# WCC-Analytics/sidecar

Hardware: AMD Instinct MI355X
Metric: record-merges/sec (whole node) + rounds-to-converge wall time, H=32768 S=16 (higher is better)
Workload: dtype int64

## Files before the change

sidecar_amd/csrc/gx_device.hpp:

```cpp
#pragma once
#include <hip/hip_runtime.h>
#include <stdint.h>

#include "../../include/gx.h"

#define GXD __device__ __forceinline__
#define GXHD __host__ __device__ __forceinline__

#define GX_GLOBAL __attribute__((address_space(1)))
typedef unsigned int gx_u32x4 __attribute__((ext_vector_type(4)));
template <class T>
GXD T gld(const T *p) {
  return *(const GX_GLOBAL T *)p;
}
typedef unsigned int gx_u32x3 __attribute__((ext_vector_type(3)));
template <class T>
GXD void gst(T *p, T v) {
  *(GX_GLOBAL T *)p = v;
}
GXD gx_u32x4 gld4(const void *p) { return *(const GX_GLOBAL gx_u32x4 *)p; }
GXD gx_u32x3 gld3(const void *p) { return *(const GX_GLOBAL gx_u32x3 *)p; }
GXD void gst4(void *p, gx_u32x4 v) { *(GX_GLOBAL gx_u32x4 *)p = v; }

struct grec {
  uint64_t w;
  uint32_t r;
  uint32_t pad;
};
GXD grec gld_rec(const grec *p) {
  const gx_u32x4 x = gld4(p);
  grec g;
  g.w = (uint64_t)x.x | ((uint64_t)x.y << 32);
  g.r = x.z;
  g.pad = x.w;
  return g;
}
GXD void gst_rec(grec *p, const grec &g) {
  gx_u32x4 x;
  x.x = (uint32_t)g.w;
  x.y = (uint32_t)(g.w >> 32);
  x.z = g.r;
  x.w = g.pad;
  gst4(p, x);
}

enum {
  C_GOSSIP_MERGES, C_AE_MERGES, C_LOCAL_MERGES, C_GOSSIP_ACC, C_AE_ACC, C_LOCAL_ACC, C_STALE,
  C_RETX, C_QDROP, C_LDROP, C_SDROP, C_PDROP, C_DEQ, C_NIL, C_PACKETS, C_RECSENT, C_EXPIRED,
  C_GC, C_OWNTOMB, C_EXPSRV, C_SENDJOBS, C_AEX, C_CHURN, C_SCANSLOTS, C_AESLOTS, C_BYTESENT,
  C_CAPCUT, C_CHG, C_QDEFER,
  C_LOCKED_MERGES, C_LOCK_BUF, C_LOCK_DROP, C_LOCK_DRAIN, C_AE_LOCKED, C_NCTR
};
enum {
  C_LOST = C_NCTR, C_FD_PROBES, C_FD_PROBE_FAIL, C_FD_SUSPECT, C_FD_CONFIRM, C_FD_DEATH, C_FD_REFUTE,
  C_FD_ALIVE, C_FD_SENT, C_FD_RECV, C_FD_STATE_MERGE, C_EXP_DEFER, C_FEXP, C_AE_DEFER, C_AE_DEFER_LOST, C_FD_HQ, C_FD_HQ_DROP, C_NCTR_ALL
};
#define GX_NCTR_SLOTS 56
static_assert(C_NCTR_ALL <= GX_NCTR_SLOTS, "counter slots");

#define GX_SHARDS 64
#define GX_DI_MAX 256
struct DevCtr {
  unsigned long long c[GX_SHARDS][GX_NCTR_SLOTS];
  unsigned long long last_change_p1[GX_SHARDS][8];
  unsigned long long bytes[GX_SHARDS][16];
  unsigned long long units[GX_SHARDS][16];
  unsigned long long first_drop[GX_SHARDS][8];
};

enum { SRC_GOSSIP = 0, SRC_AE = 1, SRC_LOCAL = 2 };
enum { ST_PEER = 1, ST_PHASE_BS = 2, ST_PHASE_BT = 3, ST_CHURN = 4, ST_INIT_TS = 5, ST_INIT_AGE = 6,
       ST_AE = 7, ST_FD_PHASE = 8, ST_FD_PERM = 9, ST_FD_RELAY = 10, ST_DEPART = 11, ST_PROBE = 12, ST_PP_PHASE = 13 };

#define XPLAN_BATCH 64
#define XPLAN_GMAX 64

struct Dev {
  gx_params p;
  int64_t epoch;
  uint32_t H, S, R, Q, A, L, SQ, DQ, K;
  uint32_t NG, KE;
  uint32_t KG;
  uint32_t lo, Hl, G, gid;
  uint32_t n_remote;
  uint32_t *msg_key;
  uint32_t *in_stamp;
  int64_t round, now;
  int partitioned;
  uint64_t *view;
  unsigned long long *minexp;
  uint8_t *own_status;
  gx_host_state *hs;
  gx_job *fifo;
  gx_sleeper *sleep;
  grec *dq;
  grec *arena;
  uint32_t *arena_len;
  uint32_t AW;
  uint32_t *arena_bits;
  grec *msg;
  uint64_t *msg_w0;
  uint32_t *msg_len;
  uint32_t *msg_dst;
  uint32_t DI;
  uint32_t DR;
  uint32_t *in_cnt;
  uint32_t *in_cnt_nx;
  uint4 *in_hdr;
  uint4 *in_ovf;
  grec *in_rec;
  uint32_t *work_cnt;
  uint32_t *wl_cnt, *wl_cnt_nx;
  uint32_t *ovf_cnt, *ovf_cnt_nx;
  uint32_t *work;
  uint32_t *mrec;
  grec *scan_list;
  uint32_t *scan_cnt;
  uint8_t *tick;
  uint16_t *sbytes;
  gx_server_times *srvt;
  int64_t *vlc;
  int32_t *ev_slot;
  gx_change_event *ev_log;
  uint32_t *ev_cnt;
  uint32_t ev_cap;
  DevCtr *ctr;
  gx_member *mem;
  int32_t *fd_dl;
  gx_fd_host *fdh;
  gx_fd_msg *fdm;
  uint32_t *fd_len;
  uint32_t *fd_peers;
  uint32_t *fd_np;
  uint64_t *fd_snap;
  int pair_split;
  uint64_t divS;
  uint32_t logS;
  int departures;
  uint32_t nblk_ae;
  uint64_t *snap;
  uint32_t snap_tag, snap_word;
  uint32_t *quiet_w;
  uint32_t QW;
  uint32_t sfilt;
  uint32_t C;
  grec *lkb;
  uint32_t PW;
  uint32_t *pexp;
  int in_round;
  uint32_t P;
  uint64_t *dpool;
  uint32_t *dpool_host, *dpool_res;
  uint8_t *ro_flag;
  uint32_t *ro_list;
  uint32_t *dslot;
  uint32_t *claim_bits;
  uint32_t *ro_n;
  uint32_t HQ;
  gx_fd_msg *fdq;
  uint8_t *ob_buf;
  const uint32_t *ob_cnt;
  uint32_t *ob_claim;
  unsigned long long *probe_x;
  unsigned long long *kprof;
};

GXHD uint64_t mix64(uint64_t z) {
  z += 0x9E3779B97F4A7C15ull;
  z = (z ^ (z >> 30)) * 0xBF58476D1CE4E5B9ull;
  z = (z ^ (z >> 27)) * 0x94D049BB133111EBull;
  return z ^ (z >> 31);
}
GXHD uint64_t rng4(uint64_t seed, uint64_t stream, uint64_t a, uint64_t b, uint64_t c) {
  uint64_t h = mix64(seed ^ (stream * 0xD1B54A32D192ED03ull));
  h = mix64(h ^ a);
  h = mix64(h ^ b);
  return mix64(h ^ c);
}
GXHD uint32_t unif(uint64_t x, uint32_t m) { return (uint32_t)(((x >> 32) * (uint64_t)m) >> 32); }
GXHD int st_of(uint64_t w) { return (int)(w & 7u); }
GXHD int64_t ts_of(uint64_t w) { return (int64_t)(w >> GX_TS_SHIFT); }
GXHD uint64_t pack(int64_t ts, int st) { return ((uint64_t)ts << GX_TS_SHIFT) | (uint64_t)st; }

GXHD uint32_t feistel_perm(uint64_t key, uint32_t q, uint32_t m) {
  uint32_t b = 0;
  while ((1u << b) < m) b++;
  uint32_t hb = (b + 1) / 2;
  if (hb == 0) hb = 1;
  uint32_t hmask = (1u << hb) - 1;
  uint32_t x = q;
  do {
    uint32_t L = x >> hb, Rr = x & hmask;
    for (uint32_t i = 0; i < 4; i++) {
      uint32_t F = (uint32_t)(mix64(key ^ ((uint64_t)i << 32) ^ Rr)) & hmask;
      uint32_t t = Rr;
      Rr = L ^ F;
      L = t;
    }
    x = (L << hb) | Rr;
  } while (x >= m);
  return x;
}
GXHD uint32_t feistel_inv(uint64_t key, uint32_t q, uint32_t m) {
  uint32_t b = 0;
  while ((1u << b) < m) b++;
  uint32_t hb = (b + 1) / 2;
  if (hb == 0) hb = 1;
  uint32_t hmask = (1u << hb) - 1;
  uint32_t x = q;
  do {
    uint32_t L = x >> hb, Rr = x & hmask;
    for (int i = 3; i >= 0; i--) {
      const uint32_t pr = L;
      L = Rr ^ ((uint32_t)(mix64(key ^ ((uint64_t)i << 32) ^ pr)) & hmask);
      Rr = pr;
    }
    x = (L << hb) | Rr;
  } while (x >= m);
  return x;
}

GXHD unsigned long long exp_time(const gx_params &p, uint64_t w) {
  int st = st_of(w);
  if (st == GX_ABSENT) return ~0ull;
  int64_t life = st == GX_TOMBSTONE ? p.tombstone_lifespan_ns
                                    : (st == GX_DRAINING ? p.draining_lifespan_ns : p.alive_lifespan_ns);
  return (unsigned long long)(ts_of(w) + life);
}

GXHD bool departed_at(const gx_params &p, int64_t round, uint32_t u) {
  if (p.depart_round < 0 || round < p.depart_round || !p.depart_ppm) return false;
  return (uint32_t)(rng4(p.seed, ST_DEPART, u, 0, 0) % 1000000ull) < p.depart_ppm;
}

GXD uint32_t shard_id() { return blockIdx.x & (GX_SHARDS - 1); }

GXD unsigned long long wave_sum(unsigned long long x) {
  for (int o = 32; o > 0; o >>= 1) x += __shfl_xor(x, o, 64);
  return x;
}
GXD unsigned long long wave_min(unsigned long long x) {
  for (int o = 32; o > 0; o >>= 1) {
    unsigned long long y = __shfl_xor(x, o, 64);
    x = y < x ? y : x;
  }
  return x;
}

GXD uint32_t wave_min32(uint32_t x) {
  for (int o = 32; o > 0; o >>= 1) {
    const uint32_t y = (uint32_t)__shfl_xor((int)x, o, 64);
    x = y < x ? y : x;
  }
  return x;
}

struct Acc {
  unsigned c[C_NCTR];
  bool changed;
  bool locked;
  GXD Acc() : changed(false), locked(false) {
#pragma unroll
    for (int i = 0; i < C_NCTR; i++) c[i] = 0;
  }
};

GXD void ctr_atomic(const Dev &d, int i, unsigned long long v) {
  if (v) atomicAdd(&d.ctr->c[shard_id()][i], v);
}
GXD void mark_change(const Dev &d) {
  atomicMax(&d.ctr->last_change_p1[shard_id()][0], (unsigned long long)(d.round + 1));
}
GXD void kbytes(const Dev &d, int k, unsigned long long b, unsigned long long u) {
  if (b) atomicAdd(&d.ctr->bytes[shard_id()][k], b);
  if (u) atomicAdd(&d.ctr->units[shard_id()][k], u);
}
GXD void acc_flush(const Dev &d, const Acc &a) {
#pragma unroll
  for (int i = 0; i < C_NCTR; i++) {
    if (__ballot(a.c[i] != 0) == 0) continue;
    unsigned long long x = wave_sum((unsigned long long)a.c[i]);
    if ((threadIdx.x & 63) == 0) ctr_atomic(d, i, x);
  }
  bool any = __ballot(a.changed) != 0;
  if ((threadIdx.x & 63) == 0 && any) mark_change(d);
  if (__ballot(a.locked) != 0 && (threadIdx.x & 63) == 0)
    atomicMin(&d.ctr->first_drop[shard_id()][1], (unsigned long long)d.round);
}

GXD uint32_t li(const Dev &d, uint32_t v) { return v - d.lo; }
GXD uint32_t owner_of(const Dev &d, uint32_t r) { return d.S == 1 ? r : (uint32_t)__umul64hi(d.divS, (uint64_t)r); }
GXD bool owned_by(const Dev &d, uint32_t r, uint32_t o) { return r - o * d.S < d.S; }
GXD bool departed(const Dev &d, uint32_t u) { return d.departures && departed_at(d.p, d.round, u); }

GXD void wave_sync() {
  __builtin_amdgcn_fence(__ATOMIC_SEQ_CST, "wavefront");
  __builtin_amdgcn_wave_barrier();
}

#define GX_ERR_INBOX 1u
#define GX_WC_ERR 4
#define GX_WC_SCANS 5
#define GX_WC_N 8
#define GX_SNAP_QUIET 0xffffffffu
GXD uint32_t inbox_claim(const Dev &d, uint32_t vi) { return atomicAdd(&d.in_cnt[vi], 1u); }
GXD void inbox_header(const Dev &d, uint32_t vi, uint32_t pos, uint32_t key, uint32_t entry, uint32_t len,
                      uint32_t slot) {
  if (pos < d.DI) d.in_hdr[(size_t)vi * d.DI + pos] = make_uint4(key, entry, len, slot);
  else d.in_ovf[atomicAdd(d.ovf_cnt, 1u)] = make_uint4(key, entry, len, vi);
}
GXD void inbox_header(const Dev &d, uint32_t vi, uint32_t pos, uint32_t key, uint32_t entry, uint32_t len) {
  inbox_header(d, vi, pos, key, entry, len, pos);
}
GXD void inbox_put(const Dev &d, uint32_t vi, uint32_t key, uint32_t entry, uint32_t len) {
  inbox_header(d, vi, inbox_claim(d, vi), key, entry, len);
}
GXD grec *packet_recs(const Dev &d, uint32_t vi, uint32_t slot, uint32_t entry) {
  return slot < d.DR ? &d.in_rec[((size_t)vi * d.DR + slot) * d.p.packet_cap] : &d.msg[(size_t)entry * d.p.packet_cap];
}
GXD uint4 inbox_next(const Dev &d, uint32_t vi, int64_t after) {
  uint4 best = make_uint4(0xffffffffu, 0u, 0u, 0u);
  bool found = false;
  const uint32_t cnt = d.in_cnt[vi], n = cnt < d.DI ? cnt : d.DI;
  for (uint32_t i = 0; i < n; i++) {
    const uint4 h = d.in_hdr[(size_t)vi * d.DI + i];
    if ((int64_t)h.x > after && (!found || h.x < best.x)) {
      best = h;
      found = true;
    }
  }
  const uint32_t no = *d.ovf_cnt;
  for (uint32_t i = 0; i < no; i++) {
    const uint4 h = d.in_ovf[i];
    if (h.w == vi && (int64_t)h.x > after && (!found || h.x < best.x)) {
      best = make_uint4(h.x, h.y, h.z, 0xffffffffu);
      found = true;
    }
  }
  return best;
}
GXD void flag_live(const Dev &d, uint32_t vi, uint32_t n) { atomicAdd(&d.mrec[vi], n); }
GXD gx_member *memp(const Dev &d, uint32_t v, uint32_t m) { return &d.mem[(size_t)li(d, v) * d.H + m]; }
GXD int32_t *dlp(const Dev &d, uint32_t v, uint32_t m) { return &d.fd_dl[(size_t)li(d, v) * d.H + m]; }
GXD gx_fd_host *fdhp(const Dev &d, uint32_t v) { return &d.fdh[li(d, v)]; }
GXD bool reach(const Dev &d, uint32_t a, uint32_t b) {
  if (departed(d, a) || departed(d, b)) return false;
  return !(d.partitioned && ((a < d.H / 2) != (b < d.H / 2)));
}
GXD uint64_t *vrow(const Dev &d, uint32_t v) { return &d.view[(size_t)li(d, v) * d.R]; }
GXD gx_host_state *hst(const Dev &d, uint32_t v) { return &d.hs[li(d, v)]; }

GXD void set_slot(const Dev &d, Acc &a, uint32_t v, uint64_t *slot, uint64_t nw) {
  if (*slot != nw) {
    *slot = nw;
    a.changed = true;
    atomicMin(&d.minexp[li(d, v)], exp_time(d.p, nw));
  }
}

GXD bool locked_in(const Dev &d, uint32_t lockw) { return GX_LOCK_AT(lockw, d.round) != 0u; }
GXD bool host_locked(const Dev &d, uint32_t v) { return locked_in(d, gld(&hst(d, v)->lock)); }
GXD uint32_t lock_snap(uint32_t lockw, uint32_t flags, int64_t round, bool rw) {
  const uint32_t b = 1u << (round & 1), w = 16u << (round & 1);
  lockw = (lockw & ~b) | ((flags & 3u) ? b : 0u);
  return rw ? (lockw & ~w) | ((flags & 2u) ? w : 0u) : lockw;
}
#define GX_NOHOST 0xffffffffu
#define GX_LOCK_READERS_CLAIMED 2u
GXD bool ro_side(const Dev &d, uint32_t v) {
  const gx_host_state *h = hst(d, v);
  const uint32_t lw = gld(&h->lock);
  return d.p.lock_readers && locked_in(d, lw) && !GX_LOCK_W_AT(lw, d.round) && GX_LOCK_BUF(lw) == 0u &&
         !(lw & (GX_LOCK_PENDING_EXPIRE | GX_LOCK_DEFER_MERGE)) && h->bt_next > d.round;
}
GXD bool ro_pair(const Dev &d, uint32_t a, uint32_t b) {
  return d.p.lock_readers && (!host_locked(d, a) || ro_side(d, a)) && (!host_locked(d, b) || ro_side(d, b));
}
GXD uint32_t pipe_cap(const Dev &d, uint32_t vi, uint32_t lw) {
  if (!(lw & GX_LOCK_DEFER_MERGE)) return d.C;
  uint32_t slot = (d.lo + vi) % d.P;
  if (d.p.lock_readers == GX_LOCK_READERS_CLAIMED) slot = d.dslot[d.lo + vi];
  if (slot >= d.P) return d.C;
  const uint32_t res = d.dpool_res[slot];
  return d.C > res ? d.C - res : 0u;
}
GXD uint32_t quiet_term(const Dev &d, uint32_t vi, const gx_host_state &hs) {
  const uint32_t lw = hs.lock;
  if (!(hs.flags & 3u) || !locked_in(d, lw) || !GX_LOCK_AT(lw, d.round + 1)) return 0u;
  if (GX_LOCK_BUF(lw) < pipe_cap(d, vi, lw)) return 0u;
  uint32_t dist = 0;
  if (hs.flags & 1u) dist = hs.nil_pos_bs - hs.fifo_head;
  if ((hs.flags & 2u) && hs.nil_pos_bt - hs.fifo_head > dist) dist = hs.nil_pos_bt - hs.fifo_head;
  if (dist >= hs.fifo_tail - hs.fifo_head) return 0u;
  const uint32_t kg = d.KG ? d.KG : 1u;
  const uint64_t b = (uint64_t)d.round + 1u + (dist + kg) / kg;
  return b < 0xfffffffeull ? (uint32_t)b : 0xfffffffeu;
}
GXD void next_round_fields(Dev &d) {
  d.round++;
  d.now = d.p.t0_ns + d.round * d.p.round_ns;
  d.partitioned = d.round >= d.p.partition_start && d.round < d.p.partition_end;
  uint32_t *const ic = d.in_cnt, *const wl = d.wl_cnt, *const ov = d.ovf_cnt;
  d.in_cnt = d.in_cnt_nx;
  d.in_cnt_nx = ic;
  d.wl_cnt = d.wl_cnt_nx;
  d.wl_cnt_nx = wl;
  d.ovf_cnt = d.ovf_cnt_nx;
  d.ovf_cnt_nx = ov;
}
GXD void note_locked(const Dev &d) { atomicMin(&d.ctr->first_drop[shard_id()][1], (unsigned long long)d.round); }

GXD gx_server_times *srv_times(const Dev &d, uint32_t v, uint32_t o) {
  return &d.srvt[(size_t)li(d, v) * d.H + o];
}
GXD void ev_put(const Dev &d, int32_t k, uint32_t pos, uint32_t r, uint64_t nw, int prev) {
  if (pos >= d.ev_cap) return;
  gx_change_event ev;
  ev.service.updated_ns = ts_of(nw);
  ev.service.host = r / d.S;
  ev.service.svc = (uint16_t)(r % d.S);
  ev.service.status = (uint8_t)st_of(nw);
  ev.service.flags = 0;
  ev.time_ns = ts_of(nw);
  ev.previous_status = (uint32_t)prev;
  ev.pad = 0;
  d.ev_log[(size_t)k * d.ev_cap + pos] = ev;
}
GXD void svc_changed(const Dev &d, Acc &a, uint32_t v, uint32_t r, uint64_t nw, int prev) {
  int64_t ts = ts_of(nw);
  gx_server_times *t = srv_times(d, v, owner_of(d, r));
  t->last_updated_ns = ts;
  t->last_changed_ns = ts;
  d.vlc[li(d, v)] = ts;
  a.c[C_CHG]++;
  int32_t k = d.ev_slot[li(d, v)];
  if (k >= 0) ev_put(d, k, d.ev_cnt[k]++, r, nw, prev);
}

GXD gx_job make_job(uint64_t a, uint32_t c, uint32_t meta) {
  gx_job j;
  j.a = a;
  j.c = c;
  j.meta = meta;
  return j;
}
GXHD uint32_t meta_of(int kind, uint32_t pass, uint32_t np) { return GX_JOB_META((uint32_t)kind, pass, np, 0); }
GXD uint32_t fifo_room(const Dev &d, uint32_t head, uint32_t tail, uint32_t stored) {
  return stored == tail ? d.Q - (stored - head) : 0u;
}

GXD uint32_t *list_bits(const Dev &d, uint32_t vi, uint32_t w) { return &d.arena_bits[(size_t)vi * d.AW + w]; }
GXD void list_release(const Dev &d, uint32_t vi, uint32_t &arena_used, uint32_t slot, bool lane0) {
  if (slot >= d.A) return;
  if (lane0) atomicAnd(list_bits(d, vi, slot >> 5), ~(1u << (slot & 31)));
  arena_used &= ~(1u << (slot >> 5));
}
template <int T = 1>
GXD int list_alloc(const Dev &d, uint32_t vi, uint32_t &arena_used, bool lane0) {
  const uint32_t wfree = ~arena_used & (d.AW >= 32 ? 0xffffffffu : ((1u << d.AW) - 1u));
  if (!wfree) return -1;
  const uint32_t w = (uint32_t)__builtin_ctz(wfree);
  uint32_t *p = list_bits(d, vi, w);
  uint32_t word = lane0 ? __hip_atomic_load(p, __ATOMIC_RELAXED, __HIP_MEMORY_SCOPE_AGENT) : 0u;
  if (T > 1) word = (uint32_t)__shfl((int)word, 0, T);
  const uint32_t b = (uint32_t)__builtin_ctz(~word), nw = word | (1u << b);
  if (lane0) __hip_atomic_store(p, nw, __ATOMIC_RELAXED, __HIP_MEMORY_SCOPE_AGENT);
  if (nw == 0xffffffffu) arena_used |= 1u << w;
  return (int)(w * 32 + b);
}
GXD void free_list_r(const Dev &d, uint32_t vi, gx_host_state &hs, const gx_job &j, bool lane0) {
  if (GX_JOB_KIND(j.meta) == GX_JOB_SEND) list_release(d, vi, hs.arena_used, j.c & 0xffff, lane0);
}

GXD void push_job_r(const Dev &d, Acc &a, uint32_t v, gx_host_state &hs, const gx_job &j, bool lane0) {
  const uint32_t kind = GX_JOB_KIND(j.meta);
  if (kind == GX_JOB_NIL_BS) hs.nil_pos_bs = hs.fifo_tail;
  else if (kind == GX_JOB_NIL_BT) hs.nil_pos_bt = hs.fifo_tail;
  if (fifo_room(d, hs.fifo_head, hs.fifo_tail, hs.fifo_stored)) {
    if (lane0) d.fifo[(size_t)li(d, v) * d.Q + (hs.fifo_tail % d.Q)] = j;
    hs.fifo_stored++;
  } else {
    if (lane0) a.c[C_QDEFER]++;
    free_list_r(d, li(d, v), hs, j, lane0);
  }
  hs.fifo_tail++;
}
GXD void push_sleep_r(const Dev &d, Acc &a, uint32_t v, gx_host_state &hs, const gx_job &j, uint32_t wake,
                      bool lane0) {
  if (hs.sleep_tail - hs.sleep_head >= d.SQ) {
    if (lane0) a.c[C_SDROP]++;
    free_list_r(d, li(d, v), hs, j, lane0);
    return;
  }
  if (lane0) {
    gx_sleeper *z = &d.sleep[(size_t)li(d, v) * d.SQ + (hs.sleep_tail & (d.SQ - 1u))];
    gx_u32x4 x0, x1;
    x0.x = (uint32_t)j.a;
    x0.y = (uint32_t)(j.a >> 32);
    x0.z = j.c;
    x0.w = j.meta;
    x1.x = wake;
    x1.y = x1.z = x1.w = 0u;
    gst4(&z->job, x0);
    gst4(&z->wake, x1);
  }
  hs.sleep_tail++;
}
GXD void push_job(const Dev &d, Acc &a, uint32_t v, const gx_job &j) {
  gx_host_state *h = hst(d, v);
  const uint32_t kind = GX_JOB_KIND(j.meta), tail = h->fifo_tail, stored = h->fifo_stored;
  if (kind == GX_JOB_NIL_BS) h->nil_pos_bs = tail;
  else if (kind == GX_JOB_NIL_BT) h->nil_pos_bt = tail;
  if (fifo_room(d, h->fifo_head, tail, stored)) {
    d.fifo[(size_t)li(d, v) * d.Q + (tail % d.Q)] = j;
    h->fifo_stored = stored + 1;
  } else {
    a.c[C_QDEFER]++;
    if (kind == GX_JOB_SEND) {
      uint32_t au = h->arena_used;
      list_release(d, li(d, v), au, j.c & 0xffff, true);
      h->arena_used = au;
    }
  }
  h->fifo_tail = tail + 1;
}
GXD void free_list(const Dev &d, uint32_t v, const gx_job &j) {
  gx_host_state *h = hst(d, v);
  uint32_t au = h->arena_used;
  if (GX_JOB_KIND(j.meta) == GX_JOB_SEND) list_release(d, li(d, v), au, j.c & 0xffff, true);
  h->arena_used = au;
}

GXD void wake_host(const Dev &d, Acc &a, uint32_t v) {
  gx_host_state *h = hst(d, v);
  while (h->sleep_head != h->sleep_tail) {
    const gx_sleeper &z = d.sleep[(size_t)li(d, v) * d.SQ + (h->sleep_head & (d.SQ - 1u))];
    if ((int64_t)z.wake > d.round) break;
    const gx_job j = z.job;
    h->sleep_head++;
    push_job(d, a, v, j);
  }
}

GXD gx_job pop_job_r(const Dev &d, uint32_t vi, gx_host_state &hs, const gx_job *pj) {
  const uint32_t p = hs.fifo_head++;
  if (p != hs.fifo_stored) return pj ? *pj : d.fifo[(size_t)vi * d.Q + (p % d.Q)];
  hs.fifo_stored = hs.fifo_head;
  uint32_t kind = GX_JOB_LOST;
  if ((hs.flags & 1u) && p == hs.nil_pos_bs) kind = GX_JOB_NIL_BS;
  else if ((hs.flags & 2u) && p == hs.nil_pos_bt) kind = GX_JOB_NIL_BT;
  return make_job(0, 0, meta_of((int)kind, 0, 1));
}
GXD void count_lost(const Dev &d, Acc &a, bool lane0) {
  if (!lane0) return;
  a.c[C_QDROP]++;
  atomicMin(&d.ctr->first_drop[shard_id()][0], (unsigned long long)d.round);
}

GXD uint32_t ring_add(uint32_t base, uint32_t k, uint32_t q) {
  const uint32_t x = base + k;
  return x >= q ? x - q : x;
// ... 418 lines not shown
```

sidecar_amd/csrc/gx_engine.hip:

```cpp
#include <hip/hip_runtime.h>

#include <math.h>
#include <stdio.h>
#include <stdlib.h>
#include <string.h>

#include <algorithm>
#include <chrono>
#include <deque>
#include <numeric>
#include <string>
#include <thread>
#include <type_traits>
#include <vector>


#define HIPCHK(x)                                                                          \
  do {                                                                                     \
    hipError_t _e = (x);                                                                   \
    if (_e != hipSuccess) {                                                                \
      fprintf(stderr, "gx: HIP error %s at %s:%d\n", hipGetErrorString(_e), __FILE__, __LINE__); \
      return GX_EIO;                                                                       \
    }                                                                                      \
  } while (0)
#define GXTRY(x)         \
  do {                   \
    int rc_ = (x);       \
    if (rc_) return rc_; \
  } while (0)

static uint32_t pow2_at_least(uint32_t x) {
  uint32_t v = 1;
  while (v < x) v <<= 1;
  return v;
}

#include "../../include/gx_watch.h"
#include "../../include/gx_ckpt.h"
#include "gx_kernels.hpp"
#include "gx_fd.hpp"
#include "gx_codec.hpp"

struct TimedLaunch {
  int cls;
  hipEvent_t a, b;
};

struct DevMem {
  struct Buf {
    void *p;
    size_t bytes;
    uint32_t id;
  };
  std::vector<Buf> bufs;
  DevMem() = default;
  DevMem(const DevMem &) = delete;
  DevMem &operator=(const DevMem &) = delete;
  ~DevMem() { release(); }
  template <class T>
  int take(uint32_t id, T *&p, size_t bytes) {
    void *q = nullptr;
    if (hipMalloc(&q, bytes) != hipSuccess) {
      (void)hipGetLastError();
      return GX_ENOMEM;
    }
    bufs.push_back({q, bytes, id});
    p = (T *)q;
    return GX_OK;
  }
  template <class T>
  int take(uint32_t id, T *&p, size_t bytes, int fill, hipStream_t s) {
    GXTRY(take(id, p, bytes));
    if (bytes) HIPCHK(hipMemsetAsync(p, fill, bytes, s));
    return GX_OK;
  }
  template <class T>
  int take(T *&p, size_t bytes) {
    return take(0u, p, bytes);
  }
  template <class T>
  int take(T *&p, size_t bytes, int fill, hipStream_t s) {
    return take(0u, p, bytes, fill, s);
  }
  template <class T>
  void drop(T *&p) {
    bufs.erase(std::remove_if(bufs.begin(), bufs.end(), [&](const Buf &b) { return b.p == (void *)p; }), bufs.end());
    (void)hipFree(p);
    p = nullptr;
  }
  const Buf *find(uint32_t id) const {
    for (const Buf &b : bufs)
      if (b.id == id) return &b;
    return nullptr;
  }
  void release() {
    for (const Buf &b : bufs) (void)hipFree(b.p);
    bufs.clear();
  }
};

struct DevBuf {
  void *p = nullptr;
  size_t cap = 0;
  DevBuf() = default;
  DevBuf(const DevBuf &) = delete;
  DevBuf &operator=(const DevBuf &) = delete;
  ~DevBuf() { (void)hipFree(p); }
};
static int dbuf(DevBuf &b, size_t bytes, void **out, size_t min_cap = 1 << 16) {
  if (bytes > b.cap) {
    (void)hipFree(b.p);
    b.p = nullptr;
    b.cap = 0;
    size_t c = min_cap;
    while (c < bytes) c <<= 1;
    if (hipMalloc(&b.p, c) != hipSuccess) {
      (void)hipGetLastError();
      return GX_ENOMEM;
    }
    b.cap = c;
  }
  *out = b.p;
  return GX_OK;
}

#define GX_QUIET_SLOTS 4

enum AeCall : uint32_t { AE_PLANNED = 1, AE_LOCAL = 2, AE_DELTA = 4, AE_RET = 8, AE_CLAIM = 16 };

struct gx_engine {
  Dev d{};
  DevMem mem;
  hipStream_t stream;
  hipStream_t own_stream;
  hipStream_t side_stream;
  hipEvent_t side_start, side_done;
  bool side_pending;
  bool round_open;
  bool scan_heavy = true;
  uint64_t *scan_snap;
  uint64_t *scan_snap_dev;
  uint32_t scan_tag[2] = {~0u, ~0u};
  uint32_t scan_k, scan_last;
  uint32_t quiet_tag[GX_QUIET_SLOTS], quiet_seq;
  bool quiet_nowait;
  int64_t quiet_until, quiet_from;
  bool quiet_now;
  bool quiet_send = true;
  uint32_t quiet_batch;
  uint32_t *in_cnt_buf;
  int async_phases;
  int device;
  int timing;
  std::vector<TimedLaunch> pending_ev;
  std::vector<uint32_t> pp_host, pp_idx, pp_off;
  int64_t pp_round = -1;
  uint32_t pp_cursor;
  uint32_t *pp_dev;
  int32_t *pp_prow;
  uint32_t *name_rank;
  double ms[GX_K_COUNT];
  uint64_t launches[GX_K_COUNT];
  uint64_t host_bytes[GX_K_COUNT], host_units[GX_K_COUNT];
  struct CodecState *codec;
  uint32_t *ob_entries;
  uint32_t *ob_counts;
  uint32_t n_ob;
  bool ob_async;
  uint32_t *ob_total;
  uint32_t *ae_pa, *ae_pb, *ae_pack_host, *ae_pack_t, *ae_pack_other;
  uint8_t *ae_pack_first, *ae_skip;
  uint64_t *fd_rsnap;
  int32_t *ae_prow;
  uint8_t *ae_pcount;
  uint32_t nblk, nmw;
  ulonglong2 *ae_dig;
  uint32_t *ae_mask;
  uint32_t *ae_fmask;
  uint16_t *ae_lt;
  uint16_t *ae_retL;
  uint32_t *ae_bcnt;
  uint32_t *ae_cnt;
  uint32_t *ae_nfol;
  uint64_t *ae_sz;
  uint64_t *ae_off;
  uint64_t *ae_rioff;
  uint32_t *ae_err;
  uint8_t *ae_rov;
  unsigned long long *ro_xc;
  struct AeChain {
    int64_t step = -1;
    uint32_t done;
    uint32_t n_plan, n_pack;
    std::vector<uint32_t> gstart;
    std::vector<uint64_t> lead_off;
    uint64_t lead_total, lead_in_total, ret_total;
  } chain;
  struct Listener {
    uint32_t view, id, cap;
    std::deque<gx_change_event> ring;
  };
  std::vector<Listener> listeners;
  std::vector<uint32_t> log_views;
  uint64_t listener_drops;
  DevBuf api;
  unsigned long long *conv_bad;
  uint64_t *digest_buf;
  size_t kprof_n;
  hipStream_t xplan_stream;
  uint32_t *xplan_dev;
  uint32_t *xplan_host;
  int64_t xplan_start[2] = {-1, -1};
  uint64_t xplan_waits[2];
  hipEvent_t xplan_ev[2];
  hipEvent_t xplan_join;
  int64_t xbound_round = -1;
  XBound xbound;
  const uint32_t *xbound_dev;
  uint32_t *ob_claim;
  uint32_t scan_nch;
  grec *scan_tmp;
  ScanChunk *scan_chunk;
  struct Watch {
    uint32_t n, log_rounds;
    int64_t first_round;
    uint64_t missed;
    uint32_t *keys;
    uint64_t *thr;
    uint32_t *log;
    std::vector<uint32_t> keys_host;
    std::vector<uint64_t> thr_host;
  } watch;
};

static void codec_free(gx_engine *e);

static int ensure_api(gx_engine *e, size_t bytes) {
  void *p;
  return dbuf(e->api, bytes, &p, 1 << 20);
}

static bool own(const gx_engine *e, uint32_t v) { return v >= e->d.lo && v < e->d.lo + e->d.Hl; }
static bool vec_of(const gx_engine *e) { return e->d.R % 2 == 0; }
static bool ev_of(const gx_engine *e) { return !e->log_views.empty(); }
static bool pp_state(const Dev &d) { return d.p.fd_enable && d.p.fd_push_pull_state; }
static int64_t now_of(const gx_engine *e) { return e->d.p.t0_ns + e->d.round * e->d.p.round_ns; }
static int64_t abs_tm(const gx_engine *e, int64_t t) { return t ? t + e->d.epoch : 0; }
static void set_round_fields(gx_engine *e) {
  Dev &d = e->d;
  const uint32_t par = (uint32_t)(d.round & 1);
  d.in_cnt = e->in_cnt_buf + (size_t)par * d.Hl;
  d.in_cnt_nx = e->in_cnt_buf + (size_t)(par ^ 1u) * d.Hl;
  d.wl_cnt = d.work_cnt + par;
  d.wl_cnt_nx = d.work_cnt + (par ^ 1u);
  d.ovf_cnt = d.work_cnt + 2 + par;
  d.ovf_cnt_nx = d.work_cnt + 2 + (par ^ 1u);
  e->d.now = now_of(e);
  e->d.partitioned = e->d.round >= e->d.p.partition_start && e->d.round < e->d.p.partition_end;
  e->d.pair_split = e->d.partitioned && !e->d.p.fd_enable;
}

struct LaunchTimer {
  gx_engine *e;
  int cls;
  hipEvent_t a, b;
  hipStream_t st;
  LaunchTimer(gx_engine *e_, int cls_, hipStream_t s_ = nullptr) : e(e_), cls(cls_), a(nullptr), b(nullptr), st(s_ ? s_ : e_->stream) {
    e->launches[cls]++;
    if (e->timing) {
      (void)hipEventCreate(&a);
      (void)hipEventCreate(&b);
      (void)hipEventRecord(a, st);
    }
  }
  ~LaunchTimer() {
    if (e->timing) {
      (void)hipEventRecord(b, st);
      e->pending_ev.push_back({cls, a, b});
    }
  }
};

static int drain_timing(gx_engine *e) {
  if (e->pending_ev.empty()) return GX_OK;
  HIPCHK(hipStreamSynchronize(e->stream));
  for (auto &t : e->pending_ev) {
    float ms = 0;
    (void)hipEventElapsedTime(&ms, t.a, t.b);
    e->ms[t.cls] += ms;
    (void)hipEventDestroy(t.a);
    (void)hipEventDestroy(t.b);
  }
  e->pending_ev.clear();
  return GX_OK;
}

static int deliver_events(gx_engine *e) {
  size_t nlog = e->log_views.size();
  if (!nlog) return GX_OK;
  std::vector<uint32_t> cnt(nlog);
  HIPCHK(hipMemcpy(cnt.data(), e->d.ev_cnt, sizeof(uint32_t) * nlog, hipMemcpyDeviceToHost));
  bool any = false;
  for (uint32_t c : cnt) any |= c != 0;
  if (!any) return GX_OK;
  for (size_t k = 0; k < nlog; k++) {
    if (!cnt[k]) continue;
    uint32_t n = cnt[k] < e->d.ev_cap ? cnt[k] : e->d.ev_cap;
    std::vector<gx_change_event> ev(n);
    HIPCHK(hipMemcpy(ev.data(), &e->d.ev_log[k * e->d.ev_cap], sizeof(gx_change_event) * n, hipMemcpyDeviceToHost));
    for (auto &x : ev) {
      x.service.updated_ns += e->d.epoch;
      x.time_ns = abs_tm(e, x.time_ns);
    }
    for (auto &l : e->listeners) {
      if (l.view != e->log_views[k]) continue;
      uint32_t room = l.cap - (uint32_t)l.ring.size();
      uint32_t take = cnt[k] < room ? cnt[k] : room;
      for (uint32_t i = 0; i < take; i++) l.ring.push_back(ev[i]);
      e->listener_drops += cnt[k] - take;
    }
  }
  HIPCHK(hipMemset(e->d.ev_cnt, 0, sizeof(uint32_t) * nlog));
  return GX_OK;
}

static int take_device_error(gx_engine *e) {
  if (e->d.G < 2) return GX_OK;
  uint32_t err = 0;
  HIPCHK(hipMemcpy(&err, &e->d.work_cnt[GX_WC_ERR], sizeof(err), hipMemcpyDeviceToHost));
  if (!err) return GX_OK;
  HIPCHK(hipMemset(&e->d.work_cnt[GX_WC_ERR], 0, sizeof(err)));
  return GX_EINVAL;
}

static int join_side(gx_engine *e) {
  if (!e->side_pending) return GX_OK;
  HIPCHK(hipStreamWaitEvent(e->stream, e->side_done, 0));
  e->side_pending = false;
  return GX_OK;
}

static int sync_main(gx_engine *e) {
  HIPCHK(hipStreamSynchronize(e->stream));
  HIPCHK(hipGetLastError());
  return take_device_error(e);
}

static int sync_check(gx_engine *e) {
  int jr = join_side(e);
  if (jr) return jr;
  HIPCHK(hipStreamSynchronize(e->stream));
  HIPCHK(hipGetLastError());
  int rc = take_device_error(e);
  if (rc) return rc;
  return ev_of(e) ? deliver_events(e) : GX_OK;
}

template <class T>
static int read_back(gx_engine *e, const void *dev, T *host) {
  HIPCHK(hipMemcpyAsync(host, dev, sizeof(T), hipMemcpyDeviceToHost, e->stream));
  return sync_check(e);
}

static int phase_done(gx_engine *e) {
  if (e->async_phases && !ev_of(e)) {
    HIPCHK(hipGetLastError());
    return GX_OK;
  }
  return sync_check(e);
}

static inline unsigned nblk(size_t n, unsigned t) { return (unsigned)((n + t - 1) / t); }

template <class F>
static void with_flag(bool a, F &&f) {
  if (a) f(std::true_type{});
  else f(std::false_type{});
}
template <class F>
static void with_flags(bool a, bool b, F &&f) {
  with_flag(a, [&](auto A) { with_flag(b, [&](auto B) { f(A, B); }); });
}
static int own_class(uint32_t S) { return S <= 4 ? 1 : S <= 8 ? 2 : 4; }
template <class F>
static void with_own(int own, F &&f) {
  if (own == 0) f(std::integral_constant<int, 0>{});
  else if (own == 1) f(std::integral_constant<int, 1>{});
  else if (own == 2) f(std::integral_constant<int, 2>{});
  else f(std::integral_constant<int, 4>{});
}

struct InRound {
  Dev &d;
  explicit InRound(Dev &d_) : d(d_) { d.in_round = 1; }
  ~InRound() { d.in_round = 0; }
};

template <int T>
static void launch_owner(const Dev &d, hipStream_t s) {
  k_owner<T><<<nblk(d.Hl, 256 / T), 256, 0, s>>>(d);
}
static void owner_launch(const Dev &d, hipStream_t s) {
  if (d.S <= 1) launch_owner<1>(d, s);
  else if (d.S <= 2) launch_owner<2>(d, s);
  else if (d.S <= 4) launch_owner<4>(d, s);
  else if (d.S <= 8) launch_owner<8>(d, s);
  else if (d.S <= 16) launch_owner<16>(d, s);
  else if (d.S <= 32) launch_owner<32>(d, s);
  else launch_owner<64>(d, s);
}
#define SCAN_GRID 2048

static int scan_probe_begin(gx_engine *e) {
  e->d.snap = nullptr;
  if (e->d.round % 2) return GX_OK;
  e->d.snap_tag = (uint32_t)e->d.round;
  e->d.snap_word = GX_WC_SCANS;
  const uint32_t i = e->scan_k & 1u;
  if (e->scan_k >= 2) {
    const uint64_t v = __atomic_load_n(&e->scan_snap[i], __ATOMIC_ACQUIRE);
    if ((uint32_t)(v >> 32) == e->scan_tag[i]) {
      e->scan_heavy = (uint32_t)v != e->scan_last;
      e->scan_last = (uint32_t)v;
    }
  }
  e->scan_tag[i] = (uint32_t)e->d.round;
  e->d.snap = &e->scan_snap_dev[i];
  return GX_OK;
}
static int scan_probe_end(gx_engine *e) {
  if (!e->d.snap) return GX_OK;
  if (e->d.snap < &e->scan_snap_dev[2]) e->scan_k++;
  e->d.snap = nullptr;
  return GX_OK;
}

static bool quiet_params(const Dev &d) {
  return d.G == 1 && d.K && d.p.lock_model == 1 && !d.p.lock_readers && !d.p.fd_enable && !d.departures &&
         !d.p.fd_handoff_shared && d.NG == 1 && !d.p.probe_piggyback && !d.p.limit_bytes && d.p.retransmit_rounds > 0;
}
static int quiet_take(gx_engine *e) {
  int free_slot = -1;
  for (int i = GX_QUIET_SLOTS - 1; i >= 0; i--) {
    if (e->quiet_tag[i]) {
      const uint64_t v = __atomic_load_n(&e->scan_snap[2 + i], __ATOMIC_ACQUIRE);
      if ((uint32_t)(v >> 32) != e->quiet_tag[i]) continue;
      e->quiet_tag[i] = 0;
      if ((int64_t)(uint32_t)v > e->quiet_until) e->quiet_until = (int64_t)(uint32_t)v;
    }
    free_slot = i;
  }
  return free_slot;
}
#define GX_QUIET_WAIT_MS 1000
static void quiet_probe(gx_engine *e) {
  Dev &d = e->d;
  int free_slot = quiet_take(e);
  if (d.snap || d.round <= e->quiet_from) return;
  if (free_slot < 0 && !e->quiet_nowait) {
    const auto deadline = std::chrono::steady_clock::now() + std::chrono::milliseconds(GX_QUIET_WAIT_MS);
    while ((free_slot = quiet_take(e)) < 0) {
      if (std::chrono::steady_clock::now() > deadline) {
        e->quiet_nowait = true;
        break;
      }
      std::this_thread::yield();
    }
  }
  if (free_slot < 0) return;
  if (!++e->quiet_seq) ++e->quiet_seq;
  e->quiet_tag[free_slot] = e->quiet_seq;
  d.snap = &e->scan_snap_dev[2 + free_slot];
  d.snap_tag = e->quiet_seq;
  d.snap_word = GX_SNAP_QUIET;
}
static void quiet_invalidate(gx_engine *e) {
  memset(e->quiet_tag, 0, sizeof(e->quiet_tag));
  e->quiet_until = 0;
  e->quiet_from = e->d.round;
}

enum Entry {
  ENTRY_READ,
  ENTRY_MUTATE,
  ENTRY_PHASE,
  ENTRY_ROUNDS,
};
static int enter(gx_engine *e, Entry what) {
  HIPCHK(hipSetDevice(e->device));
  if (what == ENTRY_MUTATE || what == ENTRY_PHASE) quiet_invalidate(e);
  set_round_fields(e);
  return GX_OK;
}
static bool quiet_round(const gx_engine *e, bool storm) {
  return quiet_params(e->d) && !storm && e->log_views.empty() && e->d.round < e->quiet_until;
}

struct SendSel {
  bool x, scan, plan;
  int own;
  bool quiet;
};
static void launch_send(gx_engine *e, SendSel sel, int do_bt, int nr) {
  const Dev &d = e->d;
  const unsigned g = nblk(d.Hl, 64);
  hipStream_t s = e->stream;
  if (sel.quiet && sel.plan && !ev_of(e)) {
    if (!sel.scan) {
      k_send<4, false, false, false, false, 0, true, true><<<g, 256, 0, s>>>(d, do_bt, nr);
      return;
    }
    with_flag(vec_of(e), [&](auto V) {
      with_own(sel.own, [&](auto O) { k_send<4, false, true, V(), false, O(), true, true><<<g, 256, 0, s>>>(d, do_bt, nr); });
    });
    return;
  }
  auto rest = [&](auto X, auto P) {
    if (!sel.scan) {
      k_send<4, X(), false, false, false, 0, P()><<<g, 256, 0, s>>>(d, do_bt, 1);
      return;
    }
    with_flags(vec_of(e), ev_of(e), [&](auto V, auto E) {
      with_own(sel.own, [&](auto O) { k_send<4, X(), true, V(), E(), O(), P()><<<g, 256, 0, s>>>(d, do_bt, 1); });
    });
  };
  if (sel.plan) rest(std::false_type{}, std::true_type{});
  else with_flag(sel.x, [&](auto X) { rest(X, std::false_type{}); });
}

static int round_send_impl(gx_engine *e, int nr = 1) {
  Dev &d = e->d;
  set_round_fields(e);
  InRound in_round_guard(d);
  if (nr > 1) {
    d.snap = nullptr;
    quiet_take(e);
  } else {
    int rc = scan_probe_begin(e);
    if (rc) return rc;
    if (quiet_params(d)) quiet_probe(e);
  }
  d.n_remote = 0;
  hipStream_t s = e->stream;
  if (d.p.probe_piggyback) {
    LaunchTimer t(e, GX_K_SEND);
    k_wake<<<nblk(d.Hl, 64), 64, 0, s>>>(d);
    k_probe<4><<<nblk(d.Hl, 64), 256, 0, s>>>(d);
  }
  const bool vec = vec_of(e), ev = ev_of(e);
  const bool storm = d.p.storm_round >= 0 && d.round == d.p.storm_round && d.H >= 2;
  const bool bt_apart = d.p.fd_enable || storm;
  const bool scan_in_send = !bt_apart && d.K && !e->scan_heavy;
  const bool fused = scan_in_send && d.S <= 16;
  const bool plan = !d.p.limit_bytes && d.p.retransmit_rounds > 0 && !d.departures && !d.p.fd_enable;
  e->quiet_now = quiet_round(e, storm);
  const SendSel sel{d.p.fd_enable || d.departures, scan_in_send, plan, fused ? own_class(d.S) : 0,
                    e->quiet_now && e->quiet_send};
  if (!fused) {
    LaunchTimer t(e, GX_K_OWNER);
    owner_launch(d, s);
  }
  if (!scan_in_send) {
    LaunchTimer t(e, GX_K_SCAN);
    const unsigned grid = d.Hl < SCAN_GRID ? d.Hl : SCAN_GRID;
    if (vec && !ev && e->scan_nch > 1) {
      k_scan_split<true><<<SCAN_GRID, 256, GX_SCAN_WAVE ? 4 * sizeof(grec) * d.L : 0, s>>>(d, e->scan_tmp, e->scan_chunk,
                                                                                         e->scan_nch);
      k_scan_join<<<grid, 256, 0, s>>>(d, e->scan_tmp, e->scan_chunk, e->scan_nch);
    } else {
      with_flags(vec, ev, [&](auto V, auto E) {
        k_scan<V(), E()><<<grid, 256, 0, s>>>(d, d.scan_list, d.L, d.L, d.scan_cnt, -1);
      });
    }
    if (bt_apart) k_bt_finish<<<nblk(d.Hl, 256), 256, 0, s>>>(d);
  }
  if (d.p.fd_enable) {
    LaunchTimer t(e, GX_K_FD);
    k_fd_tick<<<d.Hl, 64, 0, s>>>(d);
  }
  if (storm) {
    LaunchTimer t(e, GX_K_STORM);
    with_flag(ev, [&](auto E) {
      if (d.S >= 2 && 64 % d.S == 0) k_storm_p2<E(), true><<<d.Hl, 256, 0, s>>>(d);
      else k_storm<E()><<<d.Hl, 256, 0, s>>>(d);
    });
  }
  {
    LaunchTimer t(e, GX_K_SEND);
    if (d.p.fd_enable) k_fd_send<<<nblk(d.Hl, 64), 64, 0, s>>>(d);
    launch_send(e, sel, bt_apart ? 0 : 1, sel.quiet ? nr : 1);
  }
  HIPCHK(hipGetLastError());
  return scan_probe_end(e);
}

#ifndef GX_LOCK_APPEND
#define GX_LOCK_APPEND 1
#endif
#ifndef GX_MERGE_LAPP_NR64
#define GX_MERGE_LAPP_NR64 1
#endif
#ifndef GX_LOCK_APPEND_HL
#define GX_LOCK_APPEND_HL 32768
#endif
#ifndef GX_MERGE_SMALL_HL
#define GX_MERGE_SMALL_HL 16384
#endif
static void launch_merge(gx_engine *e, bool small) {
  const Dev &d = e->d;
  const unsigned g = nblk(d.Hl, small ? 16u : (unsigned)MERGE_NR);
  with_flags(d.R < (1u << 26), ev_of(e), [&](auto K32, auto E) {
    if (small) k_merge_seg<K32(), E(), 16, MERGE_WPE_GM><<<g, 64 * MERGE_WAVES, 0, e->stream>>>(d);
    else k_merge_seg<K32(), E()><<<g, 64 * MERGE_WAVES, 0, e->stream>>>(d);
  });
}

static int round_merge_impl(gx_engine *e) {
  Dev &d = e->d;
  set_round_fields(e);
  InRound in_round_guard(d);
  hipStream_t s = e->stream;
  if (d.p.lock_readers) {
    LaunchTimer t(e, GX_K_AE);
    with_flags(vec_of(e), ev_of(e), [&](auto V, auto E) { k_defer_drain<V(), E()><<<d.P, 256, 0, s>>>(d); });
  }
  if (d.KE) {
    LaunchTimer t(e, GX_K_MERGE);
    const bool lapp = GX_LOCK_APPEND && d.p.lock_model && !d.p.fd_handoff_shared && d.NG == 1 && d.Hl >= GX_LOCK_APPEND_HL;
    if (lapp) k_lock_append<<<nblk(d.Hl, 16), 256, 0, s>>>(d);
    const bool small = d.NG > 1 || d.Hl < GX_MERGE_SMALL_HL || (d.p.lock_model && !(GX_MERGE_LAPP_NR64 && lapp));
    launch_merge(e, small);
  }
  if (d.p.fd_enable && d.K) {
    LaunchTimer t(e, GX_K_FD);
    k_fd_recv<<<nblk(d.Hl, 64), 64, 0, s>>>(d);
  }
  HIPCHK(hipGetLastError());
  return GX_OK;
}

#ifndef GX_AE_PF_OFF
#define GX_AE_PF_OFF 1
#endif
#ifndef GX_AE_NT_OFF
#define GX_AE_NT_OFF true
#endif
#ifndef GX_AE_PF_LOCK
#define GX_AE_PF_LOCK 1
#endif
static bool ae_round(const gx_engine *e) {
  const Dev &d = e->d;
  if (d.p.ae_period_rounds && d.p.push_pull_stagger) return true;
  return d.p.ae_period_rounds && (uint64_t)d.round % d.p.ae_period_rounds == d.p.ae_phase;
}
static bool pp_initiates(const Dev &d, uint32_t i) {
  if (!d.p.push_pull_stagger) return true;
  return (uint64_t)d.round % d.p.ae_period_rounds == rng4(d.p.seed, ST_PP_PHASE, i, 0, 0) % d.p.ae_period_rounds;
}
struct AeMatching {
  uint32_t base[2], len[2];
  uint64_t key0, key1;
  uint32_t n0, np;
};
static AeMatching ae_matching(const Dev &d) {
  AeMatching m;
  m.base[0] = 0;
  m.base[1] = d.H / 2;
  m.len[0] = d.pair_split ? d.H / 2 : d.H;
  m.len[1] = d.pair_split ? d.H - d.H / 2 : 0;
  m.key0 = rng4(d.p.seed, ST_AE, (uint64_t)d.round, m.base[0], 0);
  m.key1 = m.len[1] ? rng4(d.p.seed, ST_AE, (uint64_t)d.round, m.base[1], 0) : 0;
  m.n0 = m.len[0] / 2;
  m.np = m.n0 + m.len[1] / 2;
  return m;
}

static bool ae_partner(const Dev &d, uint32_t i, uint32_t *out) {
  uint32_t base = 0, m = d.H;
  if (d.partitioned && !d.p.fd_enable) {
    const uint32_t half = d.H / 2;
    base = i < half ? 0 : half;
    m = i < half ? half : d.H - half;
  }
  if (m < 2) return false;
  const uint64_t x = rng4(d.p.seed, ST_AE, (uint64_t)d.round, i, 1);
  const uint32_t idx = unif(x, m - 1), self = i - base;
  *out = base + (idx >= self ? idx + 1 : idx);
  return true;
}
static void ae_ro_launch(gx_engine *e, const uint32_t *pa, const uint32_t *pb, uint64_t key0, uint64_t key1, uint32_t np) {
  const Dev &d = e->d;
  k_ae_claim<<<1, 256, 0, e->stream>>>(d, pa, pb, key0, key1, np);
  with_flags(vec_of(e), ev_of(e), [&](auto V, auto E) {
    k_ae_rox<V(), E()><<<ae_grid(np, 1), 256, 0, e->stream>>>(d, pa, pb, key0, key1);
  });
}
static void launch_ae_plan(gx_engine *e, bool pf2, unsigned np, hipStream_t st, const uint32_t *pa, const uint32_t *pb,
                           const int32_t *prow, const uint8_t *pcount, const AeIn &in, const uint8_t *skip) {
  const bool ev = ev_of(e);
  with_flag(vec_of(e), [&](auto V) {
    (ev ? k_ae_plan_ev<V()> : pf2 ? k_ae_plan_pf2<V()> : k_ae_plan<V()>)<<<np, 256, 0, st>>>(e->d, pa, pb, prow, pcount, in, skip);
  });
}
static uint32_t pp_schedule(gx_engine *e) {
  Dev &d = e->d;
  if (e->pp_round == d.round) return (uint32_t)e->pp_off.size() - 1;
  set_round_fields(e);
  const bool dep = d.departures;
  std::vector<uint32_t> last(d.H, 0), bat, ia, ib;
  uint32_t nb = 0;
  for (uint32_t i = 0; i < d.H; i++) {
    uint32_t b;
    if (!pp_initiates(d, i) || (dep && departed_at(d.p, d.round, i)) || !ae_partner(d, i, &b) ||
        (dep && departed_at(d.p, d.round, b)))
      continue;
    const uint32_t k = 1 + std::max(last[i], last[b]);
    last[i] = last[b] = k;
    ia.push_back(i);
    ib.push_back(b);
    bat.push_back(k - 1);
    nb = std::max(nb, k);
  }
  const size_t n = ia.size();
  e->pp_off.assign(nb + 1, 0);
  for (uint32_t x : bat) e->pp_off[x + 1]++;
  for (uint32_t q = 0; q < nb; q++) e->pp_off[q + 1] += e->pp_off[q];
  std::vector<uint32_t> cur(e->pp_off.begin(), e->pp_off.end() - 1);
  e->pp_host.assign(2 * n, 0);
  e->pp_idx.assign(n, 0);
  for (size_t t = 0; t < n; t++) {
    const uint32_t at = cur[bat[t]]++;
    e->pp_host[at] = ia[t];
    e->pp_host[n + at] = ib[t];
    e->pp_idx[at] = (uint32_t)t;
  }
  e->pp_round = d.round;
  e->pp_cursor = 0;
  return nb;
}
static bool ae_step_due(gx_engine *e) {
  if (e->d.G < 2 || !ae_round(e)) return false;
  if (e->d.p.push_pull_mode != GX_PP_INITIATE) return true;
  const uint32_t nb = pp_schedule(e);
  return e->pp_cursor < nb;
}
static int64_t ae_step(const gx_engine *e) {
  return e->d.round * (2 * (int64_t)GX_MAX_HOSTS) + (e->d.p.push_pull_mode == GX_PP_INITIATE ? e->pp_cursor : 0);
}
static int ae_initiate(gx_engine *e) {
  Dev &d = e->d;
  const uint32_t nb = pp_schedule(e);
  const size_t n = e->pp_idx.size();
  if (!n) return GX_OK;
  const std::vector<uint32_t> &off = e->pp_off;
  HIPCHK(hipMemcpyAsync(e->pp_dev, e->pp_host.data(), sizeof(uint32_t) * 2 * n, hipMemcpyHostToDevice, e->stream));
  AeIn none;
  memset(&none, 0, sizeof(none));
  LaunchTimer t(e, GX_K_AE);
  for (uint32_t q = 0; q < nb; q++) {
    const uint32_t *pa = e->pp_dev + off[q], *pb = e->pp_dev + n + off[q];
    const unsigned np = off[q + 1] - off[q];
    launch_ae_plan(e, false, np, e->stream, pa, pb, e->pp_prow, nullptr, none, nullptr);
    if (d.p.lock_readers) ae_ro_launch(e, pa, pb, 0, 0, np);
  }
  return GX_OK;
}

static int ae_whole_impl(gx_engine *e, bool quiet) {
  Dev &d = e->d;
  set_round_fields(e);
  hipStream_t s = e->stream;
  if (ae_round(e) && d.p.push_pull_mode == GX_PP_INITIATE) {
    int rc = ae_initiate(e);
    if (rc) return rc;
  } else if (ae_round(e)) {
    const AeMatching m = ae_matching(d);
    const uint32_t np = m.np;
    const uint64_t key0 = m.key0, key1 = m.key1;
    if (np && quiet) {
      LaunchTimer t(e, GX_K_AE);
      k_ae_locked_note<<<1, 64, 0, s>>>(d, np, 1u);
    } else if (np) {
      LaunchTimer t(e, GX_K_AE);
      const bool vec = vec_of(e), ev = ev_of(e);
      if (vec && !ev && d.p.lock_model)
        k_ae_chunk<true, GX_AE_PF_LOCK, true, true><<<ae_grid(np, 1), 256, 0, s>>>(d, key0, key1, np);
      else if (vec && !ev) k_ae<true, GX_AE_PF_OFF, GX_AE_NT_OFF, GX_AE_NT_OFF><<<np, 256, 0, s>>>(d, key0, key1);
      else if (vec) k_ae_ev<true><<<np, 256, 0, s>>>(d, key0, key1);
      else if (!ev) k_ae<false><<<np, 256, 0, s>>>(d, key0, key1);
      else k_ae_ev<false><<<np, 256, 0, s>>>(d, key0, key1);
    }
    if (np && pp_state(d)) {
      LaunchTimer t(e, GX_K_FD);
      k_fd_pushpull_pair<<<np, 128, 0, s>>>(d, key0, key1);
    }
    if (np && d.p.lock_readers) {
      LaunchTimer t(e, GX_K_AE);
      ae_ro_launch(e, nullptr, nullptr, key0, key1, np);
    }
  }
  HIPCHK(hipGetLastError());
  return GX_OK;
}

#define WATCH_GRID 512
static int watch_round_end(gx_engine *e) {
  gx_engine::Watch &w = e->watch;
  Dev &d = e->d;
  if (w.n) {
    const int64_t k = d.round - w.first_round;
    if (k >= (int64_t)w.log_rounds) {
      w.missed++;
    } else if (d.Hl) {
      LaunchTimer t(e, GX_K_CONVERGE);
      const unsigned gx = std::min(nblk(d.Hl, WATCH_VIEWS), (unsigned)WATCH_GRID);
      k_watch<<<dim3(gx, nblk(w.n, 64)), 256, 0, e->stream>>>(d, w.keys, w.thr, w.n, w.log + 2 * ((size_t)w.n + 1) * (size_t)k);
      HIPCHK(hipGetLastError());
    }
  }
  d.round++;
  return GX_OK;
}

static int run_one_round(gx_engine *e) {
  int rc = round_send_impl(e);
  const bool quiet = e->quiet_now;
  e->quiet_now = false;
  if (!rc && !quiet) rc = round_merge_impl(e);
  if (!rc) rc = ae_whole_impl(e, quiet);
  if (!rc) rc = watch_round_end(e);
  return rc;
}

#ifndef GX_QUIET_BATCH
#define GX_QUIET_BATCH 32
#endif
static uint32_t quiet_batch_len(gx_engine *e, uint32_t left) {
  Dev &d = e->d;
  if (e->quiet_batch < 2 || left < 2 || !e->quiet_send || !quiet_params(d) || !e->log_views.empty() || e->watch.n) return 1;
  quiet_take(e);
  const int64_t r0 = d.round;
  if (r0 >= e->quiet_until) return 1;
  uint32_t n = (uint32_t)std::min<int64_t>({(int64_t)left, (int64_t)e->quiet_batch, e->quiet_until - r0});
  for (uint32_t j = 0; j < n; j++) {
    d.round = r0 + j;
    const bool storm = d.p.storm_round >= 0 && d.round == d.p.storm_round;
    if (storm || (d.p.push_pull_mode == GX_PP_INITIATE && ae_round(e))) n = j;
  }
  d.round = r0;
  return n < 2 ? 1 : n;
}
static int run_quiet_batch(gx_engine *e, uint32_t n) {
  Dev &d = e->d;
  int rc = round_send_impl(e, (int)n);
  e->quiet_now = false;
  if (rc) return rc;
  const int64_t r0 = d.round;
  int64_t first = -1;
  uint32_t pairs = 0;
  for (uint32_t j = 0; j < n; j++) {
    d.round = r0 + j;
    if (!ae_round(e)) continue;
    set_round_fields(e);
    const uint32_t np = ae_matching(d).np;
    if (np && first < 0) first = d.round;
    pairs += np;
  }
  if (pairs) {
    d.round = first;
    set_round_fields(e);
    LaunchTimer t(e, GX_K_AE);
    k_ae_locked_note<<<1, 64, 0, e->stream>>>(d, pairs, 1u);
  }
  d.round = r0 + n;
  HIPCHK(hipGetLastError());
  return GX_OK;
}

static int wake_all(gx_engine *e) {
  set_round_fields(e);
  k_wake<<<nblk(e->d.Hl, 64), 64, 0, e->stream>>>(e->d);
  HIPCHK(hipGetLastError());
  return GX_OK;
}

extern "C" {

int gx_abi_version(void) { return GX_ABI_VERSION; }

int gx_set_stream(gx_engine *e, void *stream, int mode) {
  if (!e || (mode & ~(GX_STREAM_CALLER | GX_STREAM_ASYNC))) return GX_EINVAL;
  GXTRY(enter(e, ENTRY_MUTATE));
  if (e->side_pending) HIPCHK(hipStreamSynchronize(e->side_stream));
  e->side_pending = false;
  HIPCHK(hipStreamSynchronize(e->stream));
  e->stream = (mode & GX_STREAM_CALLER) ? (hipStream_t)stream : e->own_stream;
  e->async_phases = (mode & GX_STREAM_ASYNC) ? 1 : 0;
  return GX_OK;
}
const char *gx_backend(void) { return "hip-gfx950"; }

void gx_params_default(gx_params *p) {
  memset(p, 0, sizeof(*p));
  p->n_hosts = 64;
  p->n_services = 8;
  p->fanout = 3;
  p->packet_cap = 32;
  p->pending_cap = 100;
  p->queue_cap = 1024;
  p->list_slots = 16;
  p->gossip_stop_on_empty = 1;
  p->alive_interval_rounds = 5;
  p->tombstone_interval_rounds = 10;
  p->retransmit_rounds = 5;
  p->alive_count = 5;
  p->tombstone_count = 10;
  p->init_mode = GX_INIT_EMPTY;
  p->t0_ns = 1700000000000000000ll;
  p->round_ns = 200000000ll;
  p->alive_lifespan_ns = 80000000000ll;
  p->draining_lifespan_ns = 600000000000ll;
  p->tombstone_lifespan_ns = 10800000000000ll;
  p->stale_fudge_ns = 60000000000ll;
  p->alive_broadcast_interval_ns = 60000000000ll;
  p->pass_increment_ns = 50;
  p->tombstone_bump_ns = 1000000000ll;
  p->seed = 0x5EEDull;
  p->aged_max_ns = 100000000000ll;
  p->storm_round = -1;
  p->overhead_bytes = 3;
  p->fd_probe_rounds = 5;
  p->fd_indirect_checks = 3;
  p->fd_msg_cap = 16;
  p->fd_msg_bytes = 64;
  p->fd_gossip_dead_rounds = 150;
  p->depart_round = -1;
  p->fd_push_pull_state = 1;
  p->lock_model = 1;
  p->lock_buffer = 1024 + 1 + 25 + 1 + 25 + 1;
  gx_fd_defaults(p);
}

int gx_fd_defaults(gx_params *p) {
  if (!p || p->n_hosts < 1 || p->fd_probe_rounds < 1 || p->round_ns <= 0) return GX_EINVAL;
  const int suspicion_mult = 4, max_mult = 6, retransmit_mult = 4;
  const double n = (double)p->n_hosts;
  uint32_t limit = (uint32_t)(retransmit_mult * (int)ceil(log10(n + 1.0)));
  p->fd_retransmit_limit = limit > GX_FD_MAX_TX ? GX_FD_MAX_TX : limit;
  const double node_scale = fmax(1.0, log10(fmax(1.0, n)));
  const int64_t interval = (int64_t)p->fd_probe_rounds * p->round_ns;
  const int64_t tmin = (int64_t)suspicion_mult * (int64_t)(node_scale * 1000.0) * interval / 1000;
  const int64_t tmax = (int64_t)max_mult * tmin;
  int k = suspicion_mult - 2;
  if ((int)p->n_hosts - 2 < k) k = 0;
  p->fd_suspicion_k = (uint32_t)k;
  for (int c = 0; c < 8; c++) {
    int64_t t = tmin;
    if (c == 0) {
      t = k < 1 ? tmin : tmax;
    } else if (c <= k) {
      const double frac = log((double)c + 1.0) / log((double)k + 1.0);
      const double raw = (double)tmax / 1e9 - frac * ((double)tmax / 1e9 - (double)tmin / 1e9);
      t = (int64_t)floor(1000.0 * raw) * 1000000ll;
      if (t < tmin) t = tmin;
    }
    p->fd_suspicion_rounds[c] = (uint32_t)((t + p->round_ns - 1) / p->round_ns);
  }
  return GX_OK;
}

static int check_params(const gx_params *p) {
  if (!p || p->n_hosts < 1 || p->n_services < 1 || p->n_services > 64) return GX_EINVAL;
  if (p->fanout > 16 || p->packet_cap < 1 || p->packet_cap > 256 || p->pending_cap > 256) return GX_EINVAL;
  if (p->queue_cap < 1 || p->list_slots < 1 || p->list_slots > GX_MAX_LIST_SLOTS) return GX_EINVAL;
  if (p->n_hosts > GX_MAX_HOSTS) return GX_EINVAL;
  if (p->alive_interval_rounds < 1 || p->tombstone_interval_rounds < 1) return GX_EINVAL;
  if (p->retransmit_rounds > 1000) return GX_EINVAL;
  if (p->alive_count < 1 || p->alive_count > GX_JOB_MAX_PASSES || p->tombstone_count < 1 ||
      p->tombstone_count > GX_JOB_MAX_PASSES)
    return GX_EINVAL;
  if (p->init_mode > GX_INIT_WARM) return GX_EINVAL;
  if (p->t0_ns < 0 || p->t0_ns > ((int64_t)1 << 62) || p->round_ns <= 0) return GX_EINVAL;
  {
    const int64_t lim = (int64_t)1 << 58;
    for (int64_t x : {p->alive_lifespan_ns, p->draining_lifespan_ns, p->tombstone_lifespan_ns, p->stale_fudge_ns,
                      p->aged_max_ns})
      if (x < 0 || x > lim) return GX_EINVAL;
  }
  if ((uint64_t)p->n_hosts * p->n_services > 0xffffffffull) return GX_EINVAL;
  if (p->ae_period_rounds && p->ae_phase >= p->ae_period_rounds) return GX_EINVAL;
  if (p->limit_bytes > (1u << 24) || p->overhead_bytes > (1u << 16)) return GX_EINVAL;
  if (p->n_shards > 1 && (p->shard_id >= p->n_shards || p->n_shards > p->n_hosts || p->n_shards > 64)) return GX_EINVAL;
  if (p->depart_ppm > 1000000u) return GX_EINVAL;
  if (p->gossip_messages > 16) return GX_EINVAL;
  if (p->push_pull_mode > GX_PP_INITIATE || (p->push_pull_mode == GX_PP_INITIATE && p->fd_enable)) return GX_EINVAL;
  if (p->inbox_slots > GX_DI_MAX) return GX_EINVAL;
  if (p->lock_model > 1 || p->lock_buffer < 1 || p->lock_buffer > 65535) return GX_EINVAL;
  if (p->lock_model && (((uint64_t)p->n_hosts + (p->n_shards > 1 ? p->n_shards : 1) - 1) / (p->n_shards > 1 ? p->n_shards : 1)) *
                               p->lock_buffer * 16ull > GX_LOCK_BUF_MAX_BYTES)
    return GX_EINVAL;
  if (p->probe_piggyback > 1 || (p->probe_piggyback && (p->fd_enable || p->fd_probe_rounds < 1)))
    return GX_EINVAL;
  if (p->push_pull_stagger > 1 || (p->push_pull_stagger && (p->push_pull_mode != GX_PP_INITIATE || !p->ae_period_rounds)))
    return GX_EINVAL;
  if (p->lock_readers > GX_LOCK_READERS_CLAIMED || (p->lock_readers && !p->lock_model) || p->lock_defer_slots > GX_POOL_MAX)
    return GX_EINVAL;
  if (p->lock_readers && p->n_shards > 1 && (p->lock_readers == GX_LOCK_READERS_CLAIMED || p->fd_enable))
    return GX_EINVAL;
  if (p->fd_handoff_shared > 1 || (p->fd_handoff_shared && (!p->fd_enable || !p->lock_model || p->n_shards > 1)))
    return GX_EINVAL;
  if (p->fd_enable) {
    if (p->n_hosts > 65534 || p->fanout > 16) return GX_EINVAL;
    if (p->fd_probe_rounds < 1 || p->fd_indirect_checks > 16 || p->fd_msg_cap < 1 || p->fd_msg_cap > 64) return GX_EINVAL;
    if (p->fd_retransmit_limit < 1 || p->fd_retransmit_limit > GX_FD_MAX_TX || p->fd_suspicion_k > 2) return GX_EINVAL;
    for (uint32_t c = 0; c <= p->fd_suspicion_k; c++)
      if (p->fd_suspicion_rounds[c] > (1u << 30)) return GX_EINVAL;
  }
  return GX_OK;
}

int gx_destroy(gx_engine *e) {
  if (!e) return GX_EINVAL;
  (void)hipSetDevice(e->device);
  if (e->stream) (void)hipStreamSynchronize(e->stream);
  if (e->side_stream) (void)hipStreamSynchronize(e->side_stream);
  if (e->xplan_stream) (void)hipStreamSynchronize(e->xplan_stream);
  for (auto &t : e->pending_ev) {
    (void)hipEventDestroy(t.a);
    (void)hipEventDestroy(t.b);
  }
  e->mem.release();
  codec_free(e);
  if (e->own_stream) (void)hipStreamDestroy(e->own_stream);
  if (e->side_stream) (void)hipStreamDestroy(e->side_stream);
  if (e->xplan_stream) (void)hipStreamDestroy(e->xplan_stream);
  for (hipEvent_t ev : {e->side_start, e->side_done, e->xplan_ev[0], e->xplan_ev[1], e->xplan_join})
    if (ev) (void)hipEventDestroy(ev);
  if (e->scan_snap) (void)hipHostFree(e->scan_snap);
  if (e->xplan_host) (void)hipHostFree(e->xplan_host);
  delete e;
  return GX_OK;
}

static void create_dims(gx_engine *e, const gx_params *p) {
  Dev &d = e->d;
  d.p = *p;
  d.epoch = gx_epoch_of(p->t0_ns);
  d.p.t0_ns -= d.epoch;
  d.H = p->n_hosts;
  d.S = p->n_services;
  d.R = p->n_hosts * p->n_services;
  d.Q = p->queue_cap;
  d.A = p->list_slots;
  d.AW = (d.A + 31) / 32;
  d.L = p->packet_cap + p->pending_cap;
  d.K = p->fanout;
  d.NG = p->gossip_messages > 1 ? p->gossip_messages : 1;
  d.KG = d.K * d.NG;
  d.KE = d.KG + (p->probe_piggyback ? 2u : 0u);
  d.divS = d.S > 1 ? ~0ull / d.S + 1 : 0;
  while ((1u << d.logS) < d.S) d.logS++;
  d.G = p->n_shards > 1 ? p->n_shards : 1;
  d.gid = d.G > 1 ? p->shard_id : 0;
  d.lo = (uint32_t)(((uint64_t)d.gid * d.H) / d.G);
  d.Hl = (uint32_t)(((uint64_t)(d.gid + 1) * d.H) / d.G) - d.lo;
  d.SQ = pow2_at_least(64 > d.KE * (p->retransmit_rounds + 1) ? 64 : d.KE * (p->retransmit_rounds + 1));
  d.DQ = pow2_at_least(d.L + p->pending_cap + 64);
  d.nblk_ae = (d.R + GX_DIGEST_SLOTS - 1) / GX_DIGEST_SLOTS;
  d.DI = p->inbox_slots ? p->inbox_slots : (d.NG > 1 ? GX_DI_MAX : 64);
  d.DR = d.DI < 8 ? d.DI : 8;
  d.sfilt = 1u;
  d.QW = 4 * nblk(d.Hl ? d.Hl : 1, 64);
  d.departures = p->depart_round >= 0 && p->depart_ppm;
  if (p->lock_model) {
    d.C = p->lock_buffer;
    d.PW = (d.H + 31) / 32;
    if (p->lock_readers) d.P = p->lock_defer_slots ? p->lock_defer_slots : 64;
    if (p->fd_handoff_shared) d.HQ = d.C > GX_LOCK_HANDLER_AT ? d.C - GX_LOCK_HANDLER_AT : 0;
  }
  e->scan_nch = 1;
  if (d.R >= 65536 && d.S >= 2 && 128 % d.S == 0)
    e->scan_nch = d.R / 32768 < 16 ? d.R / 32768 : 16;
  if (getenv("GX_KPROF"))
    e->kprof_n = (size_t)nblk(d.Hl, 64) * 4 * 8 + GX_KPROF_MERGE_N + 3ull * d.H;
  if (const char *qs = getenv("GX_QUIET_SEND")) e->quiet_send = strcmp(qs, "0") != 0;
  e->quiet_batch = GX_QUIET_BATCH;
  if (const char *qb = getenv("GX_QUIET_BATCH")) e->quiet_batch = (uint32_t)std::min(std::max(atol(qb), 1l), 1024l);
  if (d.G > 1) {
    e->nblk = d.nblk_ae;
    e->nmw = (e->nblk + 31) / 32;
  }
}

static int create_streams(gx_engine *e) {
  HIPCHK(hipStreamCreateWithFlags(&e->own_stream, hipStreamNonBlocking));
  e->stream = e->own_stream;
  HIPCHK(hipStreamCreateWithFlags(&e->side_stream, hipStreamNonBlocking));
  HIPCHK(hipEventCreateWithFlags(&e->side_start, hipEventDisableTiming));
  HIPCHK(hipEventCreateWithFlags(&e->side_done, hipEventDisableTiming));
  HIPCHK(hipHostMalloc((void **)&e->scan_snap, (2 + GX_QUIET_SLOTS) * sizeof(uint64_t), hipHostMallocMapped));
  HIPCHK(hipHostGetDevicePointer((void **)&e->scan_snap_dev, e->scan_snap, 0));
  e->scan_snap[0] = e->scan_snap[1] = ~0ull;
  for (int i = 0; i < GX_QUIET_SLOTS; i++) e->scan_snap[2 + i] = 0;
  return GX_OK;
}

#define DERIVED 0u
#define TAKE(...) GXTRY(e->mem.take(__VA_ARGS__))

static int create_buffers(gx_engine *e) {
  Dev &d = e->d;
  const gx_params *p = &d.p;
  hipStream_t s = e->stream;
  const size_t Hg = d.H, H = d.Hl, K = d.KE ? d.KE : 1;
  TAKE(GX_CK_VIEW, d.view, sizeof(uint64_t) * H * d.R);
  TAKE(GX_CK_OWN_STATUS, d.own_status, H * d.S);
  TAKE(GX_CK_HS, d.hs, sizeof(gx_host_state) * H);
  TAKE(GX_CK_FIFO, d.fifo, sizeof(gx_job) * H * d.Q);
  TAKE(GX_CK_SLEEP, d.sleep, sizeof(gx_sleeper) * H * d.SQ);
  TAKE(GX_CK_DQ, d.dq, sizeof(grec) * H * d.DQ);
  TAKE(GX_CK_ARENA, d.arena, sizeof(grec) * H * d.A * d.L);
  TAKE(GX_CK_ARENA_LEN, d.arena_len, sizeof(uint32_t) * H * d.A, 0, s);
  TAKE(GX_CK_ARENA_BITS, d.arena_bits, sizeof(uint32_t) * H * d.AW);
  TAKE(GX_CK_MSG, d.msg, sizeof(grec) * Hg * K * p->packet_cap);
  TAKE(GX_CK_MSG_W0, d.msg_w0, sizeof(uint64_t) * Hg * K * p->packet_cap);
  TAKE(GX_CK_MSG_LEN, d.msg_len, sizeof(uint32_t) * Hg * K, 0, s);
  TAKE(GX_CK_MSG_DST, d.msg_dst, sizeof(uint32_t) * Hg * K);
  TAKE(GX_CK_MSG_KEY, d.msg_key, sizeof(uint32_t) * Hg * K);
  TAKE(GX_CK_IN_CNT, e->in_cnt_buf, sizeof(uint32_t) * 2 * H, 0, s);
  TAKE(GX_CK_IN_HDR, d.in_hdr, sizeof(uint4) * H * d.DI);
  TAKE(GX_CK_IN_OVF, d.in_ovf, sizeof(uint4) * Hg * K);
  TAKE(GX_CK_IN_REC, d.in_rec, sizeof(grec) * H * d.DR * p->packet_cap);
  TAKE(GX_CK_WORK_CNT, d.work_cnt, sizeof(uint32_t) * GX_WC_N, 0, s);
  TAKE(DERIVED, d.quiet_w, sizeof(uint32_t) * 2 * d.QW, 0, s);
  TAKE(GX_CK_WORK, d.work, sizeof(uint32_t) * H);
  if (p->push_pull_mode == GX_PP_INITIATE && d.G < 2) {
    TAKE(DERIVED, e->pp_dev, sizeof(uint32_t) * 2 * Hg);
    TAKE(DERIVED, e->pp_prow, sizeof(int32_t) * Hg, 0xff, s);
  }
  TAKE(GX_CK_MREC, d.mrec, sizeof(uint32_t) * H, 0, s);
  TAKE(GX_CK_MINEXP, d.minexp, sizeof(unsigned long long) * H);
  TAKE(GX_CK_SCAN_LIST, d.scan_list, sizeof(grec) * H * d.L);
  TAKE(GX_CK_SCAN_CNT, d.scan_cnt, sizeof(uint32_t) * H);
  if (e->scan_nch > 1) {
    TAKE(DERIVED, e->scan_tmp, sizeof(grec) * H * e->scan_nch * d.L);
    TAKE(DERIVED, e->scan_chunk, sizeof(ScanChunk) * H * e->scan_nch);
  }
  TAKE(GX_CK_TICK, d.tick, H, 0, s);
  TAKE(GX_CK_SBYTES, d.sbytes, sizeof(uint16_t) * d.R);
  TAKE(GX_CK_SRVT, d.srvt, sizeof(gx_server_times) * H * Hg);
  TAKE(GX_CK_VLC, d.vlc, sizeof(int64_t) * H);
  TAKE(DERIVED, d.ev_slot, sizeof(int32_t) * H, 0xff, s);
  TAKE(GX_CK_CTR, d.ctr, sizeof(DevCtr), 0, s);
  if (p->fd_enable) {
    TAKE(GX_CK_MEM, d.mem, sizeof(gx_member) * H * Hg);
    TAKE(GX_CK_FD_DL, d.fd_dl, sizeof(int32_t) * H * Hg);
    TAKE(GX_CK_FDH, d.fdh, sizeof(gx_fd_host) * H);
    TAKE(GX_CK_FDM, d.fdm, sizeof(gx_fd_msg) * Hg * K * p->fd_msg_cap);
    TAKE(GX_CK_FD_LEN, d.fd_len, sizeof(uint32_t) * Hg * K, 0, s);
    TAKE(GX_CK_FD_PEERS, d.fd_peers, sizeof(uint32_t) * H * K);
    TAKE(GX_CK_FD_NP, d.fd_np, sizeof(uint32_t) * H);
    if (p->fd_push_pull_state) TAKE(GX_CK_FD_SNAP, d.fd_snap, sizeof(uint64_t) * H * Hg);
  }
  if (p->lock_model) {
    TAKE(GX_CK_LKB, d.lkb, sizeof(grec) * H * d.C);
    if (p->storm_round >= 0 || p->fd_enable) TAKE(GX_CK_PEXP, d.pexp, sizeof(uint32_t) * H * d.PW, 0, s);
    if (p->lock_readers) {
      TAKE(GX_CK_DPOOL, d.dpool, sizeof(uint64_t) * d.P * d.R);
      TAKE(GX_CK_DPOOL_HOST, d.dpool_host, sizeof(uint32_t) * d.P, 0xff, s);
      TAKE(GX_CK_DPOOL_RES, d.dpool_res, sizeof(uint32_t) * d.P, 0, s);
      TAKE(DERIVED, d.ro_flag, H, 0, s);
      TAKE(DERIVED, d.ro_list, sizeof(uint32_t) * H);
      TAKE(DERIVED, d.ro_n, sizeof(uint32_t), 0, s);
      TAKE(GX_CK_DSLOT, d.dslot, sizeof(uint32_t) * Hg, 0xff, s);
      TAKE(DERIVED, d.claim_bits, sizeof(uint32_t) * ((Hg + 31) / 32), 0, s);
    }
    if (p->fd_handoff_shared) TAKE(GX_CK_FDQ, d.fdq, sizeof(gx_fd_msg) * H * (d.HQ ? d.HQ : 1));
  }
  TAKE(DERIVED, e->conv_bad, sizeof(unsigned long long));
  if (e->kprof_n) TAKE(DERIVED, d.kprof, sizeof(unsigned long long) * e->kprof_n, 0, s);
  TAKE(DERIVED, e->digest_buf, sizeof(uint64_t) * H);
  if (d.G > 1) {
    TAKE(DERIVED, e->ob_entries, sizeof(uint32_t) * H * K);
    TAKE(GX_CK_IN_STAMP, d.in_stamp, sizeof(uint32_t) * Hg * K, 0, s);
    TAKE(DERIVED, e->ob_total, sizeof(uint32_t));
    TAKE(DERIVED, e->ob_claim, sizeof(uint32_t) * (XPLAN_GMAX + 1), 0, s);
    if (p->probe_piggyback) TAKE(GX_CK_PROBE_X, d.probe_x, sizeof(unsigned long long) * 2, 0, s);
    TAKE(DERIVED, e->ob_counts, sizeof(uint32_t) * d.G * (1 + 2 * ((H * K + 255) / 256)));
    const size_t np = Hg / 2 + 1;
    TAKE(DERIVED, e->ae_pa, sizeof(uint32_t) * np);
    TAKE(DERIVED, e->ae_pb, sizeof(uint32_t) * np);
    TAKE(DERIVED, e->ae_prow, sizeof(int32_t) * np);
    TAKE(DERIVED, e->ae_pcount, np);
    TAKE(DERIVED, e->ae_pack_host, sizeof(uint32_t) * np);
    TAKE(DERIVED, e->ae_pack_t, sizeof(uint32_t) * np);
    TAKE(DERIVED, e->ae_pack_other, sizeof(uint32_t) * np);
    TAKE(DERIVED, e->ae_pack_first, np);
    TAKE(DERIVED, e->ae_skip, np);
    if (pp_state(d)) TAKE(DERIVED, e->fd_rsnap, sizeof(uint64_t) * np * Hg);
    TAKE(DERIVED, e->ae_dig, sizeof(ulonglong2) * H * e->nblk);
    TAKE(DERIVED, e->ae_mask, sizeof(uint32_t) * H * e->nmw);
    TAKE(DERIVED, e->ae_fmask, sizeof(uint32_t) * H * e->nmw);
    TAKE(DERIVED, e->ae_lt, sizeof(uint16_t) * H * e->nblk);
    TAKE(DERIVED, e->ae_retL, sizeof(uint16_t) * H * e->nblk);
    TAKE(DERIVED, e->ae_bcnt, sizeof(uint32_t) * H * e->nblk);
    TAKE(DERIVED, e->ae_cnt, sizeof(uint32_t) * H);
    TAKE(DERIVED, e->ae_nfol, sizeof(uint32_t) * H);
    TAKE(DERIVED, e->ae_sz, sizeof(uint64_t) * 4 * H);
    TAKE(DERIVED, e->ae_off, sizeof(uint64_t) * 4 * H);
    TAKE(DERIVED, e->ae_rioff, sizeof(uint64_t) * H);
    TAKE(DERIVED, e->ae_err, sizeof(uint32_t));
    if (p->lock_readers) {
      TAKE(DERIVED, e->ae_rov, np, 0, s);
      TAKE(GX_CK_RO_XC, e->ro_xc, sizeof(unsigned long long) * 3, 0, s);
    }
  }
  return GX_OK;
}
#undef TAKE
#undef DERIVED

static int create_init(gx_engine *e) {
  Dev &d = e->d;
  hipStream_t s = e->stream;
  DevMem tmp;
  uint64_t *rec_word;
  GXTRY(tmp.take(rec_word, sizeof(uint64_t) * d.R));
  HIPCHK(hipMemsetAsync(d.ctr->first_drop, 0xff, sizeof(d.ctr->first_drop), s));
  k_fill_u16<<<256, 256, 0, s>>>(d.sbytes, d.R, (uint16_t)GX_STATIC_BYTES_DEFAULT);
  set_round_fields(e);
  k_init_rec<<<nblk(d.R, 256), 256, 0, s>>>(d, rec_word);
  k_init_views<<<2048, 256, 0, s>>>(d, rec_word);
  k_init_times<<<2048, 256, 0, s>>>(d, rec_word);
  k_init_hosts<<<nblk(d.Hl, 256), 256, 0, s>>>(d);
  if (d.p.fd_enable) k_fd_init<<<2048, 256, 0, s>>>(d);
  k_minexp_recompute<<<d.Hl, 256, 0, s>>>(d, 0);
  return sync_check(e);
}

int gx_create(const gx_params *p, gx_engine **out) {
  if (!out) return GX_EINVAL;
  int rc = check_params(p);
  if (rc) return rc;
  int ndev = 0;
  if (hipGetDeviceCount(&ndev) != hipSuccess || ndev <= 0 || p->device < 0 || p->device >= ndev) return GX_EIO;
  HIPCHK(hipSetDevice(p->device));
  gx_engine *e = new gx_engine();
  e->device = p->device;
  create_dims(e, p);
  if ((rc = create_streams(e)) || (rc = create_buffers(e)) || (rc = create_init(e))) {
    (void)hipGetLastError();
    gx_destroy(e);
    return rc;
  }
  *out = e;
  return GX_OK;
}

int gx_set_round(gx_engine *e, int64_t round) {
  if (!e || round < e->d.round || round >= GX_MAX_ROUND) return GX_EINVAL;
  const bool jump = round != e->d.round;
  e->d.round = round;
  e->pp_cursor = 0;
  GXTRY(enter(e, ENTRY_MUTATE));
  if (jump) {
    HIPCHK(hipMemsetAsync(e->in_cnt_buf, 0, sizeof(uint32_t) * 2 * e->d.Hl, e->stream));
    HIPCHK(hipMemsetAsync(e->d.work_cnt, 0, sizeof(uint32_t) * GX_WC_ERR, e->stream));
  }
  int rc = wake_all(e);
  return rc ? rc : sync_check(e);
}

int gx_get_round(gx_engine *e, int64_t *round) {
  if (!e || !round) return GX_EINVAL;
  *round = e->d.round;
  return GX_OK;
}

int gx_enable_timing(gx_engine *e, int on) {
  if (!e) return GX_EINVAL;
  e->timing = on ? 1 : 0;
  return GX_OK;
}

int gx_run_rounds(gx_engine *e, uint32_t n_rounds) {
  if (!e || e->d.G > 1 || e->d.round + n_rounds >= GX_MAX_ROUND) return GX_EINVAL;
  GXTRY(enter(e, ENTRY_ROUNDS));
  e->quiet_nowait = false;
  for (uint32_t i = 0; i < n_rounds;) {
    const uint32_t nb = quiet_batch_len(e, n_rounds - i);
    int rc = nb > 1 ? run_quiet_batch(e, nb) : run_one_round(e);
    if (rc) return rc;
    i += nb;
    if (e->pending_ev.size() > 4096) {
      rc = drain_timing(e);
      if (rc) return rc;
    }
  }
  int rc = wake_all(e);
  if (rc) return rc;
  return sync_check(e);
}

static uint32_t shard_of(const Dev &d, uint32_t v) {
  uint32_t g = (uint32_t)(((uint64_t)v * d.G) / d.H);
  while (g > 0 && (uint32_t)(((uint64_t)g * d.H) / d.G) > v) g--;
  while (g + 1 < d.G && (uint32_t)(((uint64_t)(g + 1) * d.H) / d.G) <= v) g++;
  return g;
}
static size_t slot_bytes(const Dev &d) {
  return 16 + 16ull * d.p.packet_cap + (d.p.fd_enable ? 16ull * d.p.fd_msg_cap : 0);
}

int gx_round_send(gx_engine *e) {
  if (!e) return GX_EINVAL;
  GXTRY(enter(e, ENTRY_PHASE));
  e->round_open = true;
  int rc = round_send_impl(e);
  return rc ? rc : phase_done(e);
}

static void outbox_plan(gx_engine *e) {
  const Dev &d = e->d;
  const size_t ne = (size_t)d.Hl * d.KE;
  const uint32_t nchunk = (uint32_t)((ne + 255) / 256);
  uint32_t *ccnt = e->ob_counts + d.G, *off = ccnt + (size_t)nchunk * d.G;
  const size_t lds = sizeof(uint32_t) * 4 * d.G;
  k_ob_count<<<nchunk, 256, lds, e->stream>>>(d, ccnt);
  k_ob_scan<<<1, 256, 0, e->stream>>>(d, ccnt, nchunk, off, e->ob_counts);
  k_ob_fill<<<nchunk, 256, lds, e->stream>>>(d, off, e->ob_entries);
}

int gx_outbox_bytes(gx_engine *e, uint64_t *bytes) {
  if (!e || !bytes) return GX_EINVAL;
  GXTRY(enter(e, ENTRY_PHASE));
  Dev &d = e->d;
  for (uint32_t g = 0; g < d.G; g++) bytes[g] = 0;
  e->n_ob = 0;
  e->ob_async = false;
  if (d.G < 2 || !d.KE) return GX_OK;
  outbox_plan(e);
  std::vector<uint32_t> cnt(d.G);
  HIPCHK(hipMemcpyAsync(cnt.data(), e->ob_counts, sizeof(uint32_t) * d.G, hipMemcpyDeviceToHost, e->stream));
  int rc = sync_check(e);
  if (rc) return rc;
  uint64_t n = 0;
  for (uint32_t g = 0; g < d.G; g++) {
    bytes[g] = cnt[g] * slot_bytes(d);
    n += cnt[g];
  }
  e->n_ob = (uint32_t)n;
  return GX_OK;
}

int gx_outbox_sizes_async(gx_engine *e, uint64_t *bytes) {
  if (!e || !bytes) return GX_EINVAL;
  GXTRY(enter(e, ENTRY_PHASE));
  Dev &d = e->d;
  e->n_ob = 0;
  e->ob_async = false;
  if (d.G < 2 || !d.KE) {
    HIPCHK(hipMemsetAsync(bytes, 0, sizeof(uint64_t) * d.G, e->stream));
    return phase_done(e);
  }
  outbox_plan(e);
  k_ob_bytes<<<1, 64, 0, e->stream>>>(d, e->ob_counts, (unsigned long long *)bytes, e->ob_total);
  e->ob_async = true;
  return phase_done(e);
}

int gx_outbox_pack(gx_engine *e, void *buf, uint64_t cap) {
  if (!e || (cap && !buf)) return GX_EINVAL;
  if (!e->ob_async && !e->n_ob) return GX_OK;
  if (!e->ob_async && cap < e->n_ob * slot_bytes(e->d)) return GX_EINVAL;
  GXTRY(enter(e, ENTRY_PHASE));
  if (e->ob_async) {
    e->ob_async = false;
    const uint32_t cap_slots = (uint32_t)(cap / slot_bytes(e->d));
    const uint32_t nmax = e->d.Hl * e->d.KE;
    if (nmax) k_outbox_pack<<<nmax, 64, 0, e->stream>>>(e->d, e->ob_entries, 0, (uint8_t *)buf, e->ob_total, cap_slots);
    return phase_done(e);
  }
  k_outbox_pack<<<e->n_ob, 64, 0, e->stream>>>(e->d, e->ob_entries, e->n_ob, (uint8_t *)buf);
  return phase_done(e);
}

static bool send_packs(const Dev &d);
static int xplan_launch(gx_engine *e, int k, int64_t start) {
  Dev &d = e->d;
  const size_t n = (size_t)XPLAN_BATCH * d.G * d.G;
  uint32_t *dev = e->xplan_dev + (size_t)k * n;
  if (send_packs(d)) {
    HIPCHK(hipEventRecord(e->xplan_join, e->stream));
    HIPCHK(hipStreamWaitEvent(e->xplan_stream, e->xplan_join, 0));
  }
  HIPCHK(hipMemsetAsync(dev, 0, sizeof(uint32_t) * n, e->xplan_stream));
  k_xplan<<<dim3(nblk(d.H, 256), XPLAN_BATCH), 256, 0, e->xplan_stream>>>(d, start, dev);
  HIPCHK(hipGetLastError());
  HIPCHK(hipMemcpyAsync(e->xplan_host + (size_t)k * n, dev, sizeof(uint32_t) * n, hipMemcpyDeviceToHost,
                        e->xplan_stream));
  HIPCHK(hipEventRecord(e->xplan_ev[k], e->xplan_stream));
  e->xplan_start[k] = start;
  return GX_OK;
}
static int xplan_counts(gx_engine *e, const uint32_t **out) {
  Dev &d = e->d;
  if (!e->xplan_dev) {
    if (hipStreamCreateWithFlags(&e->xplan_stream, hipStreamNonBlocking) != hipSuccess ||
        hipEventCreateWithFlags(&e->xplan_ev[0], hipEventDisableTiming) != hipSuccess ||
        hipEventCreateWithFlags(&e->xplan_ev[1], hipEventDisableTiming) != hipSuccess ||
        hipEventCreateWithFlags(&e->xplan_join, hipEventDisableTiming) != hipSuccess ||
        hipHostMalloc((void **)&e->xplan_host, sizeof(uint32_t) * 2 * XPLAN_BATCH * d.G * d.G) != hipSuccess ||
        e->mem.take(e->xplan_dev, sizeof(uint32_t) * 2 * XPLAN_BATCH * d.G * d.G)) {
      (void)hipGetLastError();
      return GX_ENOMEM;
    }
  }
  const int64_t start = d.round - d.round % XPLAN_BATCH;
  const int k = (int)((start / XPLAN_BATCH) & 1);
  int rc = GX_OK;
  if (e->xplan_start[k] != start) rc = xplan_launch(e, k, start);
  if (!rc && e->xplan_start[k ^ 1] != start + XPLAN_BATCH) rc = xplan_launch(e, k ^ 1, start + XPLAN_BATCH);
  if (rc) return rc;
  e->xplan_waits[1]++;
  const hipError_t q = hipEventQuery(e->xplan_ev[k]);
  if (q == hipErrorNotReady) {
    e->xplan_waits[0]++;
    HIPCHK(hipEventSynchronize(e->xplan_ev[k]));
  } else {
    HIPCHK(q);
  }
  const size_t row = ((size_t)k * XPLAN_BATCH + (size_t)(d.round - start)) * d.G * d.G;
  *out = e->xplan_host + row;
  e->xbound_dev = e->xplan_dev + row + (size_t)d.gid * d.G;
  return GX_OK;
}

int gx_exchange_plan(gx_engine *e, uint64_t *sizes) {
  if (!e || !sizes) return GX_EINVAL;
  Dev &d = e->d;
  if (d.p.fd_enable) return GX_ENOSYS;
  if (d.G > XPLAN_GMAX) return GX_EINVAL;
  for (uint32_t i = 0; i < d.G * d.G; i++) sizes[i] = 0;
  if (d.G < 2 || !d.KE) return GX_OK;
  GXTRY(enter(e, ENTRY_PHASE));
// ... 112 lines not shown
```

sidecar_amd/csrc/gx_kernels.hpp:

```cpp
#pragma once
#include "gx_device.hpp"

GXD unsigned long long block_excl_scan64(unsigned long long x, unsigned long long *s_wave,
                                         unsigned long long &total) {
  uint32_t lane = threadIdx.x & 63, w = threadIdx.x >> 6, nw = (blockDim.x + 63) >> 6;
  unsigned long long incl = x;
  for (int o = 1; o < 64; o <<= 1) {
    unsigned long long y = __shfl_up(incl, o, 64);
    if ((int)lane >= o) incl += y;
  }
  if (lane == 63) s_wave[w] = incl;
  __syncthreads();
  unsigned long long off = 0, tot = 0;
  for (uint32_t i = 0; i < nw; i++) {
    unsigned long long c = s_wave[i];
    if (i < w) off += c;
    tot += c;
  }
  __syncthreads();
  total = tot;
  return off + incl - x;
}
GXD uint32_t fld(unsigned long long x, int i) { return (uint32_t)((x >> (16 * i)) & 0xffffu); }

// ... 1176 lines not shown
    h->fifo_tail = tail0 + jobs;
    h->fifo_stored = st0 + ok;
    if (jobs) d.vlc[vi] = d.now;
    if (evk >= 0) d.ev_cnt[evk] = ev0 + n_ev;
    kbytes(d, GX_K_STORM, 8ull * (hi - lo) * d.S + 16ull * ok + 16ull * jobs, (unsigned long long)(hi - lo) * d.S);
    ctr_atomic(d, C_EXPSRV, jobs);
    ctr_atomic(d, C_QDEFER, jobs - ok);
  }
}

GXD uint64_t peer_seed(const Dev &d) {
  return mix64(mix64(d.p.seed ^ ((uint64_t)ST_PEER * 0xD1B54A32D192ED03ull)) ^ (uint64_t)d.round);
}
GXD uint32_t sample_peers_h(const Dev &d, uint64_t h2, uint32_t u, uint32_t *peers) {
  uint32_t base = 0, m = d.H;
  if (d.partitioned) {
    uint32_t half = d.H / 2;
    if (u < half) {
      base = 0;
      m = half;
    } else {
      base = half;
      m = d.H - half;
    }
  }
  if (m < 2) return 0;
  const uint64_t h3 = mix64(h2 ^ u);
  uint32_t want = d.K < m - 1 ? d.K : m - 1, cnt = 0;
  for (uint32_t a = 0; cnt < want && a < 64u * d.K; a++) {
    uint64_t x = mix64(h3 ^ a);
    uint32_t idx = unif(x, m - 1), self = u - base;
    uint32_t p = base + (idx >= self ? idx + 1 : idx);
    bool dup = false;
    for (uint32_t i = 0; i < cnt; i++) dup |= peers[i] == p;
    if (!dup) peers[cnt++] = p;
  }
  return cnt;
}
GXD uint32_t sample_peers(const Dev &d, uint32_t u, uint32_t *peers) {
  uint32_t base = 0, m = d.H;
  if (d.partitioned) {
    uint32_t half = d.H / 2;
    if (u < half) {
      base = 0;
      m = half;
    } else {
      base = half;
      m = d.H - half;
    }
  }
  if (m < 2) return 0;
  uint32_t want = d.K < m - 1 ? d.K : m - 1, cnt = 0;
  for (uint32_t a = 0; cnt < want && a < 64u * d.K; a++) {
    uint64_t x = rng4(d.p.seed, ST_PEER, (uint64_t)d.round, u, a);
    uint32_t idx = unif(x, m - 1), self = u - base;
    uint32_t p = base + (idx >= self ? idx + 1 : idx);
    bool dup = false;
    for (uint32_t i = 0; i < cnt; i++) dup |= peers[i] == p;
    if (!dup) peers[cnt++] = p;
  }
  return cnt;
}

#define GX_KP(k)                                                                                   \
  do {                                                                                             \
    if (d.kprof && (threadIdx.x & 63) == 0)                                                        \
      d.kprof[((size_t)blockIdx.x * (blockDim.x >> 6) + (threadIdx.x >> 6)) * 8 + (k)] = wall_clock64(); \
  } while (0)

#ifndef PLAN_CH
#define PLAN_CH 4
#endif
#ifdef GX_SEND_SPLIT
#define GX_SPLIT_DECL unsigned long long sp_t = wall_clock64(), sp_acc[4] = {0, 0, 0, 0}, sp_n = 0, sp_rf = 0;
#define GX_SPLIT(k)                              \
  do {                                           \
    const unsigned long long t_ = wall_clock64(); \
    sp_acc[k] += t_ - sp_t;                      \
    sp_t = t_;                                   \
  } while (0)
#define GX_SPLIT_FLUSH()                                                                                 \
  do {                                                                                                   \
    if (d.kprof && (threadIdx.x & 63) == 0) {                                                           \
      unsigned long long *k_ = &d.kprof[((size_t)blockIdx.x * (blockDim.x >> 6) + (threadIdx.x >> 6)) * 8]; \
      k_[1] = sp_acc[0];                                                                                 \
      k_[2] = sp_acc[1];                                                                                 \
      k_[3] = sp_acc[2];                                                                                 \
      k_[4] = sp_acc[3];                                                                                 \
      k_[5] = sp_n;                                                                                      \
      k_[6] = sp_rf;                                                                                     \
    }                                                                                                    \
  } while (0)
#else
#define GX_SPLIT_DECL
#define GX_SPLIT(k) \
  do {              \
  } while (0)
#define GX_SPLIT_FLUSH() \
  do {                   \
  } while (0)
#endif
#ifndef GX_PLAN_RECS
#define GX_PLAN_RECS 32
#endif
#define PLAN_RECS GX_PLAN_RECS
struct PlanCall {
  uint64_t bw;
  uint64_t emask;
  const grec *list;
  const uint64_t *row;
  uint32_t kind, rb;
  uint32_t m, l;
  uint32_t head, nh;
  uint32_t push;
  uint32_t x, key;
  uint32_t peer;
  uint32_t lpre;
  uint32_t lk;
  uint32_t oslot;
};
GXD uint32_t shard_of_d(const Dev &d, uint32_t v) {
  uint32_t g = (uint32_t)(((uint64_t)v * d.G) / d.H);
  while (g > 0 && (uint32_t)(((uint64_t)g * d.H) / d.G) > v) g--;
  while (g + 1 < d.G && (uint32_t)(((uint64_t)(g + 1) * d.H) / d.G) <= v) g++;
  return g;
}
GXD uint32_t *ob_slot_hdr(const Dev &d, uint32_t slot) {
  return reinterpret_cast<uint32_t *>(d.ob_buf + (size_t)slot * (16u + 16u * d.p.packet_cap));
}
static_assert(sizeof(PlanCall) >= 17 * sizeof(uint32_t), "a PlanCall slot holds a team's 16 peers and their count");
#define GX_NOSLOT 0xffffffffu
#define GX_NOSLOT_W0 0xfffffffeu
GXD bool w0_fwd(const Dev &d, uint32_t slot, uint32_t tick, uint32_t key, uint32_t v) {
  return slot == GX_NOSLOT_W0 && tick != 2 && !owned_by(d, key, v);
}

GXD grec plan_item(const Dev &d, const PlanCall &c, uint32_t i) {
  grec g;
  g.pad = 0;
  if (c.kind == GX_JOB_SEND) {
    const grec s = c.list[i];
    g.w = s.w + c.bw;
    g.r = s.r;
  } else if (c.kind == GX_JOB_EXPIRE) {
    g.w = c.bw;
    g.r = c.rb + (c.emask ? nth_set_bit(c.emask, i) : i);
  } else {
    g.w = c.bw;
    g.r = c.rb;
  }
  return g;
}

template <int T, bool QUIET = false>
GXD void send_planned(const Dev &d, Acc &a, uint32_t idx, gx_host_state &hs, gx_job *pjs, PlanCall *pl,
                      const uint32_t *peers, uint32_t np, unsigned long long &kb, unsigned long long &kl,
                      uint32_t npf0 = 0) {
  constexpr int PLAN_Q = PLAN_RECS / T;
  const uint32_t lane = threadIdx.x & 63, tl = lane & (T - 1), tw = lane / T;
  const bool lead = tl == 0;
  const uint64_t tmask = T == 64 ? ~0ull : ((1ull << T) - 1ull);
  const uint32_t u = d.lo + idx, cap = d.p.packet_cap, mask = d.DQ - 1;
  grec *dq = &d.dq[(size_t)idx * d.DQ];
  grec *const arena_t = &d.arena[(size_t)idx * d.A * d.L];
  grec *const msg_t = &d.msg[(size_t)idx * d.KE * cap];
  uint64_t *const w0_t = &d.msg_w0[(size_t)idx * d.KE * cap];
  const int64_t t_stale = d.now - d.p.tombstone_lifespan_ns - d.p.stale_fudge_ns;
  const int64_t t_gc = d.now - d.p.tombstone_lifespan_ns;
  uint32_t pf0 = hs.fifo_head, npf = npf0;
  uint32_t j = 0, n = 0;
  bool stop = np == 0;
  unsigned fm = 0, fs = 0, nlines = 0;
  GX_SPLIT_DECL
  const bool lmod = QUIET || d.p.lock_model != 0;
  constexpr int NR = (16 + T - 1) / T;
  const bool direct = !QUIET && d.ob_buf != nullptr;
  uint32_t osl[NR];
  uint32_t emit = 0;
#pragma unroll
  for (int r = 0; r < NR; r++) osl[r] = GX_NOSLOT;
  uint32_t og[NR], rk[NR], ksrc[NR], krun[NR], lc[NR], lb[NR], le[NR];
  if (direct) {
    unsigned long long pend[NR];
#pragma unroll
    for (int r = 0; r < NR; r++) {
      const uint32_t jj = (uint32_t)r * T + tl;
      og[r] = jj < np && peers[jj] - d.lo >= d.Hl ? shard_of_d(d, peers[jj]) : d.G;
      pend[r] = __ballot(og[r] < d.G);
      rk[r] = ksrc[r] = krun[r] = lc[r] = 0;
    }
    for (;;) {
      int r0 = -1;
#pragma unroll
      for (int r = NR - 1; r >= 0; r--) r0 = pend[r] ? r : r0;
      if (r0 < 0) break;
      unsigned long long p0 = pend[0];
      uint32_t g0 = og[0];
#pragma unroll
      for (int r = 1; r < NR; r++) {
        p0 = r == r0 ? pend[r] : p0;
        g0 = r == r0 ? og[r] : g0;
      }
      const uint32_t src = (uint32_t)__builtin_ctzll(p0);
      const uint32_t gs = (uint32_t)__shfl((int)g0, (int)src, 64);
      uint32_t acc = 0;
#pragma unroll
      for (int r = 0; r < NR; r++) {
        const unsigned long long m = __ballot(og[r] == gs);
        if (og[r] == gs) {
          rk[r] = acc + (uint32_t)__popcll(m & ((1ull << lane) - 1ull));
          ksrc[r] = src;
          krun[r] = (uint32_t)r0;
        }
        acc += (uint32_t)__popcll(m);
        pend[r] &= ~m;
      }
#pragma unroll
      for (int r = 0; r < NR; r++)
        if (r == r0 && lane == src) lc[r] = acc;
    }
#pragma unroll
    for (int r = 0; r < NR; r++) {
      lb[r] = le[r] = 0;
      if (lc[r]) {
        lb[r] = atomicAdd(&d.ob_claim[og[r]], lc[r]);
        le[r] = d.ob_cnt[og[r]];
      }
    }
  }
  uint32_t lkm = QUIET ? ~0u : 0u, fullm = lkm;
  for (uint32_t j0 = 0; !QUIET && j0 < np; j0 += T) {
    const uint32_t jj = j0 + tl;
    const uint32_t lw = jj < np && peers[jj] - d.lo < d.Hl ? gld(&hst(d, peers[jj])->lock) : 0u;
    const bool lk = locked_in(d, lw);
    lkm |= (uint32_t)((__ballot(lk) >> (tw * T)) & tmask) << j0;
    const bool full = lk && GX_LOCK_BUF(lw) >= pipe_cap(d, jj < np ? peers[jj] - d.lo : 0u, lw);
    fullm |= (uint32_t)((__ballot(full) >> (tw * T)) & tmask) << j0;
  }
  if (direct) {
#pragma unroll
    for (int r = 0; r < NR; r++) {
      if (lc[r]) {
        uint32_t st = 0;
        for (uint32_t x = 0; x < og[r]; x++) st += d.ob_cnt[x];
        if (lb[r] + lc[r] > le[r]) atomicOr(&d.work_cnt[GX_WC_ERR], GX_ERR_INBOX);
        lb[r] += st;
        le[r] += st;
      }
    }
#pragma unroll
    for (int r = 0; r < NR; r++) {
      uint32_t b = 0, e = 0;
#pragma unroll
      for (int r2 = 0; r2 < NR; r2++) {
        const uint32_t x = (uint32_t)__shfl((int)lb[r2], (int)ksrc[r], 64), y = (uint32_t)__shfl((int)le[r2], (int)ksrc[r], 64);
        if (krun[r] == (uint32_t)r2) {
          b = x;
          e = y;
        }
      }
      if (og[r] < d.G && b + rk[r] < e) osl[r] = b + rk[r];
    }
  }
  while (!stop) {
#ifdef GX_SEND_SPLIT
    sp_n++;
    sp_t = wall_clock64();
#endif
    uint32_t nc = 0, tot = 0;
    bool any_push = false;
    PlanCall cp;
    cp.push = 0;
    while (nc < PLAN_CH && !stop) {
      PlanCall c;
      c.kind = 0xffu;
      c.bw = c.emask = 0;
      c.rb = 0;
      c.list = nullptr;
      c.m = 0;
      c.push = 0;
      c.peer = peers[j];
      c.row = !QUIET && c.peer - d.lo < d.Hl ? &d.view[(size_t)(c.peer - d.lo) * d.R] : nullptr;
      c.lk = ((lkm >> j) & 1u) | (lmod ? ((fullm >> j) & 1u) << 1 : 0u);
      c.x = idx * d.KE + j * d.NG + n;
      c.key = u * d.KE + j * d.NG + n;
      c.oslot = GX_NOSLOT;
      if (direct && !c.row) {
        uint32_t v = osl[0];
#pragma unroll
        for (int r = 1; r < NR; r++) v = j / T == (uint32_t)r ? osl[r] : v;
        c.oslot = (uint32_t)__shfl((int)v, (int)(j % T), T);
      }
      bool empty = false;
      if (hs.fifo_head != hs.fifo_tail) {
        gx_job jb = make_job(0, 0, 0);
        if (hs.fifo_head != hs.fifo_stored) {
          uint32_t q = hs.fifo_head - pf0;
          if (q >= npf) {
            const uint32_t left = hs.fifo_stored - hs.fifo_head, win = pj_window<T>(d);
            const uint32_t nl = left < win ? left : win;
            wave_sync();
            for (uint32_t x = tl; x < nl; x += T) pjs[x] = d.fifo[(size_t)idx * d.Q + ((hs.fifo_head + x) % d.Q)];
            wave_sync();
#ifdef GX_SEND_SPLIT
            sp_rf++;
#endif
            pf0 = hs.fifo_head;
            npf = nl;
            q = 0;
            if (lead) kb += 16ull * npf;
          }
          jb = pjs[q];
          hs.fifo_head++;
        } else {
          jb = pop_job_r(d, idx, hs, nullptr);
        }
        if (lead) a.c[C_DEQ]++;
        const uint32_t kind = GX_JOB_KIND(jb.meta), pass = GX_JOB_PASS(jb.meta), npass = GX_JOB_NPASSES(jb.meta);
        if (kind == GX_JOB_LOST) {
          count_lost(d, a, lead);
        } else if (kind == GX_JOB_NIL_BS) {
          if (lead) a.c[C_NIL]++;
          hs.flags &= ~1u;
          hs.bs_next = d.round + d.p.alive_interval_rounds;
        } else if (kind == GX_JOB_NIL_BT) {
          if (lead) a.c[C_NIL]++;
          hs.flags &= ~2u;
          hs.bt_next = d.round + d.p.tombstone_interval_rounds;
        } else if (kind == GX_JOB_SEND || kind == GX_JOB_EXPIRE) {
          if (pass + 1 < npass) {
            gx_job nj = jb;
            nj.meta = GX_JOB_META(kind, pass + 1, npass, GX_JOB_OWNER(jb.meta));
            push_sleep_r(d, a, u, hs, nj, (uint32_t)(d.round + d.p.retransmit_rounds), lead);
          } else {
            free_list_r(d, idx, hs, jb, lead);
          }
        }
        c.m = job_len(d, jb);
        c.kind = kind;
        const uint64_t dw = ((uint64_t)pass * (uint64_t)d.p.pass_increment_ns) << GX_TS_SHIFT;
        if (kind == GX_JOB_RETX) {
          c.bw = jb.a;
          c.rb = jb.c;
        } else if (kind == GX_JOB_SEND) {
          c.bw = dw;
          c.list = arena_t + (size_t)(jb.c & 0xffffu) * d.L;
        } else if (kind == GX_JOB_EXPIRE) {
          c.bw = pack(d.p.t0_ns + (int64_t)jb.c * d.p.round_ns, GX_TOMBSTONE) + dw;
          c.rb = GX_JOB_OWNER(jb.meta) * d.S;
          c.emask = (uint32_t)__popcll(jb.a) == d.S ? 0ull : jb.a;
        }
      } else if (hs.dq_len == 0) {
        empty = true;
      }
      uint32_t l = 0;
      if (!empty) {
        const uint32_t nn = c.m + hs.dq_len;
        l = nn < cap ? nn : cap;
        c.head = hs.dq_head;
        if (l < c.m) {
          c.push = c.m - l;
          c.nh = (c.head - c.push) & mask;
          any_push = true;
        } else {
          c.nh = (c.head + (l - c.m)) & mask;
        }
        hs.dq_head = c.nh;
        hs.dq_len = nn - l;
        if (hs.dq_len > d.p.pending_cap) {
          if (lead) a.c[C_PDROP] += hs.dq_len - d.p.pending_cap;
          hs.dq_len = d.p.pending_cap;
        }
        if (l && lead) {
          a.c[C_PACKETS]++;
          a.c[C_RECSENT] += l;
          const uint32_t lb = l < c.m ? l : c.m;
          const bool filt = c.row && !(lmod && c.lk);
          if (c.lk & 2u) {
            a.c[C_LOCK_DROP] += l;
          } else {
            kb += 16ull * ((c.kind == GX_JOB_SEND ? lb : 0u) + (l - lb)) + (filt ? 8ull * l : 0ull);
          }
          if (filt) fm += l;
          if (c.lk) {
            a.locked = true;
            if (!lmod) a.c[C_LOCKED_MERGES] += l;
          }
        }
      }
      c.l = l;
      c.lpre = tot;
      if (l) {
        if (c.oslot != GX_NOSLOT) emit |= 1u << j;
        if constexpr (QUIET) {
          if (c.push) cp = c;
        } else {
          if (lead) pl[nc] = c;
        }
        nc++;
        if (!(c.lk & 2u)) tot += l;
      }
      const bool pushed = c.push != 0;
      if (l == 0) {
        if (n == 0 && d.p.gossip_stop_on_empty) stop = true;
        j++;
        n = 0;
      } else if (++n == d.NG) {
        j++;
        n = 0;
      }
      if (j >= np) stop = true;
      if (pushed) break;
    }
    if (nc == 0) break;
    if constexpr (QUIET) {
#ifndef GX_SEND_SPLIT
      if (j <= PLAN_CH) {
        GX_KP(5);
        GX_KP(6);
      }
#endif
      GX_SPLIT(0);
      for (uint32_t qq = (tl - cp.nh) & (T - 1); qq < cp.push; qq += T) {
        dq[(cp.nh + qq) & mask] = plan_item(d, cp, cp.l + qq);
        kb += 16;
      }
      GX_SPLIT(3);
      continue;
    }
    wave_sync();
#ifndef GX_SEND_SPLIT
    if (j <= PLAN_CH) GX_KP(5);
#endif
    GX_SPLIT(0);
    uint32_t lp[PLAN_CH], cb[PLAN_CH];
#pragma unroll
    for (int k = 0; k < PLAN_CH; k++) {
      lp[k] = (uint32_t)k < nc ? pl[k].lpre : 0xffffffffu;
      cb[k] = 0;
    }
    uint32_t run = 0;
    uint32_t lcarry = 0xffffffffu;
    for (uint32_t fb = 0; fb < tot; fb += T * PLAN_Q) {
      uint64_t w[PLAN_Q];
      uint32_t r[PLAN_Q], ck[PLAN_Q];
      uint32_t sel[PLAN_Q];
      gx_u32x3 lx[PLAN_Q];
      uint64_t w0[PLAN_Q];
#pragma unroll
      for (int q = 0; q < PLAN_Q; q++) {
        const uint32_t f = fb + tl + T * q;
        uint32_t k = 0;
#pragma unroll
        for (int kk = 1; kk < PLAN_CH; kk++) k += f >= lp[kk] ? 1u : 0u;
        ck[q] = k;
        const PlanCall &c = pl[k];
        const uint32_t i = f - c.lpre;
        const bool valid = f < tot, batch = i < c.m;
        const grec *src = dq;
        sel[q] = 0;
        if (valid && batch && c.kind == GX_JOB_SEND) {
          src = &c.list[i];
          sel[q] = 1;
        } else if (valid && !batch) {
          src = &dq[(c.head + (i - c.m)) & mask];
          sel[q] = 2;
        }
        lx[q] = gld3(src);
        w[q] = c.bw;
        r[q] = c.rb + (c.kind == GX_JOB_EXPIRE ? (c.emask ? nth_set_bit(c.emask, i) : i) : 0u);
        const bool filt = valid && c.row && !(lmod && c.lk);
        const uint64_t *row = filt ? c.row : reinterpret_cast<const uint64_t *>(dq);
        w0[q] = gld(&row[filt && sel[q] == 0 && r[q] < d.R ? r[q] : 0u]);
      }
      bool reload = false;
#pragma unroll
      for (int q = 0; q < PLAN_Q; q++) {
        const PlanCall &c = pl[ck[q]];
        if (sel[q]) {
          w[q] = ((uint64_t)lx[q].x | ((uint64_t)lx[q].y << 32)) + (sel[q] == 1 ? w[q] : 0ull);
          r[q] = lx[q].z;
          reload |= c.row && !(lmod && c.lk);
        }
      }
      if (__ballot(reload)) {
#pragma unroll
        for (int q = 0; q < PLAN_Q; q++) {
          const PlanCall &c = pl[ck[q]];
          const bool fl = sel[q] && c.row && !(lmod && c.lk);
          const uint64_t *row = fl ? c.row : reinterpret_cast<const uint64_t *>(dq);
          const uint64_t x = gld(&row[fl && r[q] < d.R ? r[q] : 0u]);
          w0[q] = fl ? x : w0[q];
        }
      }
#pragma unroll
      for (int q = 0; q < PLAN_Q; q++) {
        const uint32_t f = fb + tl + T * q, base = fb + T * q;
        const uint32_t k = ck[q];
        const PlanCall &c = pl[k];
        const bool valid = f < tot;
        const bool filt = c.row && !(lmod && c.lk);
        bool live = valid;
        if (valid && filt) {
          const int64_t ts = ts_of(w[q]);
          const bool stale = ts < t_stale;
          const bool gc = st_of(w0[q]) == GX_TOMBSTONE && ts_of(w0[q]) < t_gc;
          live = !stale && (st_of(w0[q]) == GX_ABSENT || ts > ts_of(w0[q]) || gc);
          fs += stale;
        }
        const uint64_t lm = (__ballot(live) >> (tw * T)) & tmask;
#pragma unroll
        for (int kk = 1; kk < PLAN_CH; kk++)
          if (lp[kk] >= base && lp[kk] < base + T) cb[kk] = run + (uint32_t)__popcll(lm & ((1ull << (lp[kk] - base)) - 1ull));
        uint32_t cbk = 0;
#pragma unroll
        for (int kk = 1; kk < PLAN_CH; kk++) cbk = (uint32_t)kk == k ? cb[kk] : cbk;
        const uint32_t rank = filt ? run + (uint32_t)__popcll(lm & ((1ull << tl) - 1ull)) - cbk : f - c.lpre;
        {
          const uint32_t line = valid && filt ? ((c.peer << 15) | (r[q] >> 4)) : 0xffffffffu;
          const uint32_t tb = lane & ~(uint32_t)(T - 1);
          const uint32_t up = (uint32_t)__shfl((int)line, (int)(tl ? lane - 1 : lane), 64);
          const uint32_t prev = tl ? up : lcarry;
          nlines += line != 0xffffffffu && line != prev;
          lcarry = (uint32_t)__shfl((int)line, (int)(tb + T - 1), 64);
        }
        if (live) {
          grec g;
          g.w = w[q];
          g.r = r[q];
          g.pad = 0;
          const uint32_t xo = (c.x - idx * d.KE) * cap + rank;
          grec *to = c.oslot != GX_NOSLOT ? reinterpret_cast<grec *>(ob_slot_hdr(d, c.oslot) + 4) + rank : &msg_t[xo];
          gst_rec(to, g);
          if (filt) gst(&w0_t[xo], w0[q]);
        }
        run += (uint32_t)__popcll(lm);
      }
    }
#pragma unroll
    for (int kk = 1; kk < PLAN_CH; kk++)
      if (lp[kk] == tot) cb[kk] = run;
    uint32_t stored_all = 0;
#ifndef GX_SEND_SPLIT
    if (j <= PLAN_CH) GX_KP(6);
#endif
    GX_SPLIT(1);
    if (tl < nc) {
      const PlanCall &c = pl[tl];
      uint32_t stored = 0;
#pragma unroll
      for (int kk = 0; kk < PLAN_CH; kk++) {
        const uint32_t end = kk + 1 < PLAN_CH && (uint32_t)(kk + 1) < nc ? cb[kk + 1] : run;
        stored = (uint32_t)kk == tl ? end - cb[kk] : stored;
      }
      const uint32_t rv = c.peer - d.lo;
      if (!c.row) stored = c.l;
      if (c.lk & 2u) stored = 0;
      d.msg_len[c.x] = stored;
      d.msg_dst[c.x] = c.peer;
      if (c.oslot != GX_NOSLOT)
        *reinterpret_cast<uint4 *>(ob_slot_hdr(d, c.oslot)) = make_uint4(c.key, c.peer, stored, 0u);
      if (c.row && stored) {
        inbox_header(d, rv, inbox_claim(d, rv), c.key, c.x, stored, lmod && c.lk ? GX_NOSLOT : GX_NOSLOT_W0);
        flag_live(d, rv, stored);
      }
      stored_all = stored + ((c.row && stored) ? 2u : 0u);
    }
    kb += 16ull * stored_all;
    GX_SPLIT(2);
    if (any_push) {
      for (uint32_t k = 0; k < nc; k++) {
        const PlanCall &c = pl[k];
        for (uint32_t qq = (tl - c.nh) & (T - 1); qq < c.push; qq += T) {
          dq[(c.nh + qq) & mask] = plan_item(d, c, c.l + qq);
          kb += 16;
        }
      }
      __threadfence_block();
    }
    wave_sync();
    GX_SPLIT(3);
  }
  GX_SPLIT_FLUSH();
#pragma unroll
  for (int r = 0; r < NR; r++)
    if (osl[r] != GX_NOSLOT && !((emit >> ((uint32_t)r * T + tl)) & 1u))
      *reinterpret_cast<uint4 *>(ob_slot_hdr(d, osl[r])) = make_uint4(GX_SLOT_EMPTY, 0u, 0u, 0u);
  a.c[C_GOSSIP_MERGES] += fm;
  kl += nlines;
  a.c[C_STALE] += fs;
}

GXD bool filt_used(const Dev &d, uint32_t pos) { return d.sfilt && pos != 0xffffffffu; }
#define PLAN_PEERS(QUIET) ((QUIET) ? 0 : PLAN_CH)
template <int T, bool FWD, int SW>
GXD uint32_t quiet_tick(const Dev &d, Acc &a, uint32_t idx, gx_host_state &hs, gx_sleeper *sj, gx_job *pj,
                        uint32_t *peers) {
  const uint32_t tl = threadIdx.x & (T - 1), o = d.lo + idx;
  const bool lead = tl == 0;
  const uint32_t win = d.NG > 1 ? (uint32_t)SW : (uint32_t)T;
  {
    const uint32_t ns = hs.sleep_tail - hs.sleep_head;
    for (uint32_t x = tl; x < ns && x < win; x += T) sj[x] = d.sleep[(size_t)idx * d.SQ + ((hs.sleep_head + x) & (d.SQ - 1u))];
  }
  uint32_t npf = 0;
  if (FWD) {
    const uint32_t q = hs.fifo_stored - hs.fifo_head, pw = pj_window<T>(d);
    npf = q < pw ? q : pw;
    for (uint32_t x = tl; x < npf; x += T) pj[x] = d.fifo[(size_t)idx * d.Q + ((hs.fifo_head + x) % d.Q)];
  }
  if (lead) peers[16] = sample_peers_h(d, peer_seed(d), o, peers);
  wave_sync();
  for (uint32_t w = 0; hs.sleep_head != hs.sleep_tail; w++) {
    if (w == win) {
      const uint32_t ns = hs.sleep_tail - hs.sleep_head;
      wave_sync();
      for (uint32_t x = tl; x < ns && x < win; x += T) sj[x] = d.sleep[(size_t)idx * d.SQ + ((hs.sleep_head + x) & (d.SQ - 1u))];
      wave_sync();
      w = 0;
    }
    const gx_sleeper z = sj[w];
    if ((int64_t)z.wake > d.round) break;
    hs.sleep_head++;
    push_job_r(d, a, o, hs, z.job, lead);
  }
  if (d.p.churn_ppm) {
    const uint64_t x = rng4(d.p.seed, ST_CHURN, (uint64_t)d.round, o, 0);
    if ((uint32_t)(x & 0xffffffffu) % 1000000u < d.p.churn_ppm) {
      const uint32_t cs = (uint32_t)((x >> 32) % d.S);
      hs.running ^= 1ull << cs;
      if (lead && ((hs.running >> cs) & 1ull)) d.own_status[(size_t)idx * d.S + cs] = GX_ALIVE;
      if (lead) a.c[C_CHURN]++;
    }
  }
  return npf;
}
template <int T, bool X, bool PLAN = false, bool FWD = false, bool QUIET = false>
GXD void send_host(const Dev &d, Acc &a, uint32_t idx, gx_job *pjs, int do_bt, unsigned &lost, PlanCall *pl,
                   unsigned long long &kb, unsigned long long &kl, const TickFwd &fwd, uint32_t &quiet,
                   gx_sleeper *sj = nullptr, int nr = 1, uint32_t *lkr = nullptr) {
  const uint32_t lane = threadIdx.x & (T - 1);
  {
    uint32_t u = d.lo + idx;
    uint32_t cap = d.p.packet_cap;
    gx_host_state *h = &d.hs[idx];
    gx_host_state hs = FWD ? fwd.hs : *h;
    const bool tick = do_bt && (FWD ? fwd.tick != 0 : d.tick[idx] != 0);
    bool pre = FWD;
    for (uint32_t j = lane; !QUIET && j < d.KG; j += T) {
      d.msg_len[(size_t)idx * d.KE + j] = 0;
      d.msg_key[(size_t)idx * d.KE + j] = u * d.KE + j;
    }
    const bool pend = do_bt && d.pexp && (hs.lock & GX_LOCK_PENDING_EXPIRE) && !locked_in(d, hs.lock) &&
                      (!X || !departed(d, u));
    if (tick || pend) {
      if (lane == 0) {
        const uint32_t n = d.scan_cnt[idx];
        if (tick) bt_finish(d, a, u, hs.running, &d.scan_list[(size_t)idx * d.L], n < d.L ? n : d.L);
        if (pend) {
          run_pending_expires(d, a, u);
          d.tick[idx] = 2;
        }
      }
      __threadfence_block();
      hs = *h;
      pre = false;
    }
    if (lane == 0) kb += 128;
    GX_KP(4);
    if (PLAN) {
      uint32_t *peers = reinterpret_cast<uint32_t *>(&pl[PLAN_PEERS(QUIET)]);
      if constexpr (QUIET) {
        Dev dr = d;
        uint32_t npf = (pre && fwd.pf0 == hs.fifo_head) ? fwd.npf : 0u;
        for (int i = 0;;) {
          const bool was = a.locked;
          send_planned<T, true>(dr, a, idx, hs, pjs, pl, peers, peers[16], kb, kl, npf);
          hs.lock = lock_snap(hs.lock, hs.flags, dr.round + 1, dr.p.lock_readers != 0);
          if (a.locked && !was) *lkr = (uint32_t)i;
          if (++i >= nr) break;
          next_round_fields(dr);
          dr.kprof = nullptr;
          __threadfence_block();
          wave_sync();
          npf = quiet_tick<T, FWD, FWD ? T * GX_JPF : T>(dr, a, idx, hs, sj, pjs, peers);
          if (lane == 0) kb += 128;
        }
        if (lane == 0) *h = hs;
        if (lane == 0 && d.p.lock_model) quiet = quiet_term(dr, idx, hs);
      } else {
        const uint32_t np = peers[16];
        send_planned<T, QUIET>(d, a, idx, hs, pjs, pl, peers, np, kb, kl, (pre && fwd.pf0 == hs.fifo_head) ? fwd.npf : 0u);
        hs.lock = lock_snap(hs.lock, hs.flags, d.round + 1, d.p.lock_readers != 0);
        if (lane == 0) *h = hs;
        if (lane == 0 && d.p.lock_model) quiet = quiet_term(d, idx, hs);
      }
    } else if (!X || !departed(d, u)) {
      const bool fd = X && d.p.fd_enable;
      uint32_t peers[16];
      uint32_t np;
      if (fd) {
        np = d.fd_np[idx];
        for (uint32_t j = 0; j < np; j++) peers[j] = d.fd_peers[(size_t)idx * d.K + j];
      } else {
        np = sample_peers(d, u, peers);
      }
      const uint32_t head0 = hs.fifo_head, n0 = hs.fifo_stored - head0;
      if (lane < n0 && lane < np * d.NG) pjs[lane] = d.fifo[(size_t)idx * d.Q + ((head0 + lane) % d.Q)];
      const bool early = np <= (uint32_t)T && d.NG == 1;
      uint32_t my_pos = 0xffffffffu;
      if (early && lane < np && (!X || reach(d, u, peers[lane])) && peers[lane] - d.lo < d.Hl)
        my_pos = inbox_claim(d, peers[lane] - d.lo);
      uint32_t called = 0;
      bool stop = false;
      for (uint32_t j = 0; j < np && !stop; j++) {
        const uint32_t pj = peers[j];
        const bool ok = !X || reach(d, u, pj), local = pj - d.lo < d.Hl;
        for (uint32_t n = 0; n < d.NG; n++) {
          const uint32_t c = j * d.NG + n;
          const size_t x = (size_t)idx * d.KE + c;
          uint32_t pos;
          if (early) {
            pos = __shfl(my_pos, (int)j, T);
          } else {
            pos = lane == 0 && ok && local ? inbox_claim(d, pj - d.lo) : 0xffffffffu;
            pos = __shfl(pos, 0, T);
          }
          uint32_t nf = fd ? d.fd_len[x] : 0, lim = d.p.limit_bytes, l = 0;
          bool call = true;
          if (fd && lim) {
            uint32_t used = nf * (d.p.fd_msg_bytes + 2);
            lim = lim > used ? lim - used : 0;
            call = lim > d.p.overhead_bytes;
          }
          grec *pk = pos < d.DR ? &d.in_rec[((size_t)(pj - d.lo) * d.DR + pos) * cap] : &d.msg[x * cap];
          const bool rlk = pos != 0xffffffffu && host_locked(d, pj);
          if (call) {
            const uint32_t q = hs.fifo_head - head0;
            const bool pf = q < n0 && q < (uint32_t)T;
            const bool filt = d.sfilt && pos != 0xffffffffu && !(rlk && d.p.lock_model);
            l = get_broadcasts_team<T>(d, a, u, hs, cap, pk, lim, d.p.overhead_bytes, pf ? &pjs[q] : nullptr,
                                       filt ? &d.view[(size_t)(pj - d.lo) * d.R] : nullptr, pj - d.lo);
          }
          if (rlk && l && lane == 0) {
            a.locked = true;
            if (d.p.lock_model) flag_live(d, pj - d.lo, l);
            else a.c[C_LOCKED_MERGES] += l;
          }
          called = j + 1;
          if (lane == 0) kb += 16 + 32ull * l + (filt_used(d, pos) && !(rlk && d.p.lock_model) ? 8ull * l : 0);
          const bool live = l || nf;
          if (lane == 0) {
            d.msg_len[x] = ok ? l : 0;
            if (fd && !ok) d.fd_len[x] = 0;
            lost += live && !ok;
            d.msg_dst[x] = pj;
            if (pos != 0xffffffffu) inbox_header(d, pj - d.lo, pos, u * d.KE + c, (uint32_t)x, l);
          }
          if (l == 0 && nf == 0) {
            stop = n == 0 && d.p.gossip_stop_on_empty;
            break;
          }
        }
      }
      if (early && lane >= called && my_pos != 0xffffffffu)
        inbox_header(d, peers[lane] - d.lo, my_pos, u * d.KE + lane, (uint32_t)((size_t)idx * d.KE + lane), 0);
      hs.lock = lock_snap(hs.lock, hs.flags, d.round + 1, d.p.lock_readers != 0);
      if (lane == 0) *h = hs;
    }
  }
}

template <int T, bool X, bool SCAN = false, bool VEC = false, bool EV = false, int OWN = 0, bool PLAN = false,
          bool QUIET = false>
__global__ __launch_bounds__(256) void k_send(Dev d, int do_bt, int nr) {
  static_assert(SCAN || (!VEC && !EV && OWN == 0), "k_send: VEC, EV and OWN need SCAN");
  static_assert(!(PLAN && X), "k_send: PLAN runs without departures or the detector (X)");
  static_assert(!QUIET || (PLAN && !EV), "k_send: QUIET needs PLAN and runs without listeners (EV)");
  __shared__ gx_job s_pj[256 / T][T * GX_JPF];
  __shared__ PlanCall s_pl[PLAN ? 256 / T : 1][PLAN_PEERS(QUIET) + 1];
  __shared__ ScanLds sm;
  __shared__ uint32_t s_scan[256 / T], s_nscan;
  constexpr int SLW = OWN ? T * GX_JPF : T;
  __shared__ gx_sleeper s_sl[OWN ? 256 * GX_JPF : QUIET ? 256 : 1];
  Acc a;
  const uint32_t idx = blockIdx.x * (256 / T) + threadIdx.x / T;
  unsigned lost = 0;
  GX_KP(0);
  TickFwd fwd;
  fwd.peers = reinterpret_cast<uint32_t *>(&s_pl[PLAN ? threadIdx.x / T : 0][PLAN_PEERS(QUIET)]);
  if (PLAN && OWN == 0 && (threadIdx.x & (T - 1)) == 0 && idx < d.Hl) {
    uint32_t pr[16];
    const uint32_t np = sample_peers_h(d, peer_seed(d), d.lo + idx, pr);
    for (uint32_t k = 0; k < np; k++) fwd.peers[k] = pr[k];
    fwd.peers[16] = np;
  }
  if (PLAN) wave_sync();
  fwd.pj = s_pj[threadIdx.x / T];
  fwd.npf = 0;
  fwd.pf0 = 0;
  fwd.tick = 0;
  if (d.snap && blockIdx.x == 0) {
    uint32_t v = 0xffffffffu;
    if (d.snap_word == GX_SNAP_QUIET) {
      __shared__ uint32_t s_q[4];
      const uint32_t *q = d.quiet_w + (size_t)((d.round + 1) & 1) * d.QW;
      for (uint32_t i = threadIdx.x; i < d.QW; i += 256) v = q[i] < v ? q[i] : v;
      v = wave_min32(v);
      if ((threadIdx.x & 63) == 0) s_q[threadIdx.x >> 6] = v;
      __syncthreads();
      for (int w = 0; w < 4; w++) v = s_q[w] < v ? s_q[w] : v;
    } else {
      v = d.work_cnt[d.snap_word];
    }
    if (threadIdx.x == 0) *d.snap = ((uint64_t)d.snap_tag << 32) | v;
  }
  if constexpr (OWN > 0) {
    if (threadIdx.x == 0) {
      s_nscan = 0;
      if (blockIdx.x == 0) {
        *d.ovf_cnt_nx = 0;
        *d.wl_cnt_nx = 0;
      }
    }
    __syncthreads();
    const bool q = owner_tick<T, OWN, PLAN, T * GX_JPF>(d, a, idx, &s_sl[(threadIdx.x / T) * SLW], fwd);
    if (q) s_scan[atomicAdd(&s_nscan, 1u)] = idx;
    GX_KP(1);
    __syncthreads();
    GX_KP(2);
    for (uint32_t k = 0; k < s_nscan; k++) {
      const uint32_t oi = s_scan[k];
      scan_view<VEC, EV>(d, oi, &d.scan_list[(size_t)oi * d.L], d.L, &d.scan_cnt[oi], sm);
      __syncthreads();
    }
  } else if (SCAN && *d.wl_cnt) {
    if (threadIdx.x == 0) s_nscan = 0;
    __syncthreads();
    if ((threadIdx.x & (T - 1)) == 0 && idx < d.Hl && d.tick[idx] == 2) s_scan[atomicAdd(&s_nscan, 1u)] = idx;
    __syncthreads();
    for (uint32_t k = 0; k < s_nscan; k++) {
      const uint32_t oi = s_scan[k];
      scan_view<VEC, EV>(d, oi, &d.scan_list[(size_t)oi * d.L], d.L, &d.scan_cnt[oi], sm);
      __syncthreads();
    }
  }
  unsigned long long kb = 0, kl = 0;
  uint32_t quiet = idx < d.Hl && (threadIdx.x & (T - 1)) == 0 ? 0u : 0xffffffffu;
  GX_KP(3);
  uint32_t lkr = 0xffffffffu;
  if (idx < d.Hl)
    send_host<T, X, PLAN, PLAN && (OWN > 0), QUIET>(d, a, idx, s_pj[threadIdx.x / T], do_bt, lost,
                                                   s_pl[PLAN ? threadIdx.x / T : 0], kb, kl, fwd, quiet,
                                                   QUIET ? &s_sl[(threadIdx.x / T) * SLW] : nullptr, QUIET ? nr : 1, &lkr);
  GX_KP(7);
  if constexpr (QUIET) {
    a.locked = false;
    lkr = wave_min32(lkr);
    if (lkr != 0xffffffffu && (threadIdx.x & 63) == 0)
      atomicMin(&d.ctr->first_drop[shard_id()][1], (unsigned long long)(d.round + lkr));
  }
  acc_flush(d, a);
  const int64_t rl = QUIET ? d.round + nr - 1 : d.round;
  if (d.p.lock_model) {
    quiet = wave_min32(quiet);
    if ((threadIdx.x & 63) == 0) d.quiet_w[(size_t)(rl & 1) * d.QW + blockIdx.x * 4u + (threadIdx.x >> 6)] = quiet;
  }
  if (X && lost) ctr_atomic(d, C_LOST, lost);
  kb = wave_sum(kb);
  kl = wave_sum(kl);
  if ((threadIdx.x & 63) == 0) kbytes(d, GX_K_SEND, kb, kl);
  if (PLAN && !QUIET && d.ob_buf) {
    __shared__ uint32_t s_last;
    __syncthreads();
    if (threadIdx.x == 0) {
      __threadfence();
      s_last = atomicAdd(&d.ob_claim[XPLAN_GMAX], 1u) == gridDim.x - 1u;
    }
    __syncthreads();
    if (s_last) {
      __threadfence();
      if (threadIdx.x < d.G && atomicExch(&d.ob_claim[threadIdx.x], 0u) != d.ob_cnt[threadIdx.x])
        atomicOr(&d.work_cnt[GX_WC_ERR], GX_ERR_INBOX);
      if (threadIdx.x == 0) atomicExch(&d.ob_claim[XPLAN_GMAX], 0u);
    }
  }
}


GXD bool probe_tick_at(const Dev &d, int64_t round, uint32_t u) {
  const uint32_t P = d.p.fd_probe_rounds;
  return (uint64_t)round % P == rng4(d.p.seed, ST_FD_PHASE, u, 0, 0) % P;
}
GXD bool probe_tick_of(const Dev &d, uint32_t u) { return probe_tick_at(d, d.round, u); }
GXD uint32_t ob_claim_wave(const Dev &d, uint32_t g) {
  const uint32_t lane = threadIdx.x & 63;
  uint32_t slot = GX_NOSLOT;
  unsigned long long pend = __ballot(g < d.G);
  while (pend) {
    const int src = __builtin_ctzll(pend);
    const uint32_t gs = (uint32_t)__shfl((int)g, src, 64);
    const unsigned long long m = __ballot(g == gs);
    uint32_t base = 0;
    if ((int)lane == src) base = atomicAdd(&d.ob_claim[gs], (uint32_t)__popcll(m));
    base = (uint32_t)__shfl((int)base, src, 64);
    if (g == gs) {
      const uint32_t at = base + (uint32_t)__popcll(m & ((1ull << lane) - 1ull));
      uint32_t st = 0;
      for (uint32_t x = 0; x < gs; x++) st += d.ob_cnt[x];
      if (at < d.ob_cnt[gs]) slot = st + at;
      else atomicOr(&d.work_cnt[GX_WC_ERR], GX_ERR_INBOX);
    }
    pend &= ~m;
  }
  return slot;
}
template <int T>
__global__ __launch_bounds__(256) void k_probe(Dev d) {
  Acc a;
  const uint32_t idx = blockIdx.x * (256 / T) + threadIdx.x / T, lane = threadIdx.x & (T - 1);
  const uint32_t u = d.lo + idx;
  unsigned lost = 0;
  unsigned long long kb = 0;
  uint32_t peer[2] = {0u, 0u}, osl[2] = {GX_NOSLOT, GX_NOSLOT}, cross[2] = {0u, 0u};
  bool act[2] = {false, false};
  if (idx < d.Hl && !departed(d, u)) {
    const uint64_t key = rng4(d.p.seed, ST_PROBE, (uint64_t)d.round, 0, 0);
    if (probe_tick_of(d, u)) {
      peer[0] = feistel_perm(key, u, d.H);
      act[0] = peer[0] != u;
    }
    peer[1] = feistel_inv(key, u, d.H);
    act[1] = peer[1] != u && !departed(d, peer[1]) && probe_tick_of(d, peer[1]) && reach(d, peer[1], u);
  }
  if (d.ob_buf) {
#pragma unroll
    for (int c = 0; c < 2; c++) {
      const bool want = lane == 0 && act[c] && reach(d, u, peer[c]) && peer[c] - d.lo >= d.Hl;
      osl[c] = ob_claim_wave(d, want ? shard_of_d(d, peer[c]) : d.G);
      osl[c] = (uint32_t)__shfl((int)osl[c], 0, T);
    }
  }
  if (idx < d.Hl) {
    const uint32_t cap = d.p.packet_cap;
    gx_host_state *h = &d.hs[idx];
    gx_host_state hs = *h;
#pragma unroll
    for (uint32_t c = 0; c < 2; c++) {
      const size_t x = (size_t)idx * d.KE + d.KG + c;
      if (lane == 0) {
        d.msg_len[x] = 0;
        d.msg_key[x] = u * d.KE + d.KG + c;
      }
      if (!act[c]) continue;
      const uint32_t pr = peer[c];
      const bool ok = reach(d, u, pr), local = pr - d.lo < d.Hl;
      uint32_t pos = lane == 0 && ok && local ? inbox_claim(d, pr - d.lo) : 0xffffffffu;
      pos = (uint32_t)__shfl((int)pos, 0, T);
      uint32_t lim = d.p.limit_bytes;
      bool call = true;
      if (lim) {
        const uint32_t used = d.p.fd_msg_bytes + 2;
        lim = lim > used ? lim - used : 0;
        call = lim > d.p.overhead_bytes;
      }
      grec *pk = pos < d.DR ? &d.in_rec[((size_t)(pr - d.lo) * d.DR + pos) * cap] : &d.msg[x * cap];
      if (osl[c] != GX_NOSLOT) pk = reinterpret_cast<grec *>(ob_slot_hdr(d, osl[c]) + 4);
      const bool rlk = pos != 0xffffffffu && host_locked(d, pr);
      const bool filt = d.sfilt && pos != 0xffffffffu && !(rlk && d.p.lock_model);
      uint32_t l = 0;
      if (call)
        l = get_broadcasts_team<T>(d, a, u, hs, cap, pk, lim, d.p.overhead_bytes, nullptr,
                                   filt ? &d.view[(size_t)(pr - d.lo) * d.R] : nullptr, pr - d.lo);
      if (rlk && l && lane == 0) {
        a.locked = true;
        if (d.p.lock_model) flag_live(d, pr - d.lo, l);
        else a.c[C_LOCKED_MERGES] += l;
      }
      if (lane == 0) {
        kb += 16 + 32ull * l + (filt ? 8ull * l : 0);
        d.msg_len[x] = ok ? l : 0;
        lost += l && !ok;
        d.msg_dst[x] = pr;
        cross[c] = l && ok && !local;
        if (pos != 0xffffffffu) inbox_header(d, pr - d.lo, pos, u * d.KE + d.KG + c, (uint32_t)x, l);
        if (osl[c] != GX_NOSLOT)
          *reinterpret_cast<uint4 *>(ob_slot_hdr(d, osl[c])) =
              l ? make_uint4(u * d.KE + d.KG + c, pr, l, 0u) : make_uint4(GX_SLOT_EMPTY, 0u, 0u, 0u);
      }
    }
    if (lane == 0) *h = hs;
  }
  acc_flush(d, a);
  if (lost) ctr_atomic(d, C_LOST, lost);
  kb = wave_sum(kb);
  if ((threadIdx.x & 63) == 0) kbytes(d, GX_K_SEND, kb, 0);
  if (d.probe_x) {
#pragma unroll
    for (int c = 0; c < 2; c++) {
      const unsigned long long n = wave_sum((unsigned long long)cross[c]);
      if ((threadIdx.x & 63) == 0 && n) atomicAdd(&d.probe_x[c], n);
    }
  }
}

template <bool K32>
GXD uint64_t bitonic64(uint64_t x, uint32_t lane) {
#pragma unroll
  for (uint32_t k = 2; k <= 64; k <<= 1) {
#pragma unroll
    for (uint32_t j = k >> 1; j > 0; j >>= 1) {
      uint64_t o;
      if (K32) o = (uint32_t)__shfl_xor((uint32_t)x, (int)j, 64);
      else o = __shfl_xor(x, (int)j, 64);
      bool keep_min = ((lane & j) == 0) == ((lane & k) == 0);
      x = keep_min ? (o < x ? o : x) : (o > x ? o : x);
    }
  }
  return x;
}

GXD uint32_t rdl(uint32_t x, uint32_t l) { return (uint32_t)__builtin_amdgcn_readlane((int)x, (int)l); }

GXD void merge_inbox_serial(const Dev &d, uint32_t vi, bool lockd = false, uint32_t nbuf = 0) {
  Acc a;
// ... 532 lines not shown
    }
    const uint64_t wn = __shfl(wme, (int)((gs + kk) & (SEG - 1)), SEG);
    if (head && kk < glen) wg = wn;
  }
  c_acc += acc;
  if (head && wg != sw0) {
    row[skey] = wg;
    c_wr++;
    const unsigned long long x = exp_time(d.p, wg);
    mexp = x < mexp ? x : mexp;
  }
  const bool chg = acc && (st_of(wprev) == GX_ABSENT || st_of(wprev) != st_of(wme));
  c_chg += chg;
  uint8_t *s_accf = &L.accf[sb], *s_chg = &L.chg[sb], *s_prev = &L.prev[sb];
  uint64_t *s_accw = &L.accw[sb];
  s_accf[src] = vs && acc && !owned_by(d, skey, v);
  if (EV) {
    s_chg[src] = chg;
    s_prev[src] = (uint8_t)(st_of(wprev) == GX_ABSENT ? GX_UNKNOWN : st_of(wprev));
  }
  s_accw[src] = wme;
  const uint32_t own = vs ? owner_of(d, skey) : 0xffffffffu;
  uint32_t mu = acc ? src + 1 : 0, mc = chg ? src + 1 : 0;
#pragma unroll
  for (int o = 1; o < SEG; o <<= 1) {
    const uint32_t yu = __shfl_down(mu, o, SEG), yc = __shfl_down(mc, o, SEG), yo = __shfl_down(own, o, SEG);
    if (sl + o < (uint32_t)SEG && yo == own) {
      mu = yu > mu ? yu : mu;
      mc = yc > mc ? yc : mc;
    }
  }
  const uint32_t pown = __shfl_up(own, 1, SEG);
  const bool ohead = vs && (sl == 0 || pown != own);
  const uint32_t mcmax = seg_max<SEG>(mc);
  __threadfence_block();
  wave_sync();
  if (ohead && (mu || mc)) {
    gx_server_times *st = srv_times(d, v, own);
    if (mu) st->last_updated_ns = ts_of(s_accw[mu - 1]);
    if (mc) st->last_changed_ns = ts_of(s_accw[mc - 1]);
    c_wr += (mu != 0) + (mc != 0);
  }
  uint32_t n_ev = 0;
  if (EV && evk >= 0) {
    const bool fe = s_chg[sl] != 0;
    const uint64_t me = sballot(fe);
    if (fe) ev_put(d, evk, ev0 + (uint32_t)__popcll(me & ((1ull << sl) - 1ull)), key, s_accw[sl], s_prev[sl]);
    n_ev = (uint32_t)__popcll(me);
  }
  const bool f = s_accf[sl];
  const uint64_t m = sballot(f);
  const uint32_t pos = (uint32_t)__popcll(m & ((1ull << sl) - 1ull));
  if (f && pos < room) d.fifo[(size_t)vi * d.Q + ((tail0 + pos) % d.Q)] = make_job(s_accw[sl], key, meta_of(GX_JOB_RETX, 0, 1));
  n_retx = (uint32_t)__popcll(m);
  c_wr = seg_sum<SEG>((uint32_t)c_wr);
  c_acc = seg_sum<SEG>(c_acc);
  c_chg = seg_sum<SEG>(c_chg);
#pragma unroll
  for (int o = SEG / 2; o > 0; o >>= 1) {
    const unsigned long long y = __shfl_xor(mexp, o, SEG);
    mexp = y < mexp ? y : mexp;
  }
  if (sl == 0) {
    const uint32_t ok = n_retx < room ? n_retx : room;
    if (n_retx) {
      d.hs[vi].fifo_tail = tail0 + n_retx;
      d.hs[vi].fifo_stored = st0 + ok;
    }
    if (mcmax) d.vlc[vi] = ts_of(s_accw[mcmax - 1]);
    if (EV && evk >= 0) d.ev_cnt[evk] = ev0 + n_ev;
    ctr_atomic(d, C_CHG, c_chg);
    kbytes(d, GX_K_MERGE, 12ull * total + 8ull * (total + c_wr) + 16ull * ok + 16ull * deg + 4, total);
    ctr_atomic(d, C_GOSSIP_ACC, c_acc);
    ctr_atomic(d, C_RETX, n_retx);
    ctr_atomic(d, C_QDEFER, n_retx - ok);
    if (c_wr) {
      mark_change(d);
      atomicMin(&d.minexp[vi], mexp);
    }
  }
  wave_sync();
  return true;
}

#ifndef MERGE_WPE_GM
#define MERGE_WPE_GM 4
#endif
#ifndef LOCK_RPL
#define LOCK_RPL 4
#endif
template <int SEG>
GXD bool lock_append_seg(const Dev &d, uint32_t vi, bool act) {
  const uint32_t lane = threadIdx.x & 63, sl = lane & (SEG - 1), sb = lane & ~(uint32_t)(SEG - 1);
  const uint32_t deg = act ? d.in_cnt[vi] : 0u;
  const uint32_t lw = act ? d.hs[vi].lock : 0u;
  uint4 hd = d.in_hdr[(size_t)vi * d.DI + (sl < d.DI ? sl : 0u)];
  if (deg > (uint32_t)SEG || deg > d.DI) return false;
  if (sl >= deg) hd = make_uint4(0xffffffffu, 0u, 0u, 0u);
  uint32_t start = 0, total = 0;
  for (uint32_t j = 0; j < (uint32_t)SEG; j++) {
    const uint32_t kj = (uint32_t)__shfl((int)hd.x, (int)(sb + j), 64);
    const uint32_t lj = (uint32_t)__shfl((int)hd.z, (int)(sb + j), 64);
    const bool before = j < deg && (kj < hd.x || (kj == hd.x && j < sl));
    start += before ? lj : 0u;
    total += j < deg ? lj : 0u;
  }
  const uint32_t capv = pipe_cap(d, vi, lw), nb0 = GX_LOCK_BUF(lw), room = capv > nb0 ? capv - nb0 : 0u;
  const uint32_t keep = total < room ? total : room;
  grec *dst = act ? &d.lkb[(size_t)vi * d.C + nb0] : d.lkb;
  for (uint32_t o0 = 0; o0 < keep; o0 += SEG * LOCK_RPL) {
    grec g[LOCK_RPL];
#pragma unroll
    for (int q = 0; q < LOCK_RPL; q++) {
      const uint32_t o = o0 + sl + SEG * q;
      uint32_t entry = 0, slot = 0, off = 0;
      for (uint32_t j = 0; j < deg; j++) {
        const uint32_t sj = (uint32_t)__shfl((int)start, (int)(sb + j), 64);
        const uint32_t lj = (uint32_t)__shfl((int)hd.z, (int)(sb + j), 64);
        const uint32_t ej = (uint32_t)__shfl((int)hd.y, (int)(sb + j), 64);
        const uint32_t wj = (uint32_t)__shfl((int)hd.w, (int)(sb + j), 64);
        if (o >= sj && o < sj + lj) {
          entry = ej;
          slot = wj;
          off = o - sj;
        }
      }
      g[q] = gld_rec(&packet_recs(d, vi, slot, entry)[off]);
    }
#pragma unroll
    for (int q = 0; q < LOCK_RPL; q++) {
      const uint32_t o = o0 + sl + SEG * q;
      if (o < keep) gst_rec(&dst[o], g[q]);
    }
  }
  if (act && sl == 0 && deg) {
    d.hs[vi].lock = (lw & ((1u << GX_LOCK_BUF_SHIFT) - 1u)) | (nb0 + keep) << GX_LOCK_BUF_SHIFT;
    ctr_atomic(d, C_LOCK_BUF, keep);
    ctr_atomic(d, C_LOCK_DROP, total - keep);
    kbytes(d, GX_K_MERGE, 32ull * keep + 16ull * deg + 4, 0);
  }
  return true;
}

#ifndef GX_LOCK_APPEND_WPE
#define GX_LOCK_APPEND_WPE 8
#endif
__global__ __launch_bounds__(256) __attribute__((amdgpu_waves_per_eu(GX_LOCK_APPEND_WPE))) void k_lock_append(Dev d) {
  const uint32_t vi = (blockIdx.x * 256u + threadIdx.x) >> 4;
  bool act = false;
  if (vi < d.Hl) act = d.mrec[vi] != 0 && locked_in(d, d.hs[vi].lock);
  if (__ballot(act) == 0) return;
  const bool ok = lock_append_seg<16>(d, act ? vi : 0u, act);
  if (act && ok && (threadIdx.x & 15) == 0) d.mrec[vi] = 0;
}

#define MERGE_NR 64
#define MERGE_NONE 0xffffffffu
template <bool K32, bool EV, int NR = MERGE_NR, int WPE = 3>
__global__ __launch_bounds__(64 * MERGE_WAVES) __attribute__((amdgpu_waves_per_eu(WPE))) void k_merge_seg(Dev d) {
  static_assert(NR <= 64, "one routing lane per receiver");
  __shared__ MergeLds s_l[MERGE_WAVES];
  __shared__ uint32_t s_it[NR][4];
  __shared__ uint32_t s_ty[NR];
  __shared__ uint32_t s_fb[NR], s_n[2];
  const uint32_t wv = threadIdx.x >> 6, lane = threadIdx.x & 63;
  const uint32_t r0 = blockIdx.x * NR;
  if (wv == 0) {
    const uint32_t vi = r0 + lane;
    uint32_t t = 0;
    if (lane < (uint32_t)NR && vi < d.Hl) t = d.mrec[vi];
    if (t) d.mrec[vi] = 0;
    if (lane < (uint32_t)NR)
      for (int q = 0; q < 4; q++) s_it[lane][q] = MERGE_NONE;
    bool lkw = false, lka = false;
    if (d.p.lock_model && lane < (uint32_t)NR && vi < d.Hl) {
      const uint32_t lw = d.hs[vi].lock;
      if (locked_in(d, lw) && d.p.fd_handoff_shared) t = 0;
      else if (locked_in(d, lw)) lka = t != 0;
      else lkw = GX_LOCK_BUF(lw) != 0 && !departed(d, d.lo + vi);
    }
    const bool sm = !lkw && !lka && t && t <= 16, md = !lkw && !lka && t > 16 && t <= 32;
    const bool lg = lkw || (!lka && t > 32);
    const uint64_t bs = __ballot(sm), bm = __ballot(md), bl = __ballot(lg), ba = __ballot(lka), below = (1ull << lane) - 1ull;
    const uint32_t nl = (uint32_t)__popcll(bl), nm = (uint32_t)__popcll(bm), ns = (uint32_t)__popcll(bs);
    const uint32_t na = (uint32_t)__popcll(ba);
    const uint32_t nim = (nm + 1) / 2, nis = (ns + 3) / 4, nia = (na + 3) / 4;
    wave_sync();
    if (lka) {
      const uint32_t q = (uint32_t)__popcll(ba & below), it = nl + nim + nis + q / 4;
      s_it[it][q & 3] = vi;
      s_ty[it] = 3;
    } else if (lg) {
      const uint32_t it = (uint32_t)__popcll(bl & below);
      s_it[it][0] = vi;
      s_ty[it] = 2;
    } else if (md) {
      const uint32_t q = (uint32_t)__popcll(bm & below), it = nl + q / 2;
      s_it[it][q & 1] = vi;
      s_ty[it] = 1;
    } else if (sm) {
      const uint32_t q = (uint32_t)__popcll(bs & below), it = nl + nim + q / 4;
      s_it[it][q & 3] = vi;
      s_ty[it] = 0;
    }
    if (lane == 0) {
      s_n[0] = nl + nim + nis + nia;
      s_n[1] = 0;
    }
    if (unsigned long long *kp = kprof_merge(d); kp && lane == 0 && (nl | nm | ns)) {
      atomicAdd(&kp[0], (unsigned long long)(nl + nm + ns));
      atomicAdd(&kp[1], (unsigned long long)ns);
      atomicAdd(&kp[2], (unsigned long long)nm);
      atomicAdd(&kp[3], (unsigned long long)nl);
    }
    if (unsigned long long *kp = kprof_merge(d); kp && t) atomicAdd(&kp[5], (unsigned long long)t);
  }
  __syncthreads();
  const uint32_t ni = s_n[0];
  if (ni == 0) return;
  for (uint32_t it = wv; it < ni; it += MERGE_WAVES) {
    const uint32_t ty = s_ty[it];
    if (ty == 2) {
      merge_receiver<K32, EV>(d, s_it[it][0], s_l[wv]);
    } else if (ty == 3) {
      const uint32_t v = s_it[it][lane >> 4];
      const bool act = v != MERGE_NONE;
      const bool ok = lock_append_seg<16>(d, act ? v : 0u, act);
      if (!ok && (lane & 15) == 0) s_fb[atomicAdd(&s_n[1], 1u)] = v;
    } else if (ty == 1) {
      const uint32_t v = s_it[it][lane >> 5];
      const bool act = v != MERGE_NONE;
      const bool ok = merge_seg<K32, EV, 32>(d, act ? v : 0u, act, s_l[wv]);
      if (!ok && (lane & 31) == 0) s_fb[atomicAdd(&s_n[1], 1u)] = v;
    } else {
      const uint32_t v = s_it[it][lane >> 4];
      const bool act = v != MERGE_NONE;
      const bool ok = merge_seg<K32, EV, 16>(d, act ? v : 0u, act, s_l[wv]);
      if (!ok && (lane & 15) == 0) s_fb[atomicAdd(&s_n[1], 1u)] = v;
    }
  }
  __syncthreads();
  const uint32_t nf = s_n[1];
  if (unsigned long long *kp = kprof_merge(d); kp && threadIdx.x == 0 && nf) atomicAdd(&kp[4], (unsigned long long)nf);
  for (uint32_t k = wv; k < nf; k += MERGE_WAVES) merge_receiver<K32, EV>(d, s_fb[k], s_l[wv]);
}

template <bool NT>
GXD ulonglong2 ld16(const uint64_t *p) {
  if (NT) {
    typedef unsigned long long v2u64 __attribute__((ext_vector_type(2)));
    v2u64 x = __builtin_nontemporal_load(reinterpret_cast<const v2u64 *>(p));
    return make_ulonglong2(x.x, x.y);
  }
  return *reinterpret_cast<const ulonglong2 *>(p);
}

GXD void side_times_shfl(const Dev &d, uint32_t x, uint32_t base, uint32_t f, const uint64_t *nw, uint32_t &lk,
                         uint32_t &words_written) {
  const uint32_t t = threadIdx.x, lane = t & 63, lpo = d.S / 2;
#pragma unroll
  for (int h = 0; h < 2; h++) {
    const uint32_t r0 = base + 512 * h + 2 * t;
    const uint32_t fa0 = (f >> (2 * h)) & 1u, fa1 = (f >> (2 * h + 1)) & 1u;
    const uint32_t fc0 = (f >> (4 + 2 * h)) & 1u, fc1 = (f >> (4 + 2 * h + 1)) & 1u;
    const uint64_t bu_all = __ballot(fa0 | fa1);
    if (!bu_all) continue;
    const uint32_t g0 = lane & ~(lpo - 1);
    const uint64_t gmask = (lpo == 32 ? 0xffffffffull : ((1ull << lpo) - 1ull)) << g0;
    const uint64_t bu = bu_all & gmask, bc = __ballot(fc0 | fc1) & gmask;
    const bool wu = bu && lane == 63u - (uint32_t)__clzll((long long)bu);
    const bool wc = bc && lane == 63u - (uint32_t)__clzll((long long)bc);
    if (wu || wc) {
      gx_server_times *st = srv_times(d, x, owner_of(d, r0));
      if (wu) st->last_updated_ns = ts_of(fa1 ? nw[2 * h + 1] : nw[2 * h]);
      if (wc) st->last_changed_ns = ts_of(fc1 ? nw[2 * h + 1] : nw[2 * h]);
      words_written += (uint32_t)wu + (uint32_t)wc;
    }
    const uint32_t kc = fc1 ? r0 + 2 : (fc0 ? r0 + 1 : 0u);
    lk = kc > lk ? kc : lk;
  }
}

template <bool VEC, bool EV>
GXD uint32_t ae_book(const Dev &d, uint32_t a, uint32_t b, bool both, uint32_t base, uint32_t fl, uint32_t os,
                     const uint64_t *A, const uint64_t *B, uint32_t *s_lu, uint32_t *s_lc, uint32_t *s_last,
                     unsigned long long *s_wave, int32_t evka, int32_t evkb, uint32_t evba, uint32_t evbb) {
  const uint32_t t = threadIdx.x, TILE = 4 * blockDim.x;
  const uint32_t o0 = base / d.S, no = ((base + TILE < d.R ? base + TILE : d.R) - 1) / d.S - o0 + 1;
  unsigned long long epre = 0, etot = 0;
  if (EV) {
    const unsigned long long ec = (unsigned long long)__popc(fl & 0x30u) |
                                  ((unsigned long long)__popc(fl & 0xC0u) << 16) |
                                  ((unsigned long long)__popc(fl & 0x3000u) << 32) |
                                  ((unsigned long long)__popc(fl & 0xC000u) << 48);
    epre = block_excl_scan64(ec, s_wave, etot);
  }
  for (int side = 0; side < (both ? 2 : 1); side++) {
    const uint64_t *X = side ? B : A;
    for (uint32_t i = t; i < no; i += blockDim.x) s_lu[i] = s_lc[i] = 0;
    __syncthreads();
#pragma unroll
    for (int k = 0; k < 4; k++) {
      const uint32_t r = (VEC ? base + 512 * (k >> 1) + 2 * t : base + 2 * blockDim.x * (k >> 1) + 2 * t) + (k & 1);
      if ((fl >> (8 * side + k)) & 1u) atomicMax(&s_lu[owner_of(d, r) - o0], r + 1);
      if ((fl >> (8 * side + 4 + k)) & 1u) {
        atomicMax(&s_lc[owner_of(d, r) - o0], r + 1);
// ... 2022 lines not shown
```

Measured before the change: 4.091 billion.

## Batch multiple locked rounds into one send plus one lock-append launch

Adds a locked-batch mode in which rounds where every host is locked are run as a single multi-round k_send, writing into per-round inbox slots, followed by a single k_lock_append_batch kernel that appends all rounds' records into the lock buffers. A second quiet reduction lane (uint2 quiet_w, snap_lk) tells the host how many future rounds are safely locked. The aim is to cut per-round launch and host-sync overhead during long locked stretches. The cost is extra device memory for LB slots, a wider quiet word and more complex batch-eligibility logic on the host. It also adds profiling scripts.

```diff
diff --git a/profiles/locked_batch/resources.py b/profiles/locked_batch/resources.py
--- /dev/null
+++ b/profiles/locked_batch/resources.py
@@ -0,0 +1,54 @@
+import json
+import os
+import re
+import subprocess
+import sys
+import tempfile
+
+LLVM = os.path.join(os.environ.get("ROCM_PATH", "/opt/rocm"), "llvm", "bin")
+NAME = re.compile(r"_Z6k_sendILi4ELb0ELb([01])ELb([01])ELb0ELi(\d)ELb1ELb([01])E(?:Lb([01])E)?Ev3Dev\w*|_Z\d+(k_lock_append\w*?)3Dev\w*")
+FIELDS = {"TotalSGPRs": "sgprs", "VGPRs": "vgprs", "ScratchSize [bytes/lane]": "scratch", "Occupancy [waves/SIMD]": "waves_per_simd",
+          "SGPRs Spill": "sgpr_spills", "LDS Size [bytes/block]": "lds"}
+
+
+def remarks(path):
+    out, cur = {}, None
+    for line in open(path):
+        m = re.search(r"remark: Function Name: (\S+)", line)
+        if m:
+            cur = out.setdefault(m.group(1), {}) if NAME.fullmatch(m.group(1)) else None
+            continue
+        m = re.search(r"remark:\s+([^:]+): (\d+) \[", line)
+        if m and cur is not None and m.group(1) in FIELDS:
+            cur[FIELDS[m.group(1)]] = int(m.group(2))
+    return out
+
+
+def code_sizes(lib):
+    with tempfile.TemporaryDirectory() as tmp:
+        co = os.path.join(tmp, "gfx950.co")
+        sec = os.path.join(tmp, "fatbin")
+        subprocess.run([os.path.join(LLVM, "llvm-objcopy"), "-O", "binary", "--only-section=.hip_fatbin", lib, sec], check=True)
+        subprocess.run([os.path.join(LLVM, "clang-offload-bundler"), "--unbundle", "--type=o", "--allow-missing-bundles",
+                        "--targets=hipv4-amdgcn-amd-amdhsa--gfx950", f"--input={sec}", f"--output={co}"], check=True)
+        txt = subprocess.run([os.path.join(LLVM, "llvm-readelf"), "-s", "-W", co], check=True, stdout=subprocess.PIPE).stdout.decode()
+    sizes = {}
+    for line in txt.splitlines():
+        f = line.split()
+        if len(f) >= 8 and f[3] == "FUNC" and NAME.fullmatch(f[7]):
+            sizes[f[7]] = max(sizes.get(f[7], 0), int(f[2]))
+    return sizes
+
+
+if __name__ == "__main__":
+    rem, sizes = remarks(sys.argv[1]), code_sizes(sys.argv[2])
+    rows = []
+    for name, r in rem.items():
+        g = NAME.fullmatch(name).groups()
+        if g[5]:
+            rows.append(dict(kernel=g[5], scan=9, vec=0, own=0, quiet=0, lkb=0, **r, code_bytes=sizes.get(name)))
+            continue
+        scan, vec, own, quiet, lkb = (int(x or 0) for x in g[:5])
+        rows.append(dict(scan=scan, vec=vec, own=own, quiet=quiet, lkb=lkb, **r, code_bytes=sizes.get(name)))
+    for row in sorted(rows, key=lambda x: (x["scan"], x["vec"], x["own"], x["quiet"], x["lkb"], x.get("kernel", ""))):
+        print(json.dumps(row))
diff --git a/profiles/locked_batch/stretch.py b/profiles/locked_batch/stretch.py
--- /dev/null
+++ b/profiles/locked_batch/stretch.py
@@ -0,0 +1,25 @@
+import json
+import os
+import sys
+import time
+
+sys.path.insert(0, os.getcwd())
+import bench
+from sidecar_amd.abi import load_product
+
+FIRST, N = 12, 30
+
+if __name__ == "__main__":
+    lib = load_product()
+    e = bench.make_engine(lib, "cfg5", 0x5EED, 0)
+    e.run_rounds(FIRST)
+    t0 = e.timing()
+    a = time.perf_counter()
+    e.run_rounds(N)
+    dt = time.perf_counter() - a
+    t1 = e.timing()
+    launches = {k: t1[k]["launches"] - t0[k]["launches"] for k in t1 if t1[k]["launches"] != t0[k]["launches"]}
+    print(json.dumps({"lib": sys.argv[1], "locked_batch_env": os.environ.get("GX_LOCKED_BATCH"),
+                      "rounds": f"{FIRST}..{FIRST + N - 1}", "us_per_round": round(dt * 1e6 / N, 2), "launches": launches,
+                      "send_bytes": t1["send"]["bytes"] - t0["send"]["bytes"],
+                      "send_units": t1["send"]["units"] - t0["send"]["units"]}))
diff --git a/profiles/locked_batch/trace_sum.py b/profiles/locked_batch/trace_sum.py
--- /dev/null
+++ b/profiles/locked_batch/trace_sum.py
@@ -0,0 +1,46 @@
+import csv
+import json
+import re
+import sys
+
+OTHERS = ("k_lock_append", "k_lock_append_batch", "k_merge_seg", "k_ae_chunk", "k_ae_locked_note", "k_storm_p2")
+
+
+def short(name):
+    m = re.search(r"(k_\w+)(<[^>]*>)?", name)
+    return (m.group(1), (m.group(1) + (m.group(2) or ""))) if m else (name, name)
+
+
+if __name__ == "__main__":
+    rows = []
+    with open(sys.argv[2]) as f:
+        for r in csv.DictReader(f):
+            base, inst = short(r["Kernel_Name"])
+            rows.append((int(r["Start_Timestamp"]), int(r["End_Timestamp"]), base, inst))
+    rows.sort()
+    sends = [r for r in rows if r[2] == "k_send"]
+    t_win = sends[2][0]
+    out = {"lib": sys.argv[1], "k_send_launches_in_process": len(sends), "k_send": {"launches": 0, "us": 0.0}, "k_send_instances": {},
+           "send_order": []}
+    for a, b, base, inst in rows:
+        if a < t_win:
+            continue
+        us = (b - a) / 1e3
+        if base == "k_send":
+            out["k_send"]["launches"] += 1
+            out["k_send"]["us"] += us
+            i = out["k_send_instances"].setdefault(inst, {"launches": 0, "us": 0.0})
+            i["launches"] += 1
+            i["us"] += us
+            tp = [x.strip() for x in inst[inst.index("<") + 1:-1].split(",")] if "<" in inst else []
+            letter = "L" if len(tp) > 8 and tp[8] in ("true", "1") else "Q" if len(tp) > 7 and tp[7] in ("true", "1") else "G"
+            out["send_order"].append(f"{letter}{us:.0f}")
+        elif base in OTHERS:
+            o = out.setdefault(base, {"launches": 0, "us": 0.0})
+            o["launches"] += 1
+            o["us"] += us
+    for v in [out["k_send"], *out["k_send_instances"].values(), *(out[k] for k in OTHERS if k in out)]:
+        v["us"] = round(v["us"], 1)
+        v["us_per_launch"] = round(v["us"] / max(1, v["launches"]), 2)
+    out["window_us"] = round((max(r[1] for r in rows) - t_win) / 1e3, 1)
+    print(json.dumps(out))
diff --git a/sidecar_amd/csrc/gx_device.hpp b/sidecar_amd/csrc/gx_device.hpp
--- a/sidecar_amd/csrc/gx_device.hpp
+++ b/sidecar_amd/csrc/gx_device.hpp
@@ -140,8 +140,16 @@
   uint32_t nblk_ae;
   uint64_t *snap;
   uint32_t snap_tag, snap_word;
-  uint32_t *quiet_w;
+  uint2 *quiet_w;
   uint32_t QW;
+  uint64_t *snap_lk;
+  uint32_t LB, lb_par;
+  grec *lb_msg;
+  uint4 *lb_hdr;
+  uint32_t *lb_cnt;
+  uint4 *lb_ovf;
+  uint32_t *lb_ovfc;
+  uint32_t *lb_rd;
   uint32_t sfilt;
   uint32_t C;
   grec *lkb;
@@ -396,6 +404,17 @@
   const uint64_t b = (uint64_t)d.round + 1u + (dist + kg) / kg;
   return b < 0xfffffffeull ? (uint32_t)b : 0xfffffffeu;
 }
+GXD uint32_t locked_term(const Dev &d, const gx_host_state &hs) {
+  const uint32_t lw = hs.lock;
+  if (!(hs.flags & 3u) || !locked_in(d, lw) || !GX_LOCK_AT(lw, d.round + 1)) return 0u;
+  uint32_t dist = 0;
+  if (hs.flags & 1u) dist = hs.nil_pos_bs - hs.fifo_head;
+  if ((hs.flags & 2u) && hs.nil_pos_bt - hs.fifo_head > dist) dist = hs.nil_pos_bt - hs.fifo_head;
+  if (dist >= hs.fifo_tail - hs.fifo_head) return 0u;
+  const uint32_t kg = d.KG ? d.KG : 1u;
+  const uint64_t b = (uint64_t)d.round + 1u + (dist + kg) / kg;
+  return b < 0xfffffffeull ? (uint32_t)b : 0xfffffffeu;
+}
 GXD void next_round_fields(Dev &d) {
   d.round++;
   d.now = d.p.t0_ns + d.round * d.p.round_ns;
@@ -407,6 +426,14 @@
   d.wl_cnt_nx = wl;
   d.ovf_cnt = d.ovf_cnt_nx;
   d.ovf_cnt_nx = ov;
+}
+GXD void lb_slot_fields(Dev &d, const Dev &d0, uint32_t i) {
+  d.msg = d0.lb_msg + (size_t)i * d0.H * d0.KE * d0.p.packet_cap;
+  d.in_hdr = d0.lb_hdr + (size_t)i * d0.Hl * d0.DI;
+  d.in_cnt = d0.lb_cnt + (size_t)i * d0.Hl;
+  d.in_ovf = d0.lb_ovf + (size_t)i * d0.H * d0.KE;
+  d.ovf_cnt = d0.lb_ovfc + (size_t)d0.lb_par * d0.LB + i;
+  d.msg_len = d0.lb_rd + (size_t)i * d0.H * d0.KE;
 }
 GXD void note_locked(const Dev &d) { atomicMin(&d.ctr->first_drop[shard_id()][1], (unsigned long long)d.round); }
 
diff --git a/sidecar_amd/csrc/gx_engine.hip b/sidecar_amd/csrc/gx_engine.hip
--- a/sidecar_amd/csrc/gx_engine.hip
+++ b/sidecar_amd/csrc/gx_engine.hip
@@ -145,9 +145,12 @@
   uint32_t quiet_tag[GX_QUIET_SLOTS], quiet_seq;
   bool quiet_nowait;
   int64_t quiet_until, quiet_from;
+  int64_t locked_until;
   bool quiet_now;
   bool quiet_send = true;
   uint32_t quiet_batch;
+  uint32_t locked_batch;
+  bool lb_off;
   uint32_t *in_cnt_buf;
   int async_phases;
   int device;
@@ -444,9 +447,11 @@
   for (int i = GX_QUIET_SLOTS - 1; i >= 0; i--) {
     if (e->quiet_tag[i]) {
       const uint64_t v = __atomic_load_n(&e->scan_snap[2 + i], __ATOMIC_ACQUIRE);
-      if ((uint32_t)(v >> 32) != e->quiet_tag[i]) continue;
+      const uint64_t v2 = __atomic_load_n(&e->scan_snap[2 + GX_QUIET_SLOTS + i], __ATOMIC_ACQUIRE);
+      if ((uint32_t)(v >> 32) != e->quiet_tag[i] || (uint32_t)(v2 >> 32) != e->quiet_tag[i]) continue;
       e->quiet_tag[i] = 0;
       if ((int64_t)(uint32_t)v > e->quiet_until) e->quiet_until = (int64_t)(uint32_t)v;
+      if ((int64_t)(uint32_t)v2 > e->locked_until) e->locked_until = (int64_t)(uint32_t)v2;
     }
     free_slot = i;
   }
@@ -471,12 +476,14 @@
   if (!++e->quiet_seq) ++e->quiet_seq;
   e->quiet_tag[free_slot] = e->quiet_seq;
   d.snap = &e->scan_snap_dev[2 + free_slot];
+  d.snap_lk = &e->scan_snap_dev[2 + GX_QUIET_SLOTS + free_slot];
   d.snap_tag = e->quiet_seq;
   d.snap_word = GX_SNAP_QUIET;
 }
 static void quiet_invalidate(gx_engine *e) {
   memset(e->quiet_tag, 0, sizeof(e->quiet_tag));
   e->quiet_until = 0;
+  e->locked_until = 0;
   e->quiet_from = e->d.round;
 }
 
@@ -499,12 +506,22 @@
 struct SendSel {
   bool x, scan, plan;
   int own;
-  bool quiet;
+  bool quiet, locked;
 };
 static void launch_send(gx_engine *e, SendSel sel, int do_bt, int nr) {
   const Dev &d = e->d;
   const unsigned g = nblk(d.Hl, 64);
   hipStream_t s = e->stream;
+  if (sel.locked && sel.plan && !ev_of(e)) {
+    if (!sel.scan) {
+      k_send<4, false, false, false, false, 0, true, false, true><<<g, 256, 0, s>>>(d, do_bt, nr);
+      return;
+    }
+    with_flag(vec_of(e), [&](auto V) {
+      with_own(sel.own, [&](auto O) { k_send<4, false, true, V(), false, O(), true, false, true><<<g, 256, 0, s>>>(d, do_bt, nr); });
+    });
+    return;
+  }
   if (sel.quiet && sel.plan && !ev_of(e)) {
     if (!sel.scan) {
       k_send<4, false, false, false, false, 0, true, true><<<g, 256, 0, s>>>(d, do_bt, nr);
@@ -528,7 +545,7 @@
   else with_flag(sel.x, [&](auto X) { rest(X, std::false_type{}); });
 }
 
-static int round_send_impl(gx_engine *e, int nr = 1) {
+static int round_send_impl(gx_engine *e, int nr = 1, bool locked = false) {
   Dev &d = e->d;
   set_round_fields(e);
   InRound in_round_guard(d);
@@ -553,9 +570,9 @@
   const bool scan_in_send = !bt_apart && d.K && !e->scan_heavy;
   const bool fused = scan_in_send && d.S <= 16;
   const bool plan = !d.p.limit_bytes && d.p.retransmit_rounds > 0 && !d.departures && !d.p.fd_enable;
-  e->quiet_now = quiet_round(e, storm);
+  e->quiet_now = !locked && quiet_round(e, storm);
   const SendSel sel{d.p.fd_enable || d.departures, scan_in_send, plan, fused ? own_class(d.S) : 0,
-                    e->quiet_now && e->quiet_send};
+                    e->quiet_now && e->quiet_send, locked};
   if (!fused) {
     LaunchTimer t(e, GX_K_OWNER);
     owner_launch(d, s);
@@ -588,7 +605,7 @@
   {
     LaunchTimer t(e, GX_K_SEND);
     if (d.p.fd_enable) k_fd_send<<<nblk(d.Hl, 64), 64, 0, s>>>(d);
-    launch_send(e, sel, bt_apart ? 0 : 1, sel.quiet ? nr : 1);
+    launch_send(e, sel, bt_apart ? 0 : 1, sel.quiet || sel.locked ? nr : 1);
   }
   HIPCHK(hipGetLastError());
   return scan_probe_end(e);
@@ -850,11 +867,15 @@
   d.round = r0;
   return n < 2 ? 1 : n;
 }
+static int batch_pp_note(gx_engine *e, uint32_t n);
 static int run_quiet_batch(gx_engine *e, uint32_t n) {
-  Dev &d = e->d;
   int rc = round_send_impl(e, (int)n);
   e->quiet_now = false;
   if (rc) return rc;
+  return batch_pp_note(e, n);
+}
+static int batch_pp_note(gx_engine *e, uint32_t n) {
+  Dev &d = e->d;
   const int64_t r0 = d.round;
   int64_t first = -1;
   uint32_t pairs = 0;
@@ -875,6 +896,68 @@
   d.round = r0 + n;
   HIPCHK(hipGetLastError());
   return GX_OK;
+}
+
+#ifndef GX_LOCKED_BATCH
+#define GX_LOCKED_BATCH 8
+#endif
+static int lb_alloc(gx_engine *e) {
+  Dev &d = e->d;
+  const size_t LB = e->locked_batch, Hg = d.H, H = d.Hl, K = d.KE;
+  hipStream_t s = e->stream;
+  int rc = e->mem.take(d.lb_msg, sizeof(grec) * LB * Hg * K * d.p.packet_cap);
+  if (!rc) rc = e->mem.take(d.lb_hdr, sizeof(uint4) * LB * H * d.DI);
+  if (!rc) rc = e->mem.take(d.lb_cnt, sizeof(uint32_t) * LB * H, 0, s);
+  if (!rc) rc = e->mem.take(d.lb_ovf, sizeof(uint4) * LB * Hg * K);
+  if (!rc) rc = e->mem.take(d.lb_ovfc, sizeof(uint32_t) * 2 * LB, 0, s);
+  if (!rc) rc = e->mem.take(d.lb_rd, sizeof(uint32_t) * LB * Hg * K);
+  if (rc) {
+    e->mem.drop(d.lb_msg);
+    e->mem.drop(d.lb_hdr);
+    e->mem.drop(d.lb_cnt);
+    e->mem.drop(d.lb_ovf);
+    e->mem.drop(d.lb_ovfc);
+    e->mem.drop(d.lb_rd);
+    return rc;
+  }
+  d.LB = (uint32_t)LB;
+  d.lb_par = 0;
+  return GX_OK;
+}
+static uint32_t locked_batch_len(gx_engine *e, uint32_t left) {
+  Dev &d = e->d;
+  if (e->locked_batch < 2 || e->quiet_batch < 2 || e->lb_off || left < 2 || !e->quiet_send || !quiet_params(d) ||
+      !e->log_views.empty() || e->watch.n)
+    return 1;
+  const int64_t r0 = d.round;
+  if (r0 >= e->locked_until) return 1;
+  uint32_t n = (uint32_t)std::min<int64_t>({(int64_t)left, (int64_t)e->locked_batch, e->locked_until - r0});
+  for (uint32_t j = 0; j < n; j++) {
+    d.round = r0 + j;
+    const bool storm = d.p.storm_round >= 0 && d.round == d.p.storm_round;
+    if (storm || (d.p.push_pull_mode == GX_PP_INITIATE && ae_round(e))) n = j;
+  }
+  d.round = r0;
+  if (n < 2) return 1;
+  if (!d.LB && lb_alloc(e)) {
+    (void)hipGetLastError();
+    e->lb_off = true;
+    return 1;
+  }
+  return n;
+}
+static int run_locked_batch(gx_engine *e, uint32_t n) {
+  Dev &d = e->d;
+  int rc = round_send_impl(e, (int)n, true);
+  e->quiet_now = false;
+  if (rc) return rc;
+  {
+    LaunchTimer t(e, GX_K_MERGE);
+    k_lock_append_batch<<<nblk(d.Hl, 16), 256, 0, e->stream>>>(d, n);
+  }
+  e->launches[GX_K_MERGE] += n - 1;
+  d.lb_par ^= 1u;
+  return batch_pp_note(e, n);
 }
 
 static int wake_all(gx_engine *e) {
@@ -1086,6 +1169,8 @@
   if (const char *qs = getenv("GX_QUIET_SEND")) e->quiet_send = strcmp(qs, "0") != 0;
   e->quiet_batch = GX_QUIET_BATCH;
   if (const char *qb = getenv("GX_QUIET_BATCH")) e->quiet_batch = (uint32_t)std::min(std::max(atol(qb), 1l), 1024l);
+  e->locked_batch = GX_LOCKED_BATCH;
+  if (const char *lb = getenv("GX_LOCKED_BATCH")) e->locked_batch = (uint32_t)std::min(std::max(atol(lb), 1l), (long)GX_LB_MAX);
   if (d.G > 1) {
     e->nblk = d.nblk_ae;
     e->nmw = (e->nblk + 31) / 32;
@@ -1098,10 +1183,10 @@
   HIPCHK(hipStreamCreateWithFlags(&e->side_stream, hipStreamNonBlocking));
   HIPCHK(hipEventCreateWithFlags(&e->side_start, hipEventDisableTiming));
   HIPCHK(hipEventCreateWithFlags(&e->side_done, hipEventDisableTiming));
-  HIPCHK(hipHostMalloc((void **)&e->scan_snap, (2 + GX_QUIET_SLOTS) * sizeof(uint64_t), hipHostMallocMapped));
+  HIPCHK(hipHostMalloc((void **)&e->scan_snap, (2 + 2 * GX_QUIET_SLOTS) * sizeof(uint64_t), hipHostMallocMapped));
   HIPCHK(hipHostGetDevicePointer((void **)&e->scan_snap_dev, e->scan_snap, 0));
   e->scan_snap[0] = e->scan_snap[1] = ~0ull;
-  for (int i = 0; i < GX_QUIET_SLOTS; i++) e->scan_snap[2 + i] = 0;
+  for (int i = 0; i < 2 * GX_QUIET_SLOTS; i++) e->scan_snap[2 + i] = 0;
   return GX_OK;
 }
 
@@ -1132,7 +1217,7 @@
   TAKE(GX_CK_IN_OVF, d.in_ovf, sizeof(uint4) * Hg * K);
   TAKE(GX_CK_IN_REC, d.in_rec, sizeof(grec) * H * d.DR * p->packet_cap);
   TAKE(GX_CK_WORK_CNT, d.work_cnt, sizeof(uint32_t) * GX_WC_N, 0, s);
-  TAKE(DERIVED, d.quiet_w, sizeof(uint32_t) * 2 * d.QW, 0, s);
+  TAKE(DERIVED, d.quiet_w, sizeof(uint2) * 2 * d.QW, 0, s);
   TAKE(GX_CK_WORK, d.work, sizeof(uint32_t) * H);
   if (p->push_pull_mode == GX_PP_INITIATE && d.G < 2) {
     TAKE(DERIVED, e->pp_dev, sizeof(uint32_t) * 2 * Hg);
@@ -1288,9 +1373,11 @@
   GXTRY(enter(e, ENTRY_ROUNDS));
   e->quiet_nowait = false;
   for (uint32_t i = 0; i < n_rounds;) {
-    const uint32_t nb = quiet_batch_len(e, n_rounds - i);
-    int rc = nb > 1 ? run_quiet_batch(e, nb) : run_one_round(e);
+    uint32_t nb = quiet_batch_len(e, n_rounds - i);
+    const uint32_t nl = nb > 1 ? 1 : locked_batch_len(e, n_rounds - i);
+    int rc = nb > 1 ? run_quiet_batch(e, nb) : nl > 1 ? run_locked_batch(e, nl) : run_one_round(e);
     if (rc) return rc;
+    nb = nb > 1 ? nb : nl;
     i += nb;
     if (e->pending_ev.size() > 4096) {
       rc = drain_timing(e);
diff --git a/sidecar_amd/csrc/gx_kernels.hpp b/sidecar_amd/csrc/gx_kernels.hpp
--- a/sidecar_amd/csrc/gx_kernels.hpp
+++ b/sidecar_amd/csrc/gx_kernels.hpp
@@ -1352,7 +1352,7 @@
   return g;
 }
 
-template <int T, bool QUIET = false>
+template <int T, bool QUIET = false, bool LKB = false>
 GXD void send_planned(const Dev &d, Acc &a, uint32_t idx, gx_host_state &hs, gx_job *pjs, PlanCall *pl,
                       const uint32_t *peers, uint32_t np, unsigned long long &kb, unsigned long long &kl,
                       uint32_t npf0 = 0) {
@@ -1372,9 +1372,9 @@
   bool stop = np == 0;
   unsigned fm = 0, fs = 0, nlines = 0;
   GX_SPLIT_DECL
-  const bool lmod = QUIET || d.p.lock_model != 0;
+  const bool lmod = QUIET || LKB || d.p.lock_model != 0;
   constexpr int NR = (16 + T - 1) / T;
-  const bool direct = !QUIET && d.ob_buf != nullptr;
+  const bool direct = !QUIET && !LKB && d.ob_buf != nullptr;
   uint32_t osl[NR];
   uint32_t emit = 0;
 #pragma unroll
@@ -1428,12 +1428,12 @@
       }
     }
   }
-  uint32_t lkm = QUIET ? ~0u : 0u, fullm = lkm;
+  uint32_t lkm = QUIET || LKB ? ~0u : 0u, fullm = QUIET ? ~0u : 0u;
   for (uint32_t j0 = 0; !QUIET && j0 < np; j0 += T) {
     const uint32_t jj = j0 + tl;
     const uint32_t lw = jj < np && peers[jj] - d.lo < d.Hl ? gld(&hst(d, peers[jj])->lock) : 0u;
-    const bool lk = locked_in(d, lw);
-    lkm |= (uint32_t)((__ballot(lk) >> (tw * T)) & tmask) << j0;
+    const bool lk = LKB ? jj < np : locked_in(d, lw);
+    if (!LKB) lkm |= (uint32_t)((__ballot(lk) >> (tw * T)) & tmask) << j0;
     const bool full = lk && GX_LOCK_BUF(lw) >= pipe_cap(d, jj < np ? peers[jj] - d.lo : 0u, lw);
     fullm |= (uint32_t)((__ballot(full) >> (tw * T)) & tmask) << j0;
   }
@@ -1575,7 +1575,7 @@
           a.c[C_PACKETS]++;
           a.c[C_RECSENT] += l;
           const uint32_t lb = l < c.m ? l : c.m;
-          const bool filt = c.row && !(lmod && c.lk);
+          const bool filt = !LKB && c.row && !(lmod && c.lk);
           if (c.lk & 2u) {
             a.c[C_LOCK_DROP] += l;
           } else {
@@ -1669,7 +1669,7 @@
         lx[q] = gld3(src);
         w[q] = c.bw;
         r[q] = c.rb + (c.kind == GX_JOB_EXPIRE ? (c.emask ? nth_set_bit(c.emask, i) : i) : 0u);
-        const bool filt = valid && c.row && !(lmod && c.lk);
+        const bool filt = valid && !LKB && c.row && !(lmod && c.lk);
         const uint64_t *row = filt ? c.row : reinterpret_cast<const uint64_t *>(dq);
         w0[q] = gld(&row[filt && sel[q] == 0 && r[q] < d.R ? r[q] : 0u]);
       }
@@ -1680,14 +1680,14 @@
         if (sel[q]) {
           w[q] = ((uint64_t)lx[q].x | ((uint64_t)lx[q].y << 32)) + (sel[q] == 1 ? w[q] : 0ull);
           r[q] = lx[q].z;
-          reload |= c.row && !(lmod && c.lk);
+          reload |= !LKB && c.row && !(lmod && c.lk);
         }
       }
       if (__ballot(reload)) {
 #pragma unroll
         for (int q = 0; q < PLAN_Q; q++) {
           const PlanCall &c = pl[ck[q]];
-          const bool fl = sel[q] && c.row && !(lmod && c.lk);
+          const bool fl = sel[q] && !LKB && c.row && !(lmod && c.lk);
           const uint64_t *row = fl ? c.row : reinterpret_cast<const uint64_t *>(dq);
           const uint64_t x = gld(&row[fl && r[q] < d.R ? r[q] : 0u]);
           w0[q] = fl ? x : w0[q];
@@ -1699,7 +1699,7 @@
         const uint32_t k = ck[q];
         const PlanCall &c = pl[k];
         const bool valid = f < tot;
-        const bool filt = c.row && !(lmod && c.lk);
+        const bool filt = !LKB && c.row && !(lmod && c.lk);
         bool live = valid;
         if (valid && filt) {
           const int64_t ts = ts_of(w[q]);
@@ -1756,13 +1756,18 @@
       const uint32_t rv = c.peer - d.lo;
       if (!c.row) stored = c.l;
       if (c.lk & 2u) stored = 0;
-      d.msg_len[c.x] = stored;
+      if constexpr (LKB) {
+        const uint32_t lb = c.l < c.m ? c.l : c.m;
+        d.msg_len[c.x] = (c.kind == GX_JOB_SEND ? lb : 0u) + (c.l - lb);
+      } else {
+        d.msg_len[c.x] = stored;
+      }
       d.msg_dst[c.x] = c.peer;
       if (c.oslot != GX_NOSLOT)
         *reinterpret_cast<uint4 *>(ob_slot_hdr(d, c.oslot)) = make_uint4(c.key, c.peer, stored, 0u);
       if (c.row && stored) {
         inbox_header(d, rv, inbox_claim(d, rv), c.key, c.x, stored, lmod && c.lk ? GX_NOSLOT : GX_NOSLOT_W0);
-        flag_live(d, rv, stored);
+        if (!LKB) flag_live(d, rv, stored);
       }
       stored_all = stored + ((c.row && stored) ? 2u : 0u);
     }
@@ -1835,9 +1840,9 @@
   }
   return npf;
 }
-template <int T, bool X, bool PLAN = false, bool FWD = false, bool QUIET = false>
+template <int T, bool X, bool PLAN = false, bool FWD = false, bool QUIET = false, bool LKB = false>
 GXD void send_host(const Dev &d, Acc &a, uint32_t idx, gx_job *pjs, int do_bt, unsigned &lost, PlanCall *pl,
-                   unsigned long long &kb, unsigned long long &kl, const TickFwd &fwd, uint32_t &quiet,
+                   unsigned long long &kb, unsigned long long &kl, const TickFwd &fwd, uint2 &quiet,
                    gx_sleeper *sj = nullptr, int nr = 1, uint32_t *lkr = nullptr) {
   const uint32_t lane = threadIdx.x & (T - 1);
   {
@@ -1870,16 +1875,18 @@
     GX_KP(4);
     if (PLAN) {
       uint32_t *peers = reinterpret_cast<uint32_t *>(&pl[PLAN_PEERS(QUIET)]);
-      if constexpr (QUIET) {
+      if constexpr (QUIET || LKB) {
         Dev dr = d;
+        if constexpr (LKB) lb_slot_fields(dr, d, 0u);
         uint32_t npf = (pre && fwd.pf0 == hs.fifo_head) ? fwd.npf : 0u;
         for (int i = 0;;) {
           const bool was = a.locked;
-          send_planned<T, true>(dr, a, idx, hs, pjs, pl, peers, peers[16], kb, kl, npf);
+          send_planned<T, QUIET, LKB>(dr, a, idx, hs, pjs, pl, peers, peers[16], kb, kl, npf);
           hs.lock = lock_snap(hs.lock, hs.flags, dr.round + 1, dr.p.lock_readers != 0);
           if (a.locked && !was) *lkr = (uint32_t)i;
           if (++i >= nr) break;
           next_round_fields(dr);
+          if constexpr (LKB) lb_slot_fields(dr, d, (uint32_t)i);
           dr.kprof = nullptr;
           __threadfence_block();
           wave_sync();
@@ -1887,13 +1894,13 @@
           if (lane == 0) kb += 128;
         }
         if (lane == 0) *h = hs;
-        if (lane == 0 && d.p.lock_model) quiet = quiet_term(dr, idx, hs);
+        if (lane == 0 && d.p.lock_model) quiet = make_uint2(quiet_term(dr, idx, hs), locked_term(dr, hs));
       } else {
         const uint32_t np = peers[16];
         send_planned<T, QUIET>(d, a, idx, hs, pjs, pl, peers, np, kb, kl, (pre && fwd.pf0 == hs.fifo_head) ? fwd.npf : 0u);
         hs.lock = lock_snap(hs.lock, hs.flags, d.round + 1, d.p.lock_readers != 0);
         if (lane == 0) *h = hs;
-        if (lane == 0 && d.p.lock_model) quiet = quiet_term(d, idx, hs);
+        if (lane == 0 && d.p.lock_model) quiet = make_uint2(quiet_term(d, idx, hs), locked_term(d, hs));
       }
     } else if (!X || !departed(d, u)) {
       const bool fd = X && d.p.fd_enable;
@@ -1972,17 +1979,19 @@
 }
 
 template <int T, bool X, bool SCAN = false, bool VEC = false, bool EV = false, int OWN = 0, bool PLAN = false,
-          bool QUIET = false>
-__global__ __launch_bounds__(256) void k_send(Dev d, int do_bt, int nr) {
+          bool QUIET = false, bool LKB = false>
+__global__ __launch_bounds__(256) __attribute__((amdgpu_waves_per_eu(LKB ? 2 : 0))) void k_send(Dev d, int do_bt, int nr) {
   static_assert(SCAN || (!VEC && !EV && OWN == 0), "k_send: VEC, EV and OWN need SCAN");
   static_assert(!(PLAN && X), "k_send: PLAN runs without departures or the detector (X)");
   static_assert(!QUIET || (PLAN && !EV), "k_send: QUIET needs PLAN and runs without listeners (EV)");
+  static_assert(!LKB || (PLAN && !EV && !QUIET), "k_send: LKB needs PLAN, runs without listeners (EV) and is not QUIET");
   __shared__ gx_job s_pj[256 / T][T * GX_JPF];
   __shared__ PlanCall s_pl[PLAN ? 256 / T : 1][PLAN_PEERS(QUIET) + 1];
   __shared__ ScanLds sm;
   __shared__ uint32_t s_scan[256 / T], s_nscan;
   constexpr int SLW = OWN ? T * GX_JPF : T;
-  __shared__ gx_sleeper s_sl[OWN ? 256 * GX_JPF : QUIET ? 256 : 1];
+  constexpr bool BATCH = QUIET || LKB;
+  __shared__ gx_sleeper s_sl[OWN ? 256 * GX_JPF : BATCH ? 256 : 1];
   Acc a;
   const uint32_t idx = blockIdx.x * (256 / T) + threadIdx.x / T;
   unsigned lost = 0;
@@ -2001,15 +2010,24 @@
   fwd.pf0 = 0;
   fwd.tick = 0;
   if (d.snap && blockIdx.x == 0) {
-    uint32_t v = 0xffffffffu;
+    uint32_t v = 0xffffffffu, v2 = 0xffffffffu;
     if (d.snap_word == GX_SNAP_QUIET) {
-      __shared__ uint32_t s_q[4];
-      const uint32_t *q = d.quiet_w + (size_t)((d.round + 1) & 1) * d.QW;
-      for (uint32_t i = threadIdx.x; i < d.QW; i += 256) v = q[i] < v ? q[i] : v;
+      __shared__ uint2 s_q[4];
+      const uint2 *q = d.quiet_w + (size_t)((d.round + 1) & 1) * d.QW;
+      for (uint32_t i = threadIdx.x; i < d.QW; i += 256) {
+        const uint2 t = q[i];
+        v = t.x < v ? t.x : v;
+        v2 = t.y < v2 ? t.y : v2;
+      }
       v = wave_min32(v);
-      if ((threadIdx.x & 63) == 0) s_q[threadIdx.x >> 6] = v;
+      v2 = wave_min32(v2);
+      if ((threadIdx.x & 63) == 0) s_q[threadIdx.x >> 6] = make_uint2(v, v2);
       __syncthreads();
-      for (int w = 0; w < 4; w++) v = s_q[w] < v ? s_q[w] : v;
+      for (int w = 0; w < 4; w++) {
+        v = s_q[w].x < v ? s_q[w].x : v;
+        v2 = s_q[w].y < v2 ? s_q[w].y : v2;
+      }
+      if (threadIdx.x == 0) *d.snap_lk = ((uint64_t)d.snap_tag << 32) | v2;
     } else {
       v = d.work_cnt[d.snap_word];
     }
@@ -2046,31 +2064,32 @@
     }
   }
   unsigned long long kb = 0, kl = 0;
-  uint32_t quiet = idx < d.Hl && (threadIdx.x & (T - 1)) == 0 ? 0u : 0xffffffffu;
+  const uint32_t q0 = idx < d.Hl && (threadIdx.x & (T - 1)) == 0 ? 0u : 0xffffffffu;
+  uint2 quiet = make_uint2(q0, q0);
   GX_KP(3);
   uint32_t lkr = 0xffffffffu;
   if (idx < d.Hl)
-    send_host<T, X, PLAN, PLAN && (OWN > 0), QUIET>(d, a, idx, s_pj[threadIdx.x / T], do_bt, lost,
-                                                   s_pl[PLAN ? threadIdx.x / T : 0], kb, kl, fwd, quiet,
-                                                   QUIET ? &s_sl[(threadIdx.x / T) * SLW] : nullptr, QUIET ? nr : 1, &lkr);
+    send_host<T, X, PLAN, PLAN && (OWN > 0), QUIET, LKB>(d, a, idx, s_pj[threadIdx.x / T], do_bt, lost,
+                                                        s_pl[PLAN ? threadIdx.x / T : 0], kb, kl, fwd, quiet,
+                                                        BATCH ? &s_sl[(threadIdx.x / T) * SLW] : nullptr, BATCH ? nr : 1, &lkr);
   GX_KP(7);
-  if constexpr (QUIET) {
+  if constexpr (BATCH) {
     a.locked = false;
     lkr = wave_min32(lkr);
     if (lkr != 0xffffffffu && (threadIdx.x & 63) == 0)
       atomicMin(&d.ctr->first_drop[shard_id()][1], (unsigned long long)(d.round + lkr));
   }
   acc_flush(d, a);
-  const int64_t rl = QUIET ? d.round + nr - 1 : d.round;
+  const int64_t rl = BATCH ? d.round + nr - 1 : d.round;
   if (d.p.lock_model) {
-    quiet = wave_min32(quiet);
+    quiet = make_uint2(wave_min32(quiet.x), wave_min32(quiet.y));
     if ((threadIdx.x & 63) == 0) d.quiet_w[(size_t)(rl & 1) * d.QW + blockIdx.x * 4u + (threadIdx.x >> 6)] = quiet;
   }
   if (X && lost) ctr_atomic(d, C_LOST, lost);
   kb = wave_sum(kb);
   kl = wave_sum(kl);
   if ((threadIdx.x & 63) == 0) kbytes(d, GX_K_SEND, kb, kl);
-  if (PLAN && !QUIET && d.ob_buf) {
+  if (PLAN && !BATCH && d.ob_buf) {
     __shared__ uint32_t s_last;
     __syncthreads();
     if (threadIdx.x == 0) {
@@ -2909,6 +2928,115 @@
   if (__ballot(act) == 0) return;
   const bool ok = lock_append_seg<16>(d, act ? vi : 0u, act);
   if (act && ok && (threadIdx.x & 15) == 0) d.mrec[vi] = 0;
+}
+
+#define GX_LB_MAX 16
+#ifndef GX_LB_GRP
+#define GX_LB_GRP 4
+#endif
+#ifndef GX_LB_APPEND_WPE
+#define GX_LB_APPEND_WPE 4
+#endif
+template <int SEG>
+GXD void lock_append_rounds(const Dev &d, uint32_t vi, bool act, uint32_t n) {
+  const uint32_t lane = threadIdx.x & 63, sl = lane & (SEG - 1), sb = lane & ~(uint32_t)(SEG - 1);
+  const uint32_t lw = act ? d.hs[vi].lock : 0u;
+  const uint32_t capv = pipe_cap(d, vi, lw), nb0 = GX_LOCK_BUF(lw);
+  uint32_t nb = nb0, drop = 0, hdrs = 0, rr = 0;
+  unsigned long long back = 0;
+  for (uint32_t s0 = 0; s0 < n; s0 += GX_LB_GRP) {
+    uint32_t degs[GX_LB_GRP];
+    uint4 hds[GX_LB_GRP];
+#pragma unroll
+    for (int g = 0; g < GX_LB_GRP; g++) {
+      const uint32_t s = s0 + g < n ? s0 + g : s0;
+      degs[g] = act && s0 + g < n ? d.lb_cnt[(size_t)s * d.Hl + vi] : 0u;
+      hds[g] = d.lb_hdr[((size_t)s * d.Hl + vi) * d.DI + (sl < d.DI ? sl : 0u)];
+    }
+#pragma unroll
+    for (int g = 0; g < GX_LB_GRP; g++) {
+      const uint32_t deg = degs[g];
+      if (deg == 0) continue;
+      Dev ds = d;
+      lb_slot_fields(ds, d, s0 + g);
+      const uint32_t room = capv > nb ? capv - nb : 0u;
+      grec *dst = &d.lkb[(size_t)vi * d.C + nb];
+      uint32_t total = 0, keep = 0;
+      if (deg > (uint32_t)SEG || deg > d.DI) {
+        unsigned long long bk = 0;
+        if (sl == 0) {
+          int64_t after = -1;
+          for (uint32_t k = 0; k < deg; k++) {
+            const uint4 h = inbox_next(ds, vi, after);
+            after = (int64_t)h.x;
+            const grec *src = packet_recs(ds, vi, h.w, h.y);
+            for (uint32_t i = 0; i < h.z; i++, total++)
+              if (total < room) gst_rec(&dst[total], gld_rec(&src[i]));
+            if (!room) bk += 16ull * (ds.msg_len[h.y] + h.z + 2u);
+          }
+          back += bk;
+        }
+        total = (uint32_t)__shfl((int)total, (int)sb, 64);
+        keep = total < room ? total : room;
+      } else {
+        uint4 hd = hds[g];
+        if (sl >= deg) hd = make_uint4(0xffffffffu, 0u, 0u, 0u);
+        uint32_t start = 0;
+        for (uint32_t j = 0; j < (uint32_t)SEG; j++) {
+          const uint32_t kj = (uint32_t)__shfl((int)hd.x, (int)(sb + j), 64);
+          const uint32_t lj = (uint32_t)__shfl((int)hd.z, (int)(sb + j), 64);
+          const bool before = j < deg && (kj < hd.x || (kj == hd.x && j < sl));
+          start += before ? lj : 0u;
+          total += j < deg ? lj : 0u;
+        }
+        keep = total < room ? total : room;
+        for (uint32_t o0 = 0; o0 < keep; o0 += SEG * LOCK_RPL) {
+          grec r[LOCK_RPL];
+#pragma unroll
+          for (int q = 0; q < LOCK_RPL; q++) {
+            const uint32_t o = o0 + sl + SEG * q;
+            uint32_t entry = 0, slot = 0xffffffffu, off = 0;
+            for (uint32_t j = 0; j < deg; j++) {
+              const uint32_t sj = (uint32_t)__shfl((int)start, (int)(sb + j), 64);
+              const uint32_t lj = (uint32_t)__shfl((int)hd.z, (int)(sb + j), 64);
+              const uint32_t ej = (uint32_t)__shfl((int)hd.y, (int)(sb + j), 64);
+              const uint32_t wj = (uint32_t)__shfl((int)hd.w, (int)(sb + j), 64);
+              if (o >= sj && o < sj + lj) {
+                entry = ej;
+                slot = wj;
+                off = o - sj;
+              }
+            }
+            r[q] = gld_rec(&packet_recs(ds, vi, slot, entry)[off]);
+          }
+#pragma unroll
+          for (int q = 0; q < LOCK_RPL; q++) {
+            const uint32_t o = o0 + sl + SEG * q;
+            if (o < keep) gst_rec(&dst[o], r[q]);
+          }
+        }
+        if (!room && sl < deg) back += 16ull * (ds.msg_len[hd.y] + hd.z + 2u);
+      }
+      nb += keep;
+      drop += total - keep;
+      hdrs += deg;
+      rr++;
+      if (sl == 0) ds.in_cnt[vi] = 0;
+    }
+  }
+  if (back) atomicAdd(&d.ctr->bytes[shard_id()][GX_K_SEND], 0ull - back);
+  if (act && sl == 0 && hdrs) {
+    d.hs[vi].lock = (lw & ((1u << GX_LOCK_BUF_SHIFT) - 1u)) | nb << GX_LOCK_BUF_SHIFT;
+    ctr_atomic(d, C_LOCK_BUF, nb - nb0);
+    ctr_atomic(d, C_LOCK_DROP, drop);
+    kbytes(d, GX_K_MERGE, 32ull * (nb - nb0) + 16ull * hdrs + 4ull * rr, 0);
+  }
+}
+__global__ __launch_bounds__(256) __attribute__((amdgpu_waves_per_eu(GX_LB_APPEND_WPE))) void k_lock_append_batch(Dev d, uint32_t n) {
+  if (blockIdx.x == 0 && threadIdx.x < d.LB) d.lb_ovfc[(size_t)(d.lb_par ^ 1u) * d.LB + threadIdx.x] = 0;
+  const uint32_t vi = (blockIdx.x * 256u + threadIdx.x) >> 4;
+  const bool act = vi < d.Hl;
+  lock_append_rounds<16>(d, act ? vi : 0u, act, n);
 }
 
 #define MERGE_NR 64
```

Measured after the change: 3.406 billion. 16.7% lower.
